# simonsobs/hmvec

Hardware: AMD Instinct MI355X
Metric: (z,m,k) grid-points/sec for P_1h+P_2h (higher is better)
Workload: dtype f64

## Files before the change

hmvec_amd/_native.py:

```python
import ctypes as C
import math
import os

import numpy as np

_HERE = os.path.dirname(os.path.abspath(__file__))
LIB_PATH = os.environ.get("HMG_LIB_PATH") or os.path.join(_HERE, "libhmgrid.so")
ABI_VERSION = 10
COMM_ID_BYTES = 128

c_double_p = C.c_void_p


class NativeError(RuntimeError):
    pass


class HaloStageArgs(C.Structure):
    _fields_ = [("d_zs", C.c_void_p), ("d_delta", C.c_void_p), ("d_rho", C.c_void_p),
                ("duffy_A", C.c_double), ("duffy_alpha", C.c_double), ("duffy_beta", C.c_double),
                ("h", C.c_double), ("d_cs", C.c_void_p), ("d_rvir", C.c_void_p), ("d_rs", C.c_void_p),
                ("d_nfw_series", C.c_void_p), ("d_drho1", C.c_void_p), ("delta2", C.c_double),
                ("d_rho2", C.c_void_p), ("d_m2", C.c_void_p), ("d_r2", C.c_void_p)]


class MassFnParams(C.Structure):
    _fields_ = [("mode", C.c_int), ("deltac", C.c_double), ("st_A", C.c_double),
                ("st_a", C.c_double), ("st_p", C.c_double), ("rho_m0", C.c_double),
                ("lnm_uniform", C.c_int), ("lnm_step", C.c_double)]


class HodParams(C.Structure):
    _fields_ = [("sig_log_mstellar", C.c_double), ("alphasat", C.c_double), ("Bsat", C.c_double),
                ("betasat", C.c_double), ("Bcut", C.c_double), ("betacut", C.c_double),
                ("corr", C.c_int)]


class Tracer(C.Structure):
    _fields_ = [("kind", C.c_int), ("d_prof", C.c_void_p), ("d_cprof", C.c_void_p),
                ("d_Nc", C.c_void_p), ("d_Ns", C.c_void_p), ("d_NcNs", C.c_void_p),
                ("d_NsNsm1", C.c_void_p), ("d_ngal", C.c_void_p),
                ("d_bias_override", C.c_void_p),
                ("d_prof_nconst", C.c_void_p), ("d_prof_cconst", C.c_void_p),
                ("d_cprof_nconst", C.c_void_p), ("d_cprof_cconst", C.c_void_p)]


class MassFnPart(C.Structure):
    _fields_ = [("h_par", C.POINTER(MassFnParams)), ("d_ms", C.c_void_p), ("d_lnms", C.c_void_p),
                ("d_tinker_z", C.c_void_p), ("d_sigma2", C.c_void_p), ("d_nzm", C.c_void_p), ("d_bh", C.c_void_p)]


class HodPart(C.Structure):
    _fields_ = [("stage", C.c_int), ("h_par", C.POINTER(HodParams)), ("d_zs", C.c_void_p), ("d_ms", C.c_void_p),
                ("d_log10mstar_thresh", C.c_void_p), ("d_nzm", C.c_void_p), ("d_bh", C.c_void_p),
                ("d_wm", C.c_void_p), ("d_Nc", C.c_void_p), ("d_Ns", C.c_void_p), ("d_NsNsm1", C.c_void_p),
                ("d_NcNs", C.c_void_p), ("d_ngal", C.c_void_p), ("d_bg", C.c_void_p)]


class RowsPart(C.Structure):
    _fields_ = [("kind", C.c_int), ("d_m200c", C.c_void_p), ("d_r200c", C.c_void_p), ("d_rvir", C.c_void_p),
                ("d_zs", C.c_void_p), ("d_rhocz", C.c_void_p), ("d_hz", C.c_void_p), ("fit", C.c_double * 9),
                ("gamma", C.c_double), ("alpha_const", C.c_double), ("amp_prefactor", C.c_double),
                ("post_prefactor", C.c_double), ("d_amp", C.c_void_p), ("d_xc", C.c_void_p),
                ("d_alpha", C.c_void_p), ("d_expo", C.c_void_p), ("d_cmax", C.c_void_p),
                ("d_rscale", C.c_void_p), ("d_post", C.c_void_p),
                ("d_ks", C.c_void_p), ("d_kts", C.c_void_p), ("nk", C.c_int), ("fft_m", C.c_int), ("d_rowsc", C.c_void_p)]


class NfwPart(C.Structure):
    _fields_ = [("d_cs", C.c_void_p), ("d_rs", C.c_void_p), ("d_zs", C.c_void_p), ("d_ks", C.c_void_p),
                ("d_nfw_series", C.c_void_p), ("d_uk", C.c_void_p)]


class ProfileFftPart(C.Structure):
    _fields_ = [("nxs", C.c_int), ("fft_step", C.c_double), ("d_xs", C.c_void_p), ("d_kts", C.c_void_p),
                ("d_amp", C.c_void_p), ("d_xc", C.c_void_p), ("d_alpha", C.c_void_p), ("d_expo", C.c_void_p),
                ("amp_const", C.c_double), ("xc_const", C.c_double), ("alpha_const", C.c_double),
                ("expo_const", C.c_double), ("gamma", C.c_double), ("d_cmax", C.c_void_p), ("d_rss", C.c_void_p),
                ("d_zs", C.c_void_p), ("d_ks", C.c_void_p), ("do_mass_norm", C.c_int), ("d_post", C.c_void_p),
                ("d_out", C.c_void_p), ("d_nconst", C.c_void_p), ("d_cconst", C.c_void_p), ("d_logxs", C.c_void_p),
                ("d_rowsc", C.c_void_p)]


class PowerBatchDesc(C.Structure):
    _fields_ = [("ntr", C.c_int), ("h_tr", C.POINTER(Tracer)), ("npairs", C.c_int),
                ("h_pair_a", C.POINTER(C.c_int)), ("h_pair_b", C.POINTER(C.c_int)),
                ("d_nzm", C.c_void_p), ("d_bh", C.c_void_p), ("d_ms", C.c_void_p), ("d_wm", C.c_void_p),
                ("d_ks", C.c_void_p), ("d_Pzk", C.c_void_p), ("rho_m0", C.c_double), ("kstar", C.c_double),
                ("h_P1h", C.POINTER(C.c_void_p)), ("h_P2h", C.POINTER(C.c_void_p))]


PB_PREPARED = 1
HOD_ALL, HOD_OCCUPATIONS, HOD_SUMS = 0, 1, 2
MF_SHETH_TORMEN, MF_TINKER10 = 0, 1
PROF_BATTAGLIA_GAS, PROF_BATTAGLIA_PRES = 1, 2
TRACER_MATTER, TRACER_HOD, TRACER_PRESSURE = 0, 1, 2
KERNEL_POWER, KERNEL_NFW, KERNEL_PROFILE_FFT = 0, 1, 2
EVENT_SLOTS = 4096
NFW_SERIES_STRIDE = 36
ROWSC_STRIDE = 8

_I, _D, _P, _Z = C.c_int, C.c_double, C.c_void_p, C.c_size_t
SIGNATURES = {
    "hmg_abi_version": [],
    "hmg_ctx_create": [_I, C.POINTER(_P)],
    "hmg_ctx_destroy": [_P],
    "hmg_malloc": [_P, _Z, C.POINTER(_P)],
    "hmg_free": [_P, _P],
    "hmg_memcpy_h2d": [_P, _P, _P, _Z],
    "hmg_memcpy_d2h": [_P, _P, _P, _Z],
    "hmg_memcpy_d2d": [_P, _P, _P, _Z],
    "hmg_sync": [_P],
    "hmg_host_alloc": [_P, _Z, C.POINTER(_P)],
    "hmg_host_free": [_P, _P],
    "hmg_memcpy_d2h_async": [_P, _P, _P, _Z],
    "hmg_memcpy_h2d_async": [_P, _P, _P, _Z],
    "hmg_event_synchronize": [_P, _I],
    "hmg_graph_begin": [_P],
    "hmg_graph_end": [_P, C.POINTER(_I)],
    "hmg_graph_abort": [_P],
    "hmg_graph_kernel_nodes": [_P, _I, C.POINTER(_I)],
    "hmg_graph_launch": [_P, _I],
    "hmg_graph_destroy": [_P, _I],
    "hmg_lane_set": [_P, _I],
    "hmg_profile_support_epoch": [_P, C.c_longlong],
    "hmg_event_wait": [_P, _I],
    "hmg_event_record": [_P, _I],
    "hmg_elapsed_ms": [_P, _I, _I, C.POINTER(_D)],
    "hmg_bracket_next": [_P, _I, _I, _I],
    "hmg_sigma2": [_P, _I, _I, _I, _P, _P, _P, _P, _D, _P],
    "hmg_sigma2_layout_size": [_I, _I, C.POINTER(_Z)],
    "hmg_sigma2_prepare": [_P, _I, _I, _P, _P],
    "hmg_sigma2_prepared": [_P, _I, _I, _I, _P, _P, _P, _P, _D, _P],
    "hmg_sigma2_massfn": [_P, _I, _I, _I, _P, _P, _P, _P, _D, C.POINTER(MassFnParams), _P, _P, _P, _P, _P, _P],
    "hmg_sigma2_massfn_halo": [_P, _I, _I, _I, _P, _P, _P, _P, _D, C.POINTER(MassFnParams), _P, _P, _P, _P, _P, _P,
                               C.POINTER(HaloStageArgs)],
    "hmg_halo_stage": [_P, _I, _I, _P, _P, _P, _P, _D, _D, _D, _D, _P, _P, _P, _P, _P, _D, _P, _P, _P],
    "hmg_massfn": [_P, _I, _I, C.POINTER(MassFnParams), _P, _P, _P, _P, _P, _P],
    "hmg_halo_structure": [_P, _I, _I, _P, _P, _P, _P, _D, _D, _D, _D, _P, _P, _P],
    "hmg_mdelta_convert": [_P, _I, _I, _P, _P, _P, _D, _P, _P, _P],
    "hmg_nfw_analytic": [_P, _I, _I, _I, _P, _P, _P, _P, _P, _P],
    "hmg_profile_rowparams": [_P, _I, _I, _I, _P, _P, _P, _P, _P, _P, C.POINTER(_D * 9), _D, _D, _D,
                              _D, _P, _P, _P, _P, _P, _P, _P],
    "hmg_profile_rows_from_mvir": [_P, _I, _I, _I, _P, _P, _P, _P, _P, _D, _P, _P, C.POINTER(_D * 9), _D, _D,
                                   _D, _D, _P, _P, _P, _P, _P, _P, _P, _P, _P],
    "hmg_profile_fft": [_P, _I, _I, _I, _I, _D, _P, _P, _P, _P, _P, _P, _D, _D, _D, _D, _D,
                        _P, _P, _P, _P, _I, _P, _P, _P, _P, _P],
    "hmg_profile_fft_logx": [_P, _I, _P, _P],
    "hmg_prefix_deferral": [_P, _I],
    "hmg_prefix_fill": [_P, _P],
    "hmg_prefix_pending": [_P, _P, C.POINTER(_I)],
    "hmg_prefix_fill_rows": [_P, _P, _P, _P, _I, _I],
    "hmg_hod": [_P, _I, _I, C.POINTER(HodParams), _P, _P, _P, _P, _P, _P, _P, _P, _P, _P, _P, _P],
    "hmg_power": [_P, _I, _I, _I, C.POINTER(Tracer), C.POINTER(Tracer), _P, _P, _P, _P, _P, _P,
                  _D, _D, _P, _P],
    "hmg_power_batch": [_P, _I, _I, _I, _I, C.POINTER(Tracer), _I, C.POINTER(_I), C.POINTER(_I),
                        _P, _P, _P, _P, _P, _P, _D, _D, C.POINTER(_P), C.POINTER(_P)],
    "hmg_power_2halo_terms": [_P, _I, _I, _I, C.POINTER(Tracer), C.POINTER(Tracer), _P, _P, _P, _P, _P, _D,
                              _P, _P, _P],
    "hmg_sigma2_halo_front": [_P, _I, _I, _I, _P, _P, _P, _P, _D, _P, C.POINTER(HaloStageArgs), C.POINTER(HodPart),
                              C.POINTER(RowsPart)],
    "hmg_group_rows": [_P, _I, _I, _I, _I, C.POINTER(MassFnPart), C.POINTER(HodPart), C.POINTER(RowsPart),
                       C.POINTER(NfwPart)],
    "hmg_group_profile": [_P, _I, _I, _I, C.POINTER(ProfileFftPart), C.POINTER(HodPart), C.POINTER(PowerBatchDesc)],
    "hmg_group_tensors": [_P, _I, _I, _I, _I, C.POINTER(MassFnPart), C.POINTER(HodPart), C.POINTER(PowerBatchDesc),
                          C.POINTER(NfwPart), C.POINTER(ProfileFftPart)],
    "hmg_power_batch_run": [_P, _I, _I, _I, C.POINTER(PowerBatchDesc), _I],
    "hmg_add": [_P, _Z, _P, _P, _P],
    "hmg_limber": [_P, _I, _P, _I, _I, _P, _P, _P, _P, _I, _P, _P, _P, _P, _P],
    "hmg_fn2d": [_P, _I, _I, _I, _I, C.POINTER(_P), C.POINTER(_I), C.POINTER(_I), C.POINTER(_D), _I, _P],
    "hmg_mstellar_halo": [_P, _I, _I, _P, _P, _P],
    "hmg_trapz_rows": [_P, _I, _I, _P, _P, _P],
    "hmg_sine_transform": [_P, _I, _I, _P, _P, _P],
    "hmg_profile_fft_table": [_P, _I, _I, _I, _I, _D, _P, _P, _P, _I, _P, _P, _P, _P, _I, _P],
    "hmg_lensing_sigma_nfw": [_P, _I, _I, _I, _P, _P, _P, _P, _P],
    "hmg_lensing_sigma_nfw_off": [_P, _I, _I, _I, _P, _P, _P, _P, _P, _P],
    "hmg_lensing_kappa_2h": [_P, _I, _I, _I, _I, _I, _P, _P, _P, _P, _P, _D, _D, _P, _P, _P, _P],
    "hmg_lensing_delta_sigma_nfw": [_P, _I, _I, _I, _P, _P, _P, _P, _P],
    "hmg_lensing_delta_sigma_nfw_off": [_P, _I, _I, _I, _P, _P, _P, _P, _P, _P],
    "hmg_lensing_gamma_t_2h": [_P, _I, _I, _I, _I, _I, _P, _P, _P, _P, _P, _D, _D, _P, _P, _P, _P],
    "hmg_ksz_pqperp": [_P, _I, _I, _I, _P, _P, _P, _P, _P, _P],
    "hmg_ksz_nvv": [_P, _I, _I, _I, _I, _I, _I, _P, _P, _P, _P, _P, _P, _P, _P, _P, _P, _P, _P, _P, _P],
    "hmg_ksz_limber_cl": [_P, _I, _I, _I, _I, _P, _P, _P, _P, _P, _P, _I, _D, _D, _P],
    "hmg_xi_transform": [_P, _I, _I, _I, _P, _P, _P, _P],
    "hmg_hankel_transform": [_P, _I, _I, _I, _P, _P, _P, _P, _P],
    "hmg_trispectrum_1h": [_P, _I, _I, _I, _I, C.POINTER(Tracer), C.POINTER(Tracer), C.POINTER(Tracer), C.POINTER(Tracer),
                           _P, _P, _P, _D, _P, _P, _P, _P, _P, _P],
    "hmg_comm_unique_id": [C.c_char * COMM_ID_BYTES],
    "hmg_comm_init": [_P, C.c_char * COMM_ID_BYTES, _I, _I],
    "hmg_comm_allgather": [_P, _P, _P, _Z],
    "hmg_comm_allgather_multi": [_P, _I, C.POINTER(_P), C.POINTER(_P), _Z],
    "hmg_comm_gather_async": [_P, _I, C.POINTER(_P), C.POINTER(_P), _Z, _I, _I, _I],
    "hmg_comm_allgatherv_multi": [_P, _I, C.POINTER(_P), C.POINTER(_P), C.POINTER(_Z)],
    "hmg_comm_gatherv_async": [_P, _I, C.POINTER(_P), C.POINTER(_P), C.POINTER(_Z), _I, _I, _I],
    "hmg_comm_info": [_P, C.POINTER(_I), C.POINTER(_I)],
    "hmg_comm_barrier": [_P],
    "hmg_comm_destroy": [_P],
}

_lib = None


def kernel_source_sha16():
    import hashlib
    h = hashlib.sha256()
    csrc = os.path.join(_HERE, "csrc")
    names = ["hmgrid.hip", "longgrid.hip", "longgrid.hpp", "rowdev.hpp", "sici.hpp", "ldsfft.hpp", "fastmath.hpp", "Makefile",
             "lensing.hip", "j0.hpp", "j1.hpp", "ksz.hip", "realspace.hip", "j01.hpp", "trispectrum.hip"]
    names += sorted(os.path.join("kernels", n) for n in os.listdir(os.path.join(csrc, "kernels")) if n.endswith(".hpp"))
    for name in names:
        with open(os.path.join(csrc, name), "rb") as f:
            h.update(f.read())
    return h.hexdigest()[:16]


def load():
    global _lib
    if _lib is not None:
        return _lib
    if not os.path.exists(LIB_PATH):
        raise ImportError(
            f"{LIB_PATH} not found: the HIP extension is not built and there is no CPU "
            "fallback. Run `make -C hmvec_amd/csrc` (needs hipcc, --offload-arch=gfx950).")
    lib = C.CDLL(LIB_PATH)
    for name, argtypes in SIGNATURES.items():
        fn = getattr(lib, name)
        fn.argtypes = argtypes
        fn.restype = C.c_int
    lib.hmg_last_error.argtypes = []
    lib.hmg_last_error.restype = C.c_char_p
    if lib.hmg_abi_version() != ABI_VERSION:
        raise ImportError(f"libhmgrid ABI {lib.hmg_abi_version()} != binding {ABI_VERSION}")
    _lib = lib
    return lib


def check(rc):
    if rc != 0:
        raise NativeError(load().hmg_last_error().decode("utf-8", "replace"))


class DeviceArray:

    __slots__ = ("ctx", "ptr", "shape", "_owner", "__weakref__")

    def __init__(self, ctx, ptr, shape, owner=True):
        self.ctx, self.ptr, self.shape, self._owner = ctx, ptr, tuple(int(s) for s in shape), owner

    @property
    def size(self):
        n = 1
        for s in self.shape:
            n *= s
        return n

    @property
    def nbytes(self):
        return self.size * 8

    def numpy(self):
        self.ctx.flush()
        out = np.empty(self.shape, dtype=np.float64)
        check(self.ctx.lib.hmg_memcpy_d2h(self.ctx.handle, out.ctypes.data, self.ptr, self.nbytes))
        return out

    def view(self, offset_elems, shape):
        v = DeviceArray(self.ctx, self.ptr + 8 * int(offset_elems), shape, owner=False)
        v._owner = self
        return v

    def free(self):
        if self._owner is True and self.ptr and self.ctx is not None and self.ctx.handle:
            self.ctx.lib.hmg_free(self.ctx.handle, self.ptr)
        self.ptr = 0

    def __del__(self):
        try:
            self.free()
        except Exception:
            pass


class PinnedArray:

    def __init__(self, ctx, shape):
        self.ctx = ctx
        shape = (shape,) if np.isscalar(shape) else tuple(int(s) for s in shape)
        n = int(np.prod(shape)) if shape else 1
        p = C.c_void_p()
        check(ctx.lib.hmg_host_alloc(ctx.handle, n * 8, C.byref(p)))
        self.ptr = p.value
        buf = (C.c_double * n).from_address(self.ptr)
        buf._hmg_owner = self
        self.array = np.frombuffer(buf, dtype=np.float64).reshape(shape)

    def __del__(self):
        try:
            if self.ptr and self.ctx.handle:
                self.ctx.lib.hmg_host_free(self.ctx.handle, self.ptr)
            self.ptr = 0
        except Exception:
            pass


class Context:

    def __init__(self, device=0):
        self.lib = load()
        h = C.c_void_p()
        check(self.lib.hmg_ctx_create(int(device), C.byref(h)))
        self.handle = h.value
        self.device = int(device)
        self.capture_serial = 0
        self._deferred = []
        self._trace = None
        self.shared = {}

    def defer(self, owner):
        if owner not in self._deferred:
            self._deferred.append(owner)

    def flush(self):
        while self._deferred:
            self._deferred.pop(0)._flush()

    def call_now(self, name, *args):
        if self._trace is not None:
            self._trace.append((name, args))
        check(getattr(self.lib, name)(self.handle, *args))

    def trace(self, fn):
        self.flush()
        self._trace = []
        try:
            fn()
            self.flush()
            return self._trace
        finally:
            self._trace = None

    def run_trace(self, calls):
        self.flush()
        lib, h = self.lib, self.handle
        for name, args in calls:
            check(getattr(lib, name)(h, *args))

    def close(self):
        self.shared = {}
        if getattr(self, "handle", None):
            self.lib.hmg_ctx_destroy(self.handle)
            self.handle = None

    def __del__(self):
        try:
            self.close()
        except Exception:
            pass

    def empty(self, shape):
        shape = (int(shape),) if isinstance(shape, (int, np.integer)) else tuple(int(v) for v in shape)
        n = math.prod(shape)
        p = C.c_void_p()
        check(self.lib.hmg_malloc(self.handle, n * 8, C.byref(p)))
        return DeviceArray(self, p.value, shape)

    def upload(self, arr):
        a = np.ascontiguousarray(arr, dtype=np.float64)
        d = self.empty(a.shape)
        check(self.lib.hmg_memcpy_h2d(self.handle, d.ptr, a.ctypes.data, a.nbytes))
        return d

    def upload_int32(self, arr):
        a = np.ascontiguousarray(arr, dtype=np.int32)
        d = self.empty(((a.size + 1) // 2,))
        check(self.lib.hmg_memcpy_h2d(self.handle, d.ptr, a.ctypes.data, a.nbytes))
        return d

    def write(self, dst, arr):
        self.flush()
        a = np.ascontiguousarray(arr, dtype=np.float64)
        if self._trace is not None:
            raise NativeError("Context.write inside Context.trace: a recorded call list cannot own host data")
        check(self.lib.hmg_memcpy_h2d(self.handle, dst.ptr, a.ctypes.data, a.nbytes))

    def copy(self, src):
        self.flush()
        d = self.empty(src.shape)
        self.call_now("hmg_memcpy_d2d", d.ptr, src.ptr, src.nbytes)
        return d

    def sync(self):
        self.flush()
        check(self.lib.hmg_sync(self.handle))

    def record(self, slot):
        self.call("hmg_event_record", slot)

    def lane(self, i):
        self.call("hmg_lane_set", i)

    def wait(self, slot):
        self.call("hmg_event_wait", slot)

    def elapsed_ms(self, s0, s1):
        ms = C.c_double()
        check(self.lib.hmg_elapsed_ms(self.handle, s0, s1, C.byref(ms)))
        return ms.value

    _NO_FLUSH = frozenset(["hmg_bracket_next", "hmg_profile_support_epoch", "hmg_prefix_deferral"])

    def call(self, name, *args):
        if name not in self._NO_FLUSH:
            self.flush()
        if self._trace is not None:
            self._trace.append((name, args))
        check(getattr(self.lib, name)(self.handle, *args))

    def capture(self, fn):
        self.flush()
        check(self.lib.hmg_graph_begin(self.handle))
        self.capture_serial += 1
        try:
            fn()
            self.flush()
        except BaseException:
            for o in self._deferred:
                o._drop_queue()
            self._deferred.clear()
            self.lib.hmg_graph_abort(self.handle)
            self.capture_serial += 1
            raise
        gid = C.c_int()
        try:
            check(self.lib.hmg_graph_end(self.handle, C.byref(gid)))
        finally:
            self.capture_serial += 1
        return gid.value

    def graph_kernel_nodes(self, gid):
        n = C.c_int()
        check(self.lib.hmg_graph_kernel_nodes(self.handle, gid, C.byref(n)))
        return n.value

    def replay(self, gid):
        self.call("hmg_graph_launch", gid)

    def copy_to_pinned(self, pinned, src):
        self.call("hmg_memcpy_d2h_async", pinned.ptr, src.ptr, src.nbytes)

    def copy_from_pinned(self, dst, pinned):
        self.call("hmg_memcpy_h2d_async", dst.ptr, pinned.ptr, dst.nbytes)

    def event_synchronize(self, slot):
        check(self.lib.hmg_event_synchronize(self.handle, slot))


_default_ctx = {}


def default_context(device=0):
    c = _default_ctx.get(device)
    if c is None or not c.handle:
        c = _default_ctx[device] = Context(device)
    return c


def context_or_default(ctx):
    return default_context(0) if ctx is None else ctx


def as_device(ctx, a):
    return a if isinstance(a, DeviceArray) else ctx.upload(np.ascontiguousarray(a, dtype=np.float64))


def ptr(x):
    return None if x is None else x.ptr
```

hmvec_amd/csrc/hmctx.hpp:

```cpp
#pragma once
#include <hip/hip_runtime.h>
#include <rccl/rccl.h>
#include <rocfft/rocfft.h>

#include <cstdio>
#include <map>
#include <string>
#include <tuple>
#include <vector>

#include "../../include/hmgrid.h"
#include "ldsfft.hpp"
#include "sici.hpp"

extern thread_local std::string g_last_error;
int fail(const char* what, const char* detail, const char* file, int line);
#define HIP_TRY(expr)                                                                   \
    do {                                                                                \
        hipError_t e_ = (expr);                                                         \
        if (e_ != hipSuccess) {                                                         \
            (void)hipGetLastError();                                                    \
            return fail(#expr, hipGetErrorString(e_), __FILE__, __LINE__);              \
        }                                                                               \
    } while (0)
#define FFT_TRY(expr)                                                                   \
    do {                                                                                \
        rocfft_status s_ = (expr);                                                      \
        if (s_ != rocfft_status_success) {                                              \
            char m_[32];                                                                \
            snprintf(m_, sizeof(m_), "rocfft status %d", (int)s_);                      \
            return fail(#expr, m_, __FILE__, __LINE__);                                 \
        }                                                                               \
    } while (0)
#define NCCL_TRY(expr)                                                                  \
    do {                                                                                \
        ncclResult_t r_ = (expr);                                                       \
        if (r_ != ncclSuccess) return fail(#expr, ncclGetErrorString(r_), __FILE__, __LINE__); \
    } while (0)
#define REQUIRE(cond, msg)                                                              \
    do {                                                                                \
        if (!(cond)) return fail("invalid argument", msg, __FILE__, __LINE__);          \
    } while (0)

struct FftPlan {
    rocfft_plan plan = nullptr;
    rocfft_execution_info info = nullptr;
    void* work = nullptr;
    size_t work_bytes = 0;
};

namespace hmg { struct UnpackTw; }
struct FusedPlan {
    hmg::FftPlanDev plan;
    hmg::cplx* twM = nullptr;
    hmg::UnpackTw* twN = nullptr;
    int maxb = 0, maxp = 0;
};

struct PrunedPlan {
    hmg::cplx* twB = nullptr;
    hmg::UnpackTw* twN = nullptr;
    hmg::cplx* twR = nullptr;
    hmg::UnpackTw* twNr = nullptr;
};
struct ChirpPlan {
    hmg::cplx *chP = nullptr, *chJ = nullptr, *Bw = nullptr;
    int Jw = 0;
};
struct SupportKey {
    const void *cmax, *xs, *rss, *ks;
    int rows, nxs, nk;
    long long epoch;
    bool operator<(const SupportKey& o) const {
        return std::tie(cmax, xs, rss, ks, rows, nxs, nk, epoch) < std::tie(o.cmax, o.xs, o.rss, o.ks, o.rows, o.nxs, o.nk, o.epoch);
    }
};

struct PrefixEntry {
    int* nconst = nullptr;
    double* cconst = nullptr;
    int rows = 0, nk = 0;
    bool pending = false;
};

struct hmg_ctx {
    int device = 0;
    hipStream_t stream = nullptr;
    hipStream_t lanes[HMG_LANES] = {};
    int lane = 0;
    hipEvent_t ev[HMG_EVENT_SLOTS] = {};
    int bracket[HMG_KERNEL_COUNT][2];
    void* scratch[7] = {nullptr, nullptr, nullptr, nullptr, nullptr, nullptr, nullptr};
    size_t scratch_bytes[7] = {0, 0, 0, 0, 0, 0, 0};
    std::map<std::pair<int, int>, FftPlan> plans;
    std::map<int, struct FusedPlan> fused;
    size_t fft_chunk_bytes = 0;
    int use_fused_fft = 1;
    int use_pruned_fft = 1;
    int fused_max_m = 6144;
    int fused_prefer_m = 2500;
    int pruned_lp_min = 0;
    int use_chirp = 1;
    int use_band_fft = 1;
    int use_tensor_group = 1;
    int fused_generic = 0;
    int force_gatherv = 0;
    std::map<std::tuple<int, int, int>, ChirpPlan> chirp;
    std::map<std::pair<int, int>, PrunedPlan> pruned;
    std::map<int, hmg::cplx*> pass_tw;
    std::map<SupportKey, std::pair<int, int>> support;
    int* h_fault = nullptr;
    int* d_fault = nullptr;
    long long support_epoch = 0;
    int sig_nz = 0, sig_nm = 0, sig_nq = 0;
    ncclComm_t comm = nullptr;
    int comm_rank = 0, comm_size = 1;
    double* d_barrier = nullptr;
    hmg::SiciTable* d_sici = nullptr;
    void* pinned[2] = {nullptr, nullptr};
    static constexpr int UP_SLOTS = 32;
    static constexpr size_t UP_SLOT_BYTES = (size_t)256 << 10;
    char* up_ring = nullptr;
    hipEvent_t up_ev[UP_SLOTS] = {};
    int up_next = 0;
    hipEvent_t pin_ev[2] = {nullptr, nullptr};
    int num_cu = 256;
    std::multimap<size_t, void*> free_blocks;
    std::map<void*, size_t> block_bytes;
    size_t cached_bytes = 0;
    bool lanes_dirty = false;
    bool capturing = false;
    std::vector<void*> freed_in_capture;
    std::map<int, std::vector<void*>> graph_blocks;
    std::map<int, hipGraphExec_t> graphs;
    std::map<int, int> graph_kernels;
    int next_graph_id = 1;
    int prefix_deferral = 0;
    std::map<void*, PrefixEntry> prefix;
    std::map<void*, PrefixEntry> prefix_capture;
    std::map<int, std::map<void*, PrefixEntry>> graph_prefix;
    hmg_ctx() { for (auto& b : bracket) b[0] = b[1] = -1; }
};
constexpr size_t FREE_CACHE_LIMIT = (size_t)4 << 30;

int event_at(hmg_ctx* c, int slot, hipEvent_t* out);
int check_fault(hmg_ctx* c);
int sync_all(hmg_ctx* c);
int ensure_scratch(hmg_ctx* c, int slot, size_t bytes);
int bracket_open(hmg_ctx* c, int kid, int* stop_slot);
int bracket_close(hmg_ctx* c, int stop_slot);
static inline void prefix_note(hmg_ctx* c, void* out, const PrefixEntry& e) {
    auto& m = c->capturing ? c->prefix_capture : c->prefix;
    if (e.nconst || c->capturing) m[out] = e;
    else m.erase(out);
}
static inline void prefix_replayed(hmg_ctx* c, const std::map<void*, PrefixEntry>& fx) {
    for (auto& kv : fx) {
        if (kv.second.nconst) c->prefix[kv.first] = kv.second;
        else c->prefix.erase(kv.first);
    }
}
static inline void prefix_drop_block(hmg_ctx* c, void* p, size_t bytes) {
    auto lo = c->prefix.lower_bound(p), hi = c->prefix.lower_bound((char*)p + bytes);
    c->prefix.erase(lo, hi);
}
static inline dim3 grid1d(size_t n, int block) { return dim3((unsigned)((n + block - 1) / block)); }
```

hmvec_amd/csrc/hmgrid.hip:

```cpp
#include <algorithm>
#include <cmath>
#include <cstdlib>
#include <cstring>

#include "hmctx.hpp"
#include "fastmath.hpp"
#include "rowdev.hpp"
#include "longgrid.hpp"

#include "kernels/common.hpp"
#include "kernels/sigma2.hpp"
#include "kernels/massfn.hpp"
#include "kernels/halo.hpp"
#include "kernels/nfw.hpp"
#include "kernels/rows.hpp"
#include "kernels/profile_chain.hpp"
#include "kernels/profile_fused.hpp"
#include "kernels/hod.hpp"
#include "kernels/power.hpp"
#include "kernels/power_batch.hpp"
#include "kernels/groups.hpp"
#include "kernels/limber.hpp"
#include "kernels/functions.hpp"

// ... 266 lines not shown
    FftPlan* P = nullptr;
    if (get_plan(c, n, nr, &P)) return 1;
    void* ib[1] = {in};
    void* ob[1] = {out};
    FFT_TRY(rocfft_execution_info_set_stream(P->info, c->stream));
    FFT_TRY(rocfft_execute(P->plan, ib, ob, P->info));
    return 0;
}


static int get_fused_plan(hmg_ctx* c, int nxs, FusedPlan** out) {
    *out = nullptr;
    auto it = c->fused.find(nxs);
    if (it != c->fused.end()) {
        if (it->second.twM) *out = &it->second;
        return 0;
    }
    FusedPlan P;
    const int M = nxs / 2;
    bool ok = (nxs % 2 == 0) && M >= 4 && fft_make_plan(M, &P.plan) && M <= c->fused_max_m;
    if (ok) {
        int maxb = 0;
        for (int i = 0; i < P.plan.npass; ++i) {
            const int nb = M / P.plan.radix[i];
            maxb = std::max(maxb, (nb + FUSED_NT - 1) / FUSED_NT);
        }
        P.maxb = maxb;
        P.maxp = (M / 2 + FUSED_NT - 1) / FUSED_NT;
        ok = maxb <= 4 && P.maxp <= 8;
    }
    if (!ok) {
        c->fused[nxs] = FusedPlan();
        return 0;
    }
    if (upload_table(pass_tw_table(P.plan), &P.twM) || upload_table(unpack_tw_table(nxs), &P.twN)) return 1;
    auto res = c->fused.emplace(nxs, P);
    *out = &res.first->second;
    return 0;
}

template <class... P, class... Args>
static int launch_lds(void (*kernel)(P...), dim3 grid, dim3 block, size_t lds, hipStream_t stream, const Args&... args) {
    if (lds > 48 * 1024)
        HIP_TRY(hipFuncSetAttribute((const void*)kernel, hipFuncAttributeMaxDynamicSharedMemorySize, (int)lds));
    hipLaunchKernelGGL(kernel, grid, block, lds, stream, args...);
    HIP_TRY(hipGetLastError());
    return 0;
}

template <int B, int P, int S, bool T = false>
struct RowShape {
    static constexpr int MAXB = B, MAXP = P, SPECM = S;
    static constexpr bool TABLE = T;
};
enum Shape { SHAPE_2500, SHAPE_500, SHAPE_1000, SHAPE_1500, SHAPE_2000, SHAPE_3000, SHAPE_RT12, SHAPE_RT23, SHAPE_RT24, SHAPE_RT48 };
template <class F>
static int with_shape(Shape s, F&& f) {
    switch (s) {
        case SHAPE_2500: return f(RowShape<2, 3, 2500, true>{});
        case SHAPE_500: return f(RowShape<1, 1, 500>{});
        case SHAPE_1000: return f(RowShape<1, 1, 1000>{});
        case SHAPE_1500: return f(RowShape<1, 2, 1500>{});
        case SHAPE_2000: return f(RowShape<2, 2, 2000>{});
        case SHAPE_3000: return f(RowShape<3, 3, 3000>{});
        case SHAPE_RT12: return f(RowShape<1, 2, 0>{});
        case SHAPE_RT23: return f(RowShape<2, 3, 0>{});
        case SHAPE_RT24: return f(RowShape<2, 4, 0, true>{});
        case SHAPE_RT48: return f(RowShape<4, 8, 0, true>{});
    }
    return fail("invalid argument", "internal: unknown row shape", __FILE__, __LINE__);
}

static Shape row_shape(const hmg_ctx* c, const FusedPlan& FP, bool table) {
    const FftPlanDev& pl = FP.plan;
    const bool ct = FUSED_NT == 512 && !c->fused_generic;
    if (ct && pl.M == 2500 && pl.npass == 5 && pl.radix[0] == 4 && pl.radix[1] == 5 && pl.radix[2] == 5 &&
        pl.radix[3] == 5 && pl.radix[4] == 5)
        return SHAPE_2500;
    if (table) return FP.maxb <= 2 && FP.maxp <= 4 ? SHAPE_RT24 : SHAPE_RT48;
    if (ct) switch (pl.M) {
            case 500: return SHAPE_500;
            case 1000: return SHAPE_1000;
            case 1500: return SHAPE_1500;
            case 2000: return SHAPE_2000;
            case 3000: return SHAPE_3000;
        }
    if (FP.maxb <= 1 && FP.maxp <= 2) return SHAPE_RT12;
    if (FP.maxb <= 2 && FP.maxp <= 3) return SHAPE_RT23;
    if (FP.maxb <= 2 && FP.maxp <= 4) return SHAPE_RT24;
    return SHAPE_RT48;
}

struct FftRiders {
    const ChainArgs* C = nullptr;
    int nchain = 0;
    size_t chain_lds = 0;
    const NfwArgs* N = nullptr;
    size_t nfw_blocks = 0;
    const double* rho_tab = nullptr;
    int rho_shared = 0;
    bool chain_done = false;
    bool nfw_done = false;
};

struct FftRoute {
    bool xs_aligned = false;
    bool try_long = false;
    FusedPlan* FP = nullptr;
    Shape shape = SHAPE_RT48;
    bool grouped = false;
    bool tensor = false;
};
static int fft_route(hmg_ctx* c, const hmg_profile_fft_part& p, bool chain, bool table, FftRoute* r) {
    *r = FftRoute{};
    r->xs_aligned = p.d_xs && ((uintptr_t)p.d_xs % 16) == 0;
    if (!c->use_fused_fft || !r->xs_aligned) return 0;
    if (get_fused_plan(c, p.nxs, &r->FP)) return 1;
    r->try_long = c->use_pruned_fft && (!r->FP || r->FP->plan.M > c->fused_prefer_m);
    if (!r->FP) return 0;
    r->shape = row_shape(c, *r->FP, table);
    r->grouped = chain && !table && FUSED_NT == 512 && p.d_rowsc && p.d_nconst;
    const bool ct = with_shape(r->shape, [](auto s) { return (int)(decltype(s)::SPECM != 0); });
    r->tensor = r->grouped && c->use_tensor_group && ct && !r->try_long;
    return 0;
}

template <class S>
static int launch_table(hmg_ctx* c, const FusedArgs& A, int rows) {
    const size_t lds = (size_t)A.plan.M * 16 + 32 * sizeof(double);
    if constexpr (S::TABLE)
        return launch_lds(profile_table_kernel<FUSED_NT, S::MAXB, S::MAXP, S::SPECM>, dim3(rows), dim3(FUSED_NT), lds, c->stream, A);
    else
        return fail("invalid argument", "internal: no table kernel of this row shape", __FILE__, __LINE__);
}

template <class S>
static int launch_fused(hmg_ctx* c, const FusedArgs& A, int rows) {
    const size_t lds = (size_t)A.plan.M * 16 + 32 * sizeof(double);
    return launch_lds(profile_fused_kernel<FUSED_NT, S::MAXB, S::MAXP, S::SPECM>, dim3(rows), dim3(FUSED_NT), lds, c->stream, A);
}

template <class S>
static int launch_group(hmg_ctx* c, const FusedArgs& A, int rows, const FftRiders& R) {
    constexpr int B = S::MAXB, P = S::MAXP, M = S::SPECM;
    const ChainArgs& C = *R.C;
    size_t lds = (size_t)A.plan.M * 16 + 32 * sizeof(double);
    if (R.chain_lds > lds) lds = R.chain_lds;
    if (R.N || C.has_mf) {
        if constexpr (M != 0) {
            const NfwArgs none{};
            const NfwArgs& N = R.N ? *R.N : none;
            const size_t nfw_blocks = R.N ? R.nfw_blocks : 0;
            REQUIRE((size_t)rows + R.nchain + nfw_blocks <= 2147483647u, "bad grid");
            return launch_lds(tensor_group_kernel<B, P, M>, dim3((unsigned)(rows + R.nchain + nfw_blocks)), dim3(FUSED_NT),
                              lds, c->stream, C, A, R.nchain, rows, N.T, N.acoef, N.ktile, N.nm, N.nk, N.cs, N.rss, N.zs,
                              N.ks, N.uk);
        } else {
            REQUIRE(false, "internal: the tensor group is compiled for compile-time plans only");
        }
    }
    return launch_lds(profile_group_kernel<B, P, M>, dim3(rows + R.nchain), dim3(FUSED_NT), lds, c->stream, C, A, R.nchain);
}

static const int PRUNED_LP[] = {1000, 1024, 1250, 1500, 2000, 2048, 2500};

static int get_pruned_plan(hmg_ctx* c, int nxs, int LP, PrunedPlan** out) {
    const auto key = std::make_pair(nxs, LP);
    auto it = c->pruned.find(key);
    if (it != c->pruned.end()) { *out = &it->second; return 0; }
    REQUIRE(!c->capturing, "long-grid tables cannot be built inside a captured step: run the step once eagerly first");
    const int M = nxs / 2;
    PrunedPlan P;
    if (LP == 0) {
        std::vector<cplx> twB(M);
        const long double twopi = 6.283185307179586476925286766559L;
        for (int t = 0; t < M; ++t) twB[t] = cplx{(double)cosl(twopi * t / M), (double)-sinl(twopi * t / M)};
        if (upload_table(twB, &P.twB) || upload_table(unpack_tw_table(nxs), &P.twN)) return 1;
    } else {
        if (upload_table(residue_tw_table(M, LP), &P.twR) || upload_table(residue_unpack_table(M, LP), &P.twNr)) return 1;
    }
    auto res = c->pruned.emplace(key, P);
    *out = &res.first->second;
    return 0;
}

static int get_pass_table(hmg_ctx* c, int L, const cplx** out) {
    auto it = c->pass_tw.find(L);
    if (it != c->pass_tw.end()) { *out = it->second; return 0; }
    REQUIRE(!c->capturing, "long-grid tables cannot be built inside a captured step: run the step once eagerly first");
    FftPlanDev plan;
    REQUIRE(fft_make_plan(L, &plan), "no radix-2/3/4/5 plan for a compiled sub-transform length");
    cplx* d = nullptr;
    if (upload_table(pass_tw_table(plan), &d)) return 1;
    c->pass_tw[L] = d;
    *out = d;
    return 0;
}

static int get_chirp_plan(hmg_ctx* c, int nxs, int LP, int p0, ChirpPlan** out) {
    const auto key = std::make_tuple(nxs, LP, p0);
    auto it = c->chirp.find(key);
    if (it != c->chirp.end()) { *out = &it->second; return 0; }
    REQUIRE(!c->capturing, "chirp tables cannot be built inside a captured step: run the step once eagerly first");
    const ChirpTables T = chirp_make_tables(nxs / 2, 2 * LP, p0);
    ChirpPlan P;
    P.Jw = T.Jw;
    if (upload_table(T.chP, &P.chP) || upload_table(T.chJ, &P.chJ) || upload_table(T.Bw, &P.Bw)) return 1;
    auto res = c->chirp.emplace(key, P);
    *out = &res.first->second;
    return 0;
}

static int profile_support(hmg_ctx* c, int rows, const FusedArgs& A, int* p0max, int* jnmax, int* known) {
    const SupportKey key{A.cmax, A.xs, A.nconst ? A.rss : nullptr, A.nconst ? A.ks : nullptr, rows, A.nxs, A.nk, c->support_epoch};
    *known = 1;
    if (c->capturing || c->support_epoch != 0) {
        auto it = c->support.find(key);
        if (it != c->support.end()) {
            *p0max = it->second.first;
            *jnmax = it->second.second;
            return 0;
        }
        if (c->capturing) { *known = 0; return 0; }
    }
    if (ensure_scratch(c, 2, 64)) return 1;
    int* d_p0 = (int*)c->scratch[2];
    HIP_TRY(hipMemsetAsync(d_p0, 0, 2 * sizeof(int), c->stream));
    HIP_TRY((hipError_t)launch_profile_support(c->stream, rows, A.nxs, A.xs, A.cmax, A.nconst ? A.rss : nullptr, A.zs, A.nm,
                                               A.kts, A.ks, A.nk, d_p0));
    int h[2] = {0, 0};
    HIP_TRY(hipMemcpyAsync(h, d_p0, 2 * sizeof(int), hipMemcpyDeviceToHost, c->stream));
    HIP_TRY(hipStreamSynchronize(c->stream));
    if (!A.nconst) h[1] = A.nxs / 2;
    if (c->support.size() >= 256) c->support.clear();
    c->support[key] = std::make_pair(h[0], h[1]);
    *p0max = h[0];
    *jnmax = h[1];
    return 0;
}

static int profile_fft_pruned(hmg_ctx* c, const FusedArgs& A0, int rows, bool can_fall_back, int* taken) {
    *taken = 0;
    const int nxs = A0.nxs, M = nxs / 2;
    if ((nxs & 1) || M < 2 * PRUNED_LP[0]) return 0;
    bool any = false;
    for (int lp : PRUNED_LP) any = any || (M % lp == 0 && M / lp >= 2);
    if (!any) return 0;
    int p0max = 0, jnmax = 0, known = 1;
    if (profile_support(c, rows, A0, &p0max, &jnmax, &known)) return 1;
    if (!known) {
        REQUIRE(can_fall_back, "profile support bound unknown inside a captured step: run the step once eagerly first");
        return 0;
    }
    int LP = 0;
    const int lp_min = c->pruned_lp_min > p0max ? c->pruned_lp_min : p0max;
    for (int lp : PRUNED_LP)
        if (M % lp == 0 && M / lp >= 2 && lp >= lp_min) { LP = lp; break; }
    if (!LP)
        for (int lp : PRUNED_LP)
            if (M % lp == 0 && M / lp >= 2 && lp >= p0max) { LP = lp; break; }
    if (!LP) {
        if (!c->use_band_fft || !A0.nconst) return 0;
        int LB = 0;
        for (int lb : {1000, 1024, 1250})
            if (M % lb == 0 && band_lb_compiled(lb) && 2 * jnmax + 2 <= lb) { LB = lb; break; }
        if (!LB) return 0;
        PrunedPlan *PP = nullptr, *PR = nullptr;
        const cplx* twL = nullptr;
        if (get_pruned_plan(c, nxs, 0, &PP)) return 1;
        if (get_pruned_plan(c, nxs, LB, &PR)) return 1;
        if (get_pass_table(c, LB, &twL)) return 1;
        PrunedArgs G{};
        G.F = A0;
        G.F.twN = PP->twN;
        if (ensure_scratch(c, 0, (size_t)3 * nxs * 8)) return 1;
        G.M = M; G.R = M / LB; G.twB = PP->twB; G.twL = twL; G.u = (double*)c->scratch[0]; G.fault = c->d_fault; G.row0 = 0;
        G.twR = PR->twR;
        int stop = -1;
        if (bracket_open(c, HMG_KERNEL_PROFILE_FFT, &stop)) return 1;
        HIP_TRY((hipError_t)launch_band(c->stream, LB, G, rows, jnmax));
        *taken = 1;
        return bracket_close(c, stop);
    }
    PrunedPlan *PP = nullptr, *PR = nullptr;
    const cplx* twL = nullptr;
    if (get_pruned_plan(c, nxs, 0, &PP)) return 1;
    if (get_pruned_plan(c, nxs, LP, &PR)) return 1;
    if (get_pass_table(c, LP, &twL)) return 1;
    size_t rpl = ((size_t)8 << 30) / ((size_t)M * 8);
    if (rpl < 1) rpl = 1;
    if (rpl > (size_t)rows) rpl = rows;
    if (ensure_scratch(c, 0, rpl * (size_t)M * 8)) return 1;
    PrunedArgs G;
    G.F = A0;
    G.F.twN = PP->twN;
    G.M = M; G.R = M / LP; G.twB = PP->twB; G.twL = twL; G.u = (double*)c->scratch[0]; G.fault = c->d_fault; G.row0 = 0;
    G.twR = PR->twR; G.twNr = PR->twNr; G.rmagic = (unsigned)(4294967296ull / (unsigned)G.R) + 1u;
    G.chP = G.chJ = G.Bw = G.twC = nullptr;
    G.Jw = 0; G.p0 = 0;
    if (c->use_chirp && (LP == 1000 || LP == 1250) && p0max >= 1) {
        int p0 = (p0max + 15) / 16 * 16;
        if (p0 > LP) p0 = LP;
        ChirpPlan* CP = nullptr;
        const cplx* twC = nullptr;
        if (get_chirp_plan(c, nxs, LP, p0, &CP)) return 1;
        if (get_pass_table(c, 2 * LP, &twC)) return 1;
        G.chP = CP->chP; G.chJ = CP->chJ; G.Bw = CP->Bw; G.twC = twC; G.Jw = CP->Jw; G.p0 = p0;
    }
    int stop = -1;
    if (bracket_open(c, HMG_KERNEL_PROFILE_FFT, &stop)) return 1;
    HIP_TRY((hipError_t)launch_pruned(c->stream, LP, G, rows, rpl));
    *taken = 1;
    return bracket_close(c, stop);
}

static FusedArgs fused_args(int nm, int nk, const hmg_profile_fft_part& p, const FusedPlan* FP, const FftRiders& R) {
    FusedArgs A{};
    if (FP) { A.plan = FP->plan; A.twM = FP->twM; A.twN = FP->twN; }
    A.nxs = p.nxs; A.nm = nm; A.nk = nk; A.do_norm = p.do_mass_norm;
    A.xs = p.d_xs; A.kts = p.d_kts;
    A.amp = p.d_amp; A.xc = p.d_xc; A.alpha = p.d_alpha; A.expo = p.d_expo;
    A.amp_c = p.amp_const; A.xc_c = p.xc_const; A.alpha_c = p.alpha_const; A.expo_c = p.expo_const; A.gamma = p.gamma;
    A.step = p.fft_step; A.cmax = p.d_cmax; A.rss = p.d_rss; A.zs = p.d_zs; A.ks = p.d_ks; A.post = p.d_post; A.out = p.d_out;
    A.nconst = p.d_nconst; A.cconst = p.d_cconst;
    A.logx = p.d_logxs;
    A.rho_tab = R.rho_tab; A.rho_shared = R.rho_shared;
    A.rowsc = (p.d_rowsc && p.d_nconst) ? p.d_rowsc : nullptr;
    return A;
}

static int profile_fft_impl(hmg_ctx* c, int nz, int nm, int nk, const hmg_profile_fft_part& p, FftRiders& R) {
    const int nxs = p.nxs;
    const double step = p.fft_step;
    const double *xs = p.d_xs, *kts = p.d_kts, *cmax = p.d_cmax, *rss = p.d_rss, *zs = p.d_zs, *ks = p.d_ks;
    R.chain_done = R.nfw_done = false;
    REQUIRE(c && xs && kts && cmax && rss && zs && ks && p.d_out, "NULL argument");
    REQUIRE((p.d_nconst == nullptr) == (p.d_cconst == nullptr), "pass both hint arrays or neither");
    REQUIRE(nz > 0 && nm > 0 && nk > 0, "empty grid");
    prefix_note(c, p.d_out, PrefixEntry{p.d_nconst, p.d_cconst, nz * nm, nk, false});
    REQUIRE(nxs >= 4, "nxs too small");
    const int nh = nxs / 2;
    const int rows = nz * nm;
    REQUIRE(step > 0.0, "step must be positive");
    const bool table = R.rho_tab != nullptr;
    FftRoute r;
    if (fft_route(c, p, R.C && R.nchain > 0, table, &r)) return 1;
    if (r.try_long) {
        int took = 0;
        if (profile_fft_pruned(c, fused_args(nm, nk, p, nullptr, R), rows, r.FP != nullptr, &took)) return 1;
        if (took) return 0;
    }
    if (r.FP) {
        FusedArgs A = fused_args(nm, nk, p, r.FP, R);
        A.defer = c->prefix_deferral && A.nconst;
        int stop = -1;
        if (bracket_open(c, HMG_KERNEL_PROFILE_FFT, &stop)) return 1;
        if (!table && !A.logx && rows >= 8192) {
            if (ensure_scratch(c, 2, (size_t)nxs * 8)) return 1;
            hipLaunchKernelGGL(logx_kernel, grid1d((size_t)nxs, 256), dim3(256), 0, c->stream, nxs, xs,
                               (double*)c->scratch[2]);
            HIP_TRY(hipGetLastError());
            A.logx = (const double*)c->scratch[2];
        }
        int rc;
        if (table) rc = with_shape(r.shape, [&](auto s) { return launch_table<decltype(s)>(c, A, rows); });
        else if (r.grouped) rc = with_shape(r.shape, [&](auto s) { return launch_group<decltype(s)>(c, A, rows, R); });
        else rc = with_shape(r.shape, [&](auto s) { return launch_fused<decltype(s)>(c, A, rows); });
        if (rc) return 1;
        if (A.defer) prefix_note(c, p.d_out, PrefixEntry{A.nconst, A.cconst, rows, nk, true});
        R.chain_done = r.grouped;
        R.nfw_done = r.grouped && R.N;
        return bracket_close(c, stop);
    }
    const int chunk = fft_chunk(c->fft_chunk_bytes ? c->fft_chunk_bytes : ((size_t)160 << 20),
                                (size_t)nxs * 8 + (size_t)(nh + 1) * 16, rows);
    if (ensure_scratch(c, 0, (size_t)chunk * nxs * 8)) return 1;
    if (ensure_scratch(c, 1, (size_t)chunk * (nh + 1) * 16)) return 1;
    if (ensure_scratch(c, 2, (size_t)chunk * 8)) return 1;
    double* fin = (double*)c->scratch[0];
    double2* fout = (double2*)c->scratch[1];
    double* mnorm = (double*)c->scratch[2];
    const bool stage = (size_t)nh * sizeof(double) <= 64 * 1024;
    const size_t lds = stage ? (size_t)nh * sizeof(double) : 0;
    int stop = -1;
    if (!table && bracket_open(c, HMG_KERNEL_PROFILE_FFT, &stop)) return 1;
    for (int r0 = 0; r0 < rows; r0 += chunk) {
        const int nr = rows - r0 < chunk ? rows - r0 : chunk;
        if (table)
            hipLaunchKernelGGL(table_integrand_kernel, dim3(nr), dim3(256), 0, c->stream, nxs, r0, xs, R.rho_tab,
                               R.rho_shared, cmax, p.do_mass_norm, fin, mnorm);
        else
            hipLaunchKernelGGL(integrand_kernel, dim3(nr), dim3(256), 0, c->stream, nxs, r0, xs, p.d_amp, p.d_xc,
                               p.d_alpha, p.d_expo, p.amp_const, p.xc_const, p.alpha_const, p.expo_const, p.gamma, cmax,
                               p.do_mass_norm, (int)r.xs_aligned, fin, mnorm);
        HIP_TRY(hipGetLastError());
        if (fft_r2c(c, nxs, nr, fin, fout)) return 1;
        if (stage)
            hipLaunchKernelGGL(interp_kernel<true>, dim3(nr), dim3(256), lds, c->stream, nm, nk, nh, r0, step,
                               (const double2*)fout, kts, mnorm, rss, zs, ks, p.d_post, p.d_out, p.d_nconst, p.d_cconst);
        else
            hipLaunchKernelGGL(interp_kernel<false>, dim3(nr), dim3(256), 0, c->stream, nm, nk, nh, r0, step,
                               (const double2*)fout, kts, mnorm, rss, zs, ks, p.d_post, p.d_out, p.d_nconst, p.d_cconst);
        HIP_TRY(hipGetLastError());
    }
    return bracket_close(c, stop);
}

int hmg_profile_fft(hmg_ctx* c, int nz, int nm, int nk, int nxs, double step, const double* xs, const double* kts,
                    const double* amp, const double* xcs, const double* alpha, const double* expo,
                    double amp_c, double xc_c, double alpha_c, double expo_c, double gamma,
                    const double* cmax, const double* rss, const double* zs, const double* ks,
                    int do_mass_norm, const double* post, double* out, int* nconst, double* cconst,
                    const double* logxs) {
    const hmg_profile_fft_part p{nxs, step, xs, kts, amp, xcs, alpha, expo, amp_c, xc_c, alpha_c, expo_c, gamma,
                                 cmax, rss, zs, ks, do_mass_norm, post, out, nconst, cconst, logxs};
    FftRiders R;
    return profile_fft_impl(c, nz, nm, nk, p, R);
}

int hmg_prefix_deferral(hmg_ctx* c, int on) {
    REQUIRE(c, "NULL ctx");
    c->prefix_deferral = on != 0;
    return 0;
}

int hmg_prefix_fill_rows(hmg_ctx* c, double* out, const int* nconst, const double* cconst, int rows, int nk) {
    REQUIRE(c && out && nconst && cconst, "NULL argument");
    REQUIRE(rows > 0 && nk > 0, "empty grid");
    hipLaunchKernelGGL(prefix_fill_kernel, dim3(rows), dim3(256), 0, c->stream, nk, nconst, cconst, out);
    HIP_TRY(hipGetLastError());
    return 0;
}

int hmg_prefix_pending(hmg_ctx* c, const double* out, int* pending) {
    REQUIRE(c && out && pending, "NULL argument");
    REQUIRE(!c->capturing, "the pending state is what replays make it: ask outside the captured step");
    auto it = c->prefix.find((void*)out);
    *pending = it != c->prefix.end() && it->second.pending;
    return 0;
}

int hmg_prefix_fill(hmg_ctx* c, double* out) {
    REQUIRE(c && out, "NULL argument");
    PrefixEntry e;
    if (c->capturing) {
        auto ic = c->prefix_capture.find(out);
        if (ic != c->prefix_capture.end()) {
            if (!ic->second.nconst || !ic->second.pending) return 0;
            e = ic->second;
        } else {
            auto ig = c->prefix.find(out);
            if (ig == c->prefix.end()) return 0;
            e = ig->second;
        }
    } else {
        auto it = c->prefix.find(out);
        if (it == c->prefix.end() || !it->second.pending) return 0;
        e = it->second;
    }
    if (hmg_prefix_fill_rows(c, out, e.nconst, e.cconst, e.rows, e.nk)) return 1;
    e.pending = false;
    prefix_note(c, out, e);
    return 0;
}

int hmg_profile_support_epoch(hmg_ctx* c, long long epoch) {
    REQUIRE(c, "NULL ctx");
    c->support_epoch = epoch;
    return 0;
}

int hmg_profile_fft_logx(hmg_ctx* c, int nxs, const double* xs, double* logxs) {
    REQUIRE(c && xs && logxs && nxs > 0, "bad argument");
    hipLaunchKernelGGL(logx_kernel, grid1d((size_t)nxs, 256), dim3(256), 0, c->stream, nxs, xs, logxs);
    HIP_TRY(hipGetLastError());
    return 0;
}

static int hod_dev(int nm, const hmg_hod_params* p, HodDev* P) {
    REQUIRE(p->corr == 0 || p->corr == 1, "corr must be 0 (max) or 1 (min)");
    REQUIRE((nm + 63) / 64 <= HOD_MAX_TILES, "nm too large for the HOD reduction (65536)");
    *P = HodDev{p->sig_log_mstellar, p->alphasat, p->Bsat, p->betasat, p->Bcut, p->betacut, p->corr};
    return 0;
}

int hmg_hod(hmg_ctx* c, int nz, int nm, const hmg_hod_params* p, const double* zs, const double* ms,
            const double* lthr, const double* nzm, const double* bh, const double* wm, double* Nc,
            double* Ns, double* NsNsm1, double* NcNs, double* ngal, double* bg) {
    REQUIRE(c && p && zs && ms && lthr && nzm && bh && wm && Nc && Ns && NsNsm1 && NcNs && ngal && bg,
            "NULL argument");
    REQUIRE(nz > 0 && nm > 0, "empty grid");
    HodDev P;
    if (hod_dev(nm, p, &P)) return 1;
    int hod_threads = std::min(1024, std::max(64, (nm + 63) / 64 * 64));
    if (const char* e = getenv("HMG_HOD_THREADS")) hod_threads = atoi(e);
    REQUIRE(hod_threads >= 64 && hod_threads <= 1024 && hod_threads % 64 == 0, "HMG_HOD_THREADS must be a multiple of 64 up to 1024");
    const HodRowArgs A{nm, P, zs, ms, lthr, nzm, bh, wm, Nc, Ns, NsNsm1, NcNs, ngal, bg};
    hipLaunchKernelGGL(hod_kernel, dim3(nz), dim3(hod_threads), 0, c->stream, A);
    HIP_TRY(hipGetLastError());
    return 0;
}

static int tensor_slot(std::vector<const double*>& list, const double* p) {
    if (!p) return -1;
    for (size_t i = 0; i < list.size(); ++i)
        if (list[i] == p) return (int)i;
    list.push_back(p);
    return (int)list.size() - 1;
}

static int fill_tracer(const hmg_tracer* t, std::vector<const double*>& tens, TracerDev* out) {
    REQUIRE(t->kind == HMG_TRACER_MATTER || t->kind == HMG_TRACER_HOD || t->kind == HMG_TRACER_PRESSURE,
            "unknown tracer kind");
    REQUIRE(t->d_prof, "tracer has no profile tensor");
    out->kind = t->kind;
    out->t_prof = tensor_slot(tens, t->d_prof);
    out->t_cprof = (t->kind == HMG_TRACER_HOD) ? tensor_slot(tens, t->d_cprof) : -1;
    out->Nc = t->d_Nc; out->Ns = t->d_Ns; out->NcNs = t->d_NcNs; out->NsNsm1 = t->d_NsNsm1;
    out->ngal = t->d_ngal; out->bias_override = t->d_bias_override;
    if (t->kind == HMG_TRACER_HOD)
        REQUIRE(t->d_Nc && t->d_Ns && t->d_NcNs && t->d_NsNsm1 && t->d_ngal, "HOD tracer needs Nc,Ns,NcNs,NsNsm1,ngal");
    return 0;
}

template <int NT, int V>
static int launch_power(hmg_ctx* c, const PowerArgs& A, int nz, int ms_split) {
    const int per_block = 64 * V;
    dim3 grid((A.nk + per_block - 1) / per_block, nz);
    const size_t lds = (size_t)ms_split * 3 * V * 64 * sizeof(double);
    int stop = -1;
    if (bracket_open(c, HMG_KERNEL_POWER, &stop)) return 1;
    if (launch_lds(power_kernel<NT, V>, grid, dim3(64 * ms_split), lds, c->stream, A)) return 1;
    return bracket_close(c, stop);
}

static int power_impl(hmg_ctx* c, int nz, int nm, int nk, const hmg_tracer* ta, const hmg_tracer* tb,
                      const double* nzm, const double* bh, const double* ms, const double* wm, const double* ks,
                      const double* Pzk, double rho_m0, double kstar, double* P1h, double* P2h,
                      double* I1, double* I2, double* Cout) {
    REQUIRE(c && ta && tb && nzm && bh && ms && wm && ks, "NULL argument");
    REQUIRE(P1h || P2h || (I1 && I2 && Cout), "no output requested");
    REQUIRE(!P2h || Pzk, "P2h needs Pzk");
    REQUIRE(nz > 0 && nm > 0 && nk > 0, "empty grid");
    REQUIRE(nz <= 65535, "nz too large");
    std::vector<const double*> tens;
    PowerPrep Q;
    if (fill_tracer(ta, tens, &Q.a)) return 1;
    if (fill_tracer(tb, tens, &Q.b)) return 1;
    Q.nt = (int)tens.size();
    Q.rho_m0 = rho_m0;
    REQUIRE(Q.nt >= 1 && Q.nt <= PW_MAXT, "bad tensor count");
    const int nc1 = 1 + Q.nt;
    if (ensure_scratch(c, 3, (size_t)nz * nm * PW_NF * nc1 * 8 + (size_t)nz * 4 * 8 + 64)) return 1;
    double* coef = (double*)c->scratch[3];
    double* side = coef + (size_t)nz * nm * PW_NF * nc1;
    hipLaunchKernelGGL(power_prep_kernel, dim3(nz), dim3(256), 0, c->stream, nm, Q, nzm, bh, ms, wm, coef, side);
    HIP_TRY(hipGetLastError());
    PowerArgs A;
    for (int i = 0; i < PW_MAXT; ++i) A.tens[i] = i < Q.nt ? tens[i] : nullptr;
    A.coef = coef; A.side = side; A.ks = ks; A.Pzk = Pzk; A.P1h = P1h; A.P2h = P2h;
    A.I1 = I1; A.I2 = I2; A.Cout = Cout;
    A.kstar = kstar; A.nm = nm; A.nk = nk;
    bool vec2 = (nk % 2 == 0);
    for (int i = 0; i < Q.nt; ++i) vec2 = vec2 && (((uintptr_t)tens[i]) % 16 == 0);
    int ms_split = 8;
    while (ms_split > 1 && ms_split > nm) ms_split >>= 1;
#define PW_CASE(NT_)                                                      \
    case NT_:                                                             \
        return vec2 ? launch_power<NT_, 2>(c, A, nz, ms_split) : launch_power<NT_, 1>(c, A, nz, ms_split);
    switch (Q.nt) {
        PW_CASE(1)
        PW_CASE(2)
        PW_CASE(3)
        PW_CASE(4)
    }
#undef PW_CASE
    return fail("hmg_power", "unreachable", __FILE__, __LINE__);
}

int hmg_power(hmg_ctx* c, int nz, int nm, int nk, const hmg_tracer* ta, const hmg_tracer* tb,
              const double* nzm, const double* bh, const double* ms, const double* wm, const double* ks,
              const double* Pzk, double rho_m0, double kstar, double* P1h, double* P2h) {
    return power_impl(c, nz, nm, nk, ta, tb, nzm, bh, ms, wm, ks, Pzk, rho_m0, kstar, P1h, P2h, nullptr, nullptr, nullptr);
}

int hmg_power_2halo_terms(hmg_ctx* c, int nz, int nm, int nk, const hmg_tracer* ta, const hmg_tracer* tb,
                          const double* nzm, const double* bh, const double* ms, const double* wm,
                          const double* ks, double rho_m0, double* I1, double* I2, double* C12) {
    REQUIRE(I1 && I2 && C12, "NULL output");
    return power_impl(c, nz, nm, nk, ta, tb, nzm, bh, ms, wm, ks, nullptr, rho_m0, 1.0, nullptr, nullptr, I1, I2, C12);
}

template <int NT, int NTR, int V, bool W16, unsigned CODE = 0>
static int launch_power_batch(hmg_ctx* c, const BatchArgs& A, int nz) {
    const int per_block = 64 * V;
    dim3 grid((A.nk + per_block - 1) / per_block, nz);
    constexpr int NACC = NTR + NTR * (NTR + 1) / 2;
    const size_t lds = (size_t)8 * NACC * V * 64 * sizeof(double);
    int stop = -1;
    if (bracket_open(c, HMG_KERNEL_POWER, &stop)) return 1;
    if (launch_lds(power_batch_kernel<NT, NTR, V, W16, CODE>, grid, dim3(W16 ? 1024 : 512), lds, c->stream, A)) return 1;
    return bracket_close(c, stop);
}

struct PbPlan {
    BatchPrep Q;
    PrepArgs PA;
    BatchArgs A;
    int ntr = 0, nt = 0, thin = 0;
    unsigned code = 0;
    bool vec2 = false;
};
static int pb_plan(hmg_ctx* c, int nz, int nm, int nk, const hmg_power_batch_desc* d, PbPlan* P) {
    REQUIRE(c && d && P, "NULL argument");
    const int ntr = d->ntr, npairs = d->npairs;
    const hmg_tracer* tr_in = d->h_tr;
    const int *pair_a = d->h_pair_a, *pair_b = d->h_pair_b;
    double* const* P1h = d->h_P1h;
    double* const* P2h = d->h_P2h;
    REQUIRE(tr_in && pair_a && pair_b && d->d_nzm && d->d_bh && d->d_ms && d->d_wm && d->d_ks, "NULL argument");
    REQUIRE(nz > 0 && nm > 0 && nk > 0, "empty grid");
    REQUIRE(nz <= 65535, "nz too large");
    REQUIRE(ntr >= 1 && ntr <= PB_MAXTR, "1..4 tracers per batch");
    REQUIRE(npairs >= 1, "no pairs");
    hmg_tracer tr[PB_MAXTR];
    int where[PB_MAXTR];
    {
        auto group = [&](int t) {
            if (tr_in[t].kind == HMG_TRACER_HOD) return 2;
            for (int u = 0; u < ntr; ++u)
                if (tr_in[u].kind == HMG_TRACER_HOD && tr_in[u].d_prof == tr_in[t].d_prof) return 0;
            return 1;
        };
        int n = 0;
        for (int pass = 0; pass < 3; ++pass)
            for (int t = 0; t < ntr; ++t)
                if (group(t) == pass) { tr[n] = tr_in[t]; where[t] = n++; }
    }
    std::vector<const double*> tens;
    BatchPrep& Q = P->Q;
    for (int t = 0; t < ntr; ++t) {
        REQUIRE(!tr[t].d_bias_override, "bias overrides are not supported in the batched kernel");
        if (fill_tracer(&tr[t], tens, &Q.tr[t])) return 1;
    }
    Q.ntr = ntr;
    Q.nt = (int)tens.size();
    Q.rho_m0 = d->rho_m0;
    REQUIRE(Q.nt >= 1 && Q.nt <= PW_MAXT, "more than 4 distinct profile tensors in one batch");
    unsigned code = 0;
    for (int t = 0; t < ntr; ++t) {
        const bool hod = Q.tr[t].kind == HMG_TRACER_HOD;
        if (hod && Q.tr[t].t_cprof >= 0) { code = 0; break; }
        code |= (hod ? PB_HOD(Q.tr[t].t_prof) : PB_LIN(Q.tr[t].t_prof)) << (4 * t);
    }
    if (getenv("HMG_PB_GENERIC")) code = 0;
    BatchArgs& A = P->A;
    for (int p = 0; p < PB_MAXPAIR; ++p) A.P1h[p] = A.P2h[p] = nullptr;
    bool any2 = false;
    for (int i = 0; i < npairs; ++i) {
        REQUIRE(pair_a[i] >= 0 && pair_a[i] < ntr && pair_b[i] >= 0 && pair_b[i] < ntr, "pair index out of range");
        int a = where[pair_a[i]], b = where[pair_b[i]];
        if (a > b) { int t = a; a = b; b = t; }
        const int p = a * ntr - a * (a - 1) / 2 + (b - a);
        REQUIRE((P1h && P1h[i]) || (P2h && P2h[i]), "pair without output");
        REQUIRE(!A.P1h[p] && !A.P2h[p], "the same unordered pair was requested twice");
        if (P1h && P1h[i]) A.P1h[p] = P1h[i];
        if (P2h && P2h[i]) { A.P2h[p] = P2h[i]; any2 = true; }
    }
    REQUIRE(!any2 || d->d_Pzk, "P2h needs Pzk");
    static const struct { int nt, ntr; unsigned code; } spec_list[] = {
#define PB_SPEC(NT_, NTR_, ...) {NT_, NTR_, pb_code(__VA_ARGS__)},
        PB_SPEC_LIST
#undef PB_SPEC
    };
    bool compiled = false;
    for (const auto& e : spec_list) compiled = compiled || (e.nt == Q.nt && e.ntr == ntr && e.code == code);
    if (!compiled) code = 0;
    Q.code = code;
    const int nc1 = 1 + Q.nt;
    const int stride = pb_stride(code, ntr, nc1);
    const int nblk = (nm + 63) / 64;
    REQUIRE(nblk <= 65535, "nm too large");
    if (ensure_scratch(c, 3, (size_t)nz * nm * stride * 8 + (size_t)nz * nblk * ntr * 2 * 8 + 64)) return 1;
    double* coef = (double*)c->scratch[3];
    double* sidep = coef + (size_t)nz * nm * stride;
    P->PA = PrepArgs{nm, nblk, Q, d->d_nzm, d->d_bh, d->d_ms, d->d_wm, coef, sidep};
    for (int i = 0; i < PW_MAXT; ++i) {
        A.tens[i] = i < Q.nt ? tens[i] : nullptr;
        A.nconst[i] = nullptr;
        A.cconst[i] = nullptr;
    }
    for (int t = 0; t < ntr; ++t) {
        const int sp = Q.tr[t].t_prof, sc = Q.tr[t].t_cprof;
        REQUIRE((tr[t].d_prof_nconst == nullptr) == (tr[t].d_prof_cconst == nullptr) &&
                (tr[t].d_cprof_nconst == nullptr) == (tr[t].d_cprof_cconst == nullptr), "hint arrays come in pairs");
        if (sp >= 0 && tr[t].d_prof_nconst && !A.nconst[sp]) { A.nconst[sp] = tr[t].d_prof_nconst; A.cconst[sp] = tr[t].d_prof_cconst; }
        if (sc >= 0 && tr[t].d_cprof_nconst && !A.nconst[sc]) { A.nconst[sc] = tr[t].d_cprof_nconst; A.cconst[sc] = tr[t].d_cprof_cconst; }
    }
    for (int t = 0; t < PB_MAXTR; ++t) {
        A.ngal[t] = (t < ntr && tr[t].kind == HMG_TRACER_HOD) ? tr[t].d_ngal : nullptr;
        A.bias_const[t] = (t < ntr && tr[t].kind == HMG_TRACER_MATTER) ? 1.0 : 0.0;
    }
    A.nblk = nblk;
    A.coef = coef; A.sidep = sidep; A.ks = d->d_ks; A.Pzk = d->d_Pzk; A.kstar = d->kstar; A.nm = nm; A.nk = nk;
    bool vec2 = (nk % 2 == 0);
    for (int i = 0; i < Q.nt; ++i) vec2 = vec2 && (((uintptr_t)tens[i]) % 16 == 0);
    const long tiles128 = (long)((nk + 127) / 128) * nz;
    int thin = tiles128 < c->num_cu ? 1 : (tiles128 < 2L * c->num_cu && vec2 ? 3 : 0);
    if (const char* e = getenv("HMG_PB_THIN")) thin = atoi(e);
    if (thin == 3 && !vec2) thin = 1;
    if (thin == 1 || thin == 2) vec2 = false;
    P->ntr = ntr; P->nt = Q.nt; P->thin = thin; P->code = code; P->vec2 = vec2;
    return 0;
}

static int pb_launch_main(hmg_ctx* c, const PbPlan& P, int nz) {
    const BatchArgs& A = P.A;
    const int thin = P.thin, ntr = P.ntr;
    const bool vec2 = P.vec2;
    const unsigned code = P.code;
#define PB_SHAPES(NT_, NTR_, CODE_)                                                        \
    if (thin == 3) return launch_power_batch<NT_, NTR_, 2, true, CODE_>(c, A, nz);         \
    return thin == 1 ? launch_power_batch<NT_, NTR_, 1, true, CODE_>(c, A, nz)             \
                     : (vec2 ? launch_power_batch<NT_, NTR_, 2, false, CODE_>(c, A, nz)    \
                             : launch_power_batch<NT_, NTR_, 1, false, CODE_>(c, A, nz));
    if (code) {
#define PB_SPEC(NT_, NTR_, ...)                                                            \
        if (P.nt == NT_ && ntr == NTR_ && code == pb_code(__VA_ARGS__)) { PB_SHAPES(NT_, NTR_, pb_code(__VA_ARGS__)) }
        PB_SPEC_LIST
#undef PB_SPEC
    }
#define PB_V(NT_, NTR_) PB_SHAPES(NT_, NTR_, 0u)
#define PB_NTR(NT_)                         \
    switch (ntr) {                          \
        case 1: PB_V(NT_, 1)                \
        case 2: PB_V(NT_, 2)                \
        case 3: PB_V(NT_, 3)                \
        case 4: PB_V(NT_, 4)                \
    }                                       \
    break;
    switch (P.nt) {
        case 1: PB_NTR(1)
        case 2: PB_NTR(2)
        case 3: PB_NTR(3)
        case 4: PB_NTR(4)
    }
#undef PB_NTR
#undef PB_V
#undef PB_SHAPES
    return fail("hmg_power_batch", "unreachable", __FILE__, __LINE__);
}

int hmg_power_batch_run(hmg_ctx* c, int nz, int nm, int nk, const hmg_power_batch_desc* d, int flags) {
    PbPlan P;
    if (pb_plan(c, nz, nm, nk, d, &P)) return 1;
    if (!(flags & HMG_PB_PREPARED)) {
        hipLaunchKernelGGL(power_batch_prep_kernel, dim3(nz, P.PA.nblk), dim3(64), 0, c->stream, P.PA);
        HIP_TRY(hipGetLastError());
    }
    return pb_launch_main(c, P, nz);
}

int hmg_power_batch(hmg_ctx* c, int nz, int nm, int nk, int ntr, const hmg_tracer* tr_in, int npairs,
                    const int* pair_a, const int* pair_b, const double* nzm, const double* bh,
                    const double* ms, const double* wm, const double* ks, const double* Pzk,
                    double rho_m0, double kstar, double* const* P1h, double* const* P2h) {
    const hmg_power_batch_desc d{ntr, tr_in, npairs, pair_a, pair_b, nzm, bh, ms, wm, ks, Pzk, rho_m0, kstar, P1h, P2h};
    return hmg_power_batch_run(c, nz, nm, nk, &d, 0);
}

static int rows_setup(int nz, int nm, const hmg_rows_part* rows, RowsArgs* out) {
    RowsArgs Rw{};
    REQUIRE(rows->d_m200c && rows->d_r200c && rows->d_rvir && rows->d_zs && rows->d_rhocz && rows->d_amp && rows->d_xc &&
                rows->d_alpha && rows->d_expo && rows->d_cmax && rows->d_rscale, "NULL argument in the rows part");
    if (row_fit(rows->kind, rows->d_hz, rows->d_post, rows->fit, &Rw.F)) return 1;
    Rw.n = nz * nm; Rw.kind = rows->kind; Rw.nm = nm;
    Rw.m200 = rows->d_m200c; Rw.r200 = rows->d_r200c; Rw.rvir = rows->d_rvir; Rw.zs = rows->d_zs;
    Rw.rhoc = rows->d_rhocz; Rw.hz = rows->d_hz;
    Rw.gamma = rows->gamma; Rw.alpha_const = rows->alpha_const; Rw.pref = rows->amp_prefactor;
    Rw.post_pref = rows->post_prefactor;
    Rw.O = RowOut{rows->d_amp, rows->d_xc, rows->d_alpha, rows->d_expo, rows->d_cmax, rows->d_rscale, rows->d_post};
    if (rows->d_rowsc) {
        REQUIRE(rows->d_ks && rows->d_kts && rows->nk > 0 && rows->fft_m >= 2, "row scalars need d_ks, d_kts, nk and fft_m");
        Rw.O.rowsc = rows->d_rowsc; Rw.O.ks = rows->d_ks; Rw.O.kts = rows->d_kts; Rw.O.nk = rows->nk; Rw.O.M = rows->fft_m;
    }
    *out = Rw;
    return 0;
}

static int hod_args(int nm, const hmg_hod_part* hod, HodRowArgs* A) {
    const hmg_hod_params* p = hod->h_par;
    REQUIRE(p && hod->d_zs && hod->d_ms && hod->d_log10mstar_thresh && hod->d_Nc && hod->d_Ns && hod->d_NsNsm1 &&
                hod->d_NcNs, "NULL argument in the HOD part");
    REQUIRE(hod->stage == HMG_HOD_OCCUPATIONS || (hod->d_nzm && hod->d_bh && hod->d_wm && hod->d_ngal && hod->d_bg),
            "NULL argument in the HOD part");
    HodDev P;
    if (hod_dev(nm, p, &P)) return 1;
    *A = HodRowArgs{nm, P, hod->d_zs, hod->d_ms, hod->d_log10mstar_thresh, hod->d_nzm, hod->d_bh, hod->d_wm,
                    hod->d_Nc, hod->d_Ns, hod->d_NsNsm1, hod->d_NcNs, hod->d_ngal, hod->d_bg};
    return 0;
}

int hmg_sigma2_halo_front(hmg_ctx* c, int nz, int nm, int nq, const double* PT, const double* kq, const double* wq,
                          const double* R, double tswitch, const double* ms, const hmg_halo_stage_args* h,
                          const hmg_hod_part* hod, const hmg_rows_part* rows) {
    REQUIRE(c && PT && kq && wq && R, "NULL argument");
    REQUIRE(nz > 0 && nm > 0 && nq > 0, "empty grid");
    HaloStageArgs H;
    if (halo_stage_check(c, nz, nm, ms, h, &H)) return 1;
    HodRowArgs O{};
    int nocc = 0;
    if (hod) {
        REQUIRE(hod->stage == HMG_HOD_OCCUPATIONS, "only the occupations of an HOD need inputs only");
        if (hod_args(nm, hod, &O)) return 1;
        nocc = (nz * nm + 63) / 64;
    }
    RowsArgs Rw{};
    if (rows) {
        if (rows_setup(nz, nm, rows, &Rw)) return 1;
        REQUIRE(h->d_m2 && rows->d_m200c == h->d_m2 && rows->d_r200c == h->d_r2 && rows->d_rvir == h->d_rvir,
                "row parameters in the front launch take M_200c, R_200c, r_vir from the halo stage of the same call");
    }
    const int nhalo = (nz * nm + 63) / 64;
    SigmaFrontArgs G;
    dim3 sig;
    if (sigma2_setup(c, nz, nm, nq, PT, kq, wq, R, tswitch, (size_t)nhalo + nocc, &G, &sig)) return 1;
    const dim3 grid((unsigned)((size_t)sig.x * sig.y * sig.z + nhalo + nocc));
    if (sigma2_ztile(nz) == 32)
        hipLaunchKernelGGL(front_group_kernel<2>, grid, dim3(64), 0, c->stream, G, H, nhalo, O, nocc, Rw);
    else
        hipLaunchKernelGGL(front_group_kernel<1>, grid, dim3(64), 0, c->stream, G, H, nhalo, O, nocc, Rw);
    HIP_TRY(hipGetLastError());
    return 0;
}

static int chain_setup(int nm, const hmg_hod_part* hod, const PbPlan* prep, ChainArgs* C, int* n) {
    C->has_hod = C->has_prep = C->has_mf = C->mf_pad = 0;
    if (hod) {
        REQUIRE(hod->stage == HMG_HOD_SUMS, "a chain takes the n_gal, b_g sums of an HOD (its occupations ride with the front)");
        if (hod_args(nm, hod, &C->H)) return 1;
        C->has_hod = 1;
    }
    if (prep && prep->code) {
        C->PA = prep->PA;
        C->has_prep = 1;
    }
    *n = (C->has_hod || C->has_prep) ? 1 : 0;
    return 0;
}
static int massfn_setup(hmg_ctx* c, int nz, int nm, int nq, const hmg_massfn_part* mf, SigmaMassFnArgs* S) {
    const hmg_massfn_params* p = mf->h_par;
    REQUIRE(p && mf->d_ms && mf->d_lnms && mf->d_sigma2 && mf->d_nzm && mf->d_bh, "NULL argument in the massfn part");
    MassFnDev P;
    if (massfn_dev(p, mf->d_tinker_z, &P)) return 1;
    REQUIRE(c->sig_nz == nz && c->sig_nm == nm && c->sig_nq == nq && c->scratch[4],
            "no sigma^2 partial sums of this shape in the context: call hmg_sigma2_halo_front first");
    const int nseg = (nq + SIG_SEG_LEN - 1) / SIG_SEG_LEN;
    *S = SigmaMassFnArgs{nz, nm, nseg, P, (const double*)c->scratch[4], mf->d_ms, mf->d_lnms, mf->d_tinker_z,
                         mf->d_sigma2, mf->d_nzm, mf->d_bh};
    return 0;
}

static int nfw_setup(hmg_ctx* c, int nz, int nm, int nk, const hmg_nfw_part* nfw, NfwArgs* N, size_t* blocks) {
    REQUIRE(nfw->d_cs && nfw->d_rs && nfw->d_zs && nfw->d_ks && nfw->d_nfw_series && nfw->d_uk, "NULL argument in the NFW part");
    const int ktile = 4096;
    *blocks = (size_t)nz * nm * ((nk + ktile - 1) / ktile);
    *N = NfwArgs{c->d_sici, nfw->d_nfw_series, ktile, nm, nk, nfw->d_cs, nfw->d_rs, nfw->d_zs, nfw->d_ks, nfw->d_uk};
    return 0;
}

static int launch_rows_group(hmg_ctx* c, int nz, int nm, const ChainArgs& C, int nchain, const SigmaMassFnArgs* S,
                             const RowsArgs& Rw, const NfwArgs* N, size_t nfw_blocks) {
    const int nrowblk = Rw.n ? (Rw.n + 255) / 256 : 0;
    const int mf_ntile = (nm + MF_TILE - 1) / MF_TILE;
    const int nmfblk = S ? nz * mf_ntile : 0;
    const size_t blocks = (size_t)nchain + nmfblk + nrowblk + nfw_blocks;
    REQUIRE(blocks > 0 && blocks <= 2147483647u, "bad grid");
    const size_t lds = nchain ? chain_lds_doubles(nm) * 8 : 0;
    RowsGroupArgs G{};
    G.C = C; G.Rw = Rw; G.nchain = nchain; G.nrowblk = nrowblk; G.nmfblk = nmfblk; G.mf_ntile = mf_ntile;
    if (S) G.S = *S;
    const NfwArgs n = N ? *N : NfwArgs{};
    hipLaunchKernelGGL(rows_group_kernel, dim3((unsigned)blocks), dim3(256), lds, c->stream, G, n.T, n.acoef, n.ktile,
                       n.nm, n.nk, n.cs, n.rss, n.zs, n.ks, n.uk);
    HIP_TRY(hipGetLastError());
    return 0;
}

int hmg_group_rows(hmg_ctx* c, int nz, int nm, int nk, int nq, const hmg_massfn_part* mf, const hmg_hod_part* hod,
                   const hmg_rows_part* rows, const hmg_nfw_part* nfw) {
    REQUIRE(c, "NULL ctx");
    REQUIRE(nz > 0 && nm > 0, "empty grid");
    REQUIRE(mf || hod || rows || nfw, "empty group");
    REQUIRE(!(mf && hod), "an HOD needs the n, b of the massfn part: it cannot share its launch");
    REQUIRE((nm + 63) / 64 <= HOD_MAX_TILES, "nm too large");
    ChainArgs C;
    int one = 0;
    if (chain_setup(nm, hod, nullptr, &C, &one)) return 1;
    REQUIRE(one || mf || rows || nfw, "empty group");
    SigmaMassFnArgs S;
    if (mf && massfn_setup(c, nz, nm, nq, mf, &S)) return 1;
    RowsArgs Rw{};
    if (rows && rows_setup(nz, nm, rows, &Rw)) return 1;
    NfwArgs N{};
    size_t nfw_blocks = 0;
    int stop = -1;
    if (nfw) {
        REQUIRE(nk > 0, "empty grid");
        if (nfw_setup(c, nz, nm, nk, nfw, &N, &nfw_blocks)) return 1;
        if (bracket_open(c, HMG_KERNEL_NFW, &stop)) return 1;
    }
    if (launch_rows_group(c, nz, nm, C, one ? nz : 0, mf ? &S : nullptr, Rw, nfw ? &N : nullptr, nfw_blocks)) return 1;
    return bracket_close(c, stop);
}

static int profile_group_launches(hmg_ctx* c, int nz, int nm, int nk, const hmg_profile_fft_part* fft, const ChainArgs& C, int one,
                                  const hmg_power_batch_desc* prep, const PbPlan& P, const NfwArgs* N = nullptr,
                                  size_t nfw_blocks = 0, bool* nfw_done = nullptr) {
    FftRiders R;
    R.C = &C; R.nchain = one ? nz : 0; R.chain_lds = chain_lds_doubles(nm, C.has_mf != 0, 512) * 8;
    R.N = N; R.nfw_blocks = nfw_blocks;
    if (fft && profile_fft_impl(c, nz, nm, nk, *fft, R)) return 1;
    if (nfw_done) *nfw_done = R.nfw_done;
    if (one && !R.chain_done) {
        REQUIRE(!C.has_mf, "internal: the transform did not take the route the tensor group was set up for");
        const RowsArgs none{};
        if (launch_rows_group(c, nz, nm, C, nz, nullptr, none, nullptr, 0)) return 1;
    }
    if (prep && !P.code) {
        hipLaunchKernelGGL(power_batch_prep_kernel, dim3(nz, P.PA.nblk), dim3(64), 0, c->stream, P.PA);
        HIP_TRY(hipGetLastError());
    }
    return 0;
}

int hmg_group_profile(hmg_ctx* c, int nz, int nm, int nk, const hmg_profile_fft_part* fft, const hmg_hod_part* hod,
                      const hmg_power_batch_desc* prep) {
    REQUIRE(c, "NULL ctx");
    REQUIRE(nz > 0 && nm > 0 && nk > 0, "empty grid");
    REQUIRE(fft || hod || prep, "empty group");
    REQUIRE((nm + 63) / 64 <= HOD_MAX_TILES, "nm too large");
    PbPlan P;
    if (prep && pb_plan(c, nz, nm, nk, prep, &P)) return 1;
    ChainArgs C;
    int one = 0;
    if (chain_setup(nm, hod, prep ? &P : nullptr, &C, &one)) return 1;
    return profile_group_launches(c, nz, nm, nk, fft, C, one, prep, P);
}

int hmg_group_tensors(hmg_ctx* c, int nz, int nm, int nk, int nq, const hmg_massfn_part* mf, const hmg_hod_part* hod,
                      const hmg_power_batch_desc* prep, const hmg_nfw_part* nfw, const hmg_profile_fft_part* fft) {
    REQUIRE(c, "NULL ctx");
    REQUIRE(nz > 0 && nm > 0 && nk > 0, "empty grid");
    REQUIRE(fft, "the tensor group is built around the rows of a profile transform: use hmg_group_rows without one");
    REQUIRE((nm + 63) / 64 <= HOD_MAX_TILES, "nm too large");
    PbPlan P;
    if (prep && pb_plan(c, nz, nm, nk, prep, &P)) return 1;
    ChainArgs C;
    int one = 0;
    if (chain_setup(nm, hod, prep ? &P : nullptr, &C, &one)) return 1;
    FftRoute r;
    if (fft_route(c, *fft, one || mf, false, &r)) return 1;
    if (!r.tensor) {
        if ((mf || nfw) && hmg_group_rows(c, nz, nm, nk, nq, mf, nullptr, nullptr, nfw)) return 1;
        return profile_group_launches(c, nz, nm, nk, fft, C, one, prep, P);
    }
    if (mf) {
        if (massfn_setup(c, nz, nm, nq, mf, &C.S)) return 1;
        C.has_mf = 1;
        one = 1;
    }
    NfwArgs N{};
    size_t nfw_blocks = 0;
    if (nfw && nfw_setup(c, nz, nm, nk, nfw, &N, &nfw_blocks)) return 1;
    bool nfw_done = false;
    if (profile_group_launches(c, nz, nm, nk, fft, C, one, prep, P, nfw ? &N : nullptr, nfw_blocks, &nfw_done)) return 1;
    REQUIRE(!nfw || nfw_done, "internal: the transform did not take the route the tensor group was set up for");
    return 0;
}

int hmg_limber(hmg_ctx* c, int nells, const double* ells, int nz, int nk, const double* zs,
               const double* ks, const double* P, const double* P2, int ngz, const double* gzs,
               const double* pref, const double* chis, const double* wz, double* out) {
    REQUIRE(c && ells && zs && ks && P && gzs && pref && chis && wz && out, "NULL argument");
    REQUIRE(nells > 0 && nz >= 1 && nk >= 2 && ngz >= 1, "bad sizes");
    hipLaunchKernelGGL(limber_kernel, grid1d((size_t)nells, LIMBER_E), dim3(LIMBER_G * LIMBER_E), 0, c->stream, nells, ells, nz,
                       nk, zs, ks, P, P2, ngz, gzs, pref, chis, wz, out);
    HIP_TRY(hipGetLastError());
    return 0;
}

int hmg_fn2d(hmg_ctx* c, int op, int rows, int cols, int nin, const double* const* in, const int* sr,
             const int* sc, const double* par, int npar, double* out) {
    static const int need_in[HMG_FN_COUNT] = {1, 4, 2, 2, 4, 1, 2, 2, 1, 3, 3, 2, 2, 4, 4, 5, 4, 3, 1, 4, 4, 1, 4, 2, 3, 2, 3};
    static const int need_par[HMG_FN_COUNT] = {1, 3, 0, 1, 1, 2, 1, 1, 0, 0, 0, 4, 3, 12, 12, 14, 14, 0, 0, 0, 0, 4, 4, 1, 3, 10, 0};
    REQUIRE(c && in && sr && sc && out, "NULL argument");
    REQUIRE(op >= 0 && op < HMG_FN_COUNT, "unknown function id");
    REQUIRE(rows > 0 && cols > 0, "empty grid");
    REQUIRE(nin == need_in[op] && nin <= HMG_FN_MAXIN, "wrong number of inputs for this function");
    REQUIRE(npar == need_par[op] && npar <= HMG_FN_MAXPAR && (npar == 0 || par), "wrong number of parameters for this function");
    FnArgs A;
    A.op = op; A.rows = rows; A.cols = cols; A.out = out;
    for (int i = 0; i < HMG_FN_MAXIN; ++i) { A.in[i] = nullptr; A.sr[i] = 0; A.sc[i] = 0; }
    for (int i = 0; i < nin; ++i) {
        REQUIRE(in[i], "NULL input");
        REQUIRE(sr[i] >= 0 && sc[i] >= 0, "negative stride");
        A.in[i] = in[i]; A.sr[i] = sr[i]; A.sc[i] = sc[i];
    }
    for (int i = 0; i < HMG_FN_MAXPAR; ++i) A.par[i] = i < npar ? par[i] : 0.0;
    if (op == HMG_FN_TINKER_FNU || op == HMG_FN_TINKER_FSIGMA) REQUIRE(par[0] == 0.0 || par[2] >= 2.0, "alpha table needs >= 2 rows");
    if (op == HMG_FN_HOD_NSNSM1 || op == HMG_FN_HOD_NCNS) REQUIRE(par[0] == 0.0 || par[0] == 1.0, "corr must be 0 (max) or 1 (min)");
    hipLaunchKernelGGL(fn2d_kernel, grid1d((size_t)rows * cols, 256), dim3(256), 0, c->stream, A);
    HIP_TRY(hipGetLastError());
    return 0;
}

int hmg_mstellar_halo(hmg_ctx* c, int nz, int nm, const double* zs, const double* lmh, double* out) {
    REQUIRE(c && zs && lmh && out, "NULL argument");
    REQUIRE(nz > 0 && nm > 0, "empty grid");
    hipLaunchKernelGGL(mstellar_halo_kernel, dim3(nz), dim3(1024), 0, c->stream, nm, zs, lmh, out);
    HIP_TRY(hipGetLastError());
    return 0;
}

int hmg_add(hmg_ctx* c, size_t n, const double* a, const double* b, double* out) {
    REQUIRE(c && a && b && out, "NULL argument");
    if (!n) return 0;
    hipLaunchKernelGGL(add2_kernel, grid1d(n, 256), dim3(256), 0, c->stream, n, a, b, out);
    HIP_TRY(hipGetLastError());
    return 0;
}

int hmg_trapz_rows(hmg_ctx* c, int rows, int cols, const double* y, const double* x, double* out) {
    REQUIRE(c && y && x && out, "NULL argument");
    REQUIRE(rows > 0 && cols > 0, "empty grid");
    hipLaunchKernelGGL(trapz_rows_kernel, dim3(rows), dim3(256), 0, c->stream, cols, y, x, out);
    HIP_TRY(hipGetLastError());
    return 0;
}

int hmg_sine_transform(hmg_ctx* c, int rows, int n, const double* x, const double* y, double* uk) {
    REQUIRE(c && x && y && uk, "NULL argument");
    REQUIRE(rows > 0 && n >= 2, "bad sizes");
    const int nh1 = n / 2 + 1;
    const int chunk = fft_chunk((size_t)160 << 20, (size_t)n * 8 + (size_t)nh1 * 16, rows);
    if (ensure_scratch(c, 0, (size_t)chunk * n * 8)) return 1;
    if (ensure_scratch(c, 1, (size_t)chunk * nh1 * 16)) return 1;
    double* fin = (double*)c->scratch[0];
    double2* fout = (double2*)c->scratch[1];
    double ends[2];
    HIP_TRY(hipMemcpyAsync(&ends[0], x, 8, hipMemcpyDeviceToHost, c->stream));
    HIP_TRY(hipMemcpyAsync(&ends[1], x + (n - 1), 8, hipMemcpyDeviceToHost, c->stream));
    HIP_TRY(hipStreamSynchronize(c->stream));
    const double step = (ends[1] - ends[0]) / (double)n;
    for (int r0 = 0; r0 < rows; r0 += chunk) {
        const int nr = rows - r0 < chunk ? rows - r0 : chunk;
        hipLaunchKernelGGL(xy_kernel, grid1d((size_t)nr * n, 256), dim3(256), 0, c->stream, nr, n, x,
                           y + (size_t)r0 * n, fin);
        HIP_TRY(hipGetLastError());
        if (fft_r2c(c, n, nr, fin, fout)) return 1;
        hipLaunchKernelGGL(neg_imag_kernel, grid1d((size_t)nr * nh1, 256), dim3(256), 0, c->stream,
                           (size_t)nr * nh1, step, (const double2*)fout, uk + (size_t)r0 * nh1);
        HIP_TRY(hipGetLastError());
    }
    return 0;
}

int hmg_profile_fft_table(hmg_ctx* c, int nz, int nm, int nk, int nxs, double step, const double* xs,
                          const double* kts, const double* rho, int rho_rows, const double* cmax,
                          const double* rss, const double* zs, const double* ks, int do_mass_norm,
                          double* out) {
    REQUIRE(c && xs && kts && rho && cmax && rss && zs && ks && out, "NULL argument");
    REQUIRE(nz > 0 && nm > 0 && nk > 0, "empty grid");
    REQUIRE(nxs >= 4, "nxs too small");
    REQUIRE(step > 0.0, "step must be positive");
    const int rows = nz * nm;
    REQUIRE(rho_rows == 1 || rho_rows == rows, "rho must have 1 or nz*nm rows");
    hmg_profile_fft_part p{};
    p.nxs = nxs; p.fft_step = step; p.d_xs = xs; p.d_kts = kts; p.d_cmax = cmax; p.d_rss = rss; p.d_zs = zs; p.d_ks = ks;
    p.do_mass_norm = do_mass_norm; p.d_out = out;
    p.amp_const = p.xc_const = p.alpha_const = p.expo_const = 1.0;
    FftRiders R;
    R.rho_tab = rho; R.rho_shared = rho_rows == 1;
    return profile_fft_impl(c, nz, nm, nk, p, R);
}
```

hmvec_amd/csrc/kernels/groups.hpp:

```cpp
#pragma once

namespace hmg {

struct RowsArgs {
    int n;
    int kind, nm;
    const double *m200, *r200, *rvir, *zs, *rhoc, *hz;
    RowFit F;
    double gamma, alpha_const, pref, post_pref;
    RowOut O;
};
struct SigmaFrontArgs {
    int nz, nzp, nm, nq, gx, nseg;
    const double *PT, *kq, *wq, *R;
    double tswitch;
    double* partial;
};
template <int ZB>
__global__ __launch_bounds__(64, HMG_SIG_OCC) void front_group_kernel(SigmaFrontArgs G, HaloStageArgs H, int nhalo,
                                                                     HodRowArgs O, int nocc, RowsArgs Rw) {
    int b = blockIdx.x;
    if (b < nocc) {
        const int idx = b * 64 + threadIdx.x;
        if (idx < G.nz * O.nm) hod_occ_point(O, idx / O.nm, idx - (idx / O.nm) * O.nm);
        return;
    }
    b -= nocc;
    if (b < nhalo) {
        const int idx = b * 64 + threadIdx.x;
        if (idx < H.nz * H.nm) {
            double rv, m2, r2;
            halo_stage_point(H, idx, &rv, &m2, &r2);
            if (Rw.n) {
                const int z = idx / Rw.nm;
                rowparams_body(Rw.kind, idx, m2, r2, rv, 1.0 + Rw.zs[z], Rw.rhoc[z], Rw.hz ? Rw.hz[z] : 1.0, Rw.F,
                               Rw.gamma, Rw.alpha_const, Rw.pref, Rw.post_pref, Rw.O);
            }
        }
        return;
    }
    b -= nhalo;
    const int r = b / G.gx, bx = b - r * G.gx;
    const int bz = r / G.nseg, seg = r - bz * G.nseg;
    sigma2_mfma_block<ZB>(bx, seg, bz, G.nz, G.nzp, G.nm, G.nq, G.PT, G.kq, G.wq, G.R, G.tswitch, G.partial);
}

struct ChainArgs {
    int has_hod, has_prep;
    HodRowArgs H;
    PrepArgs PA;
    int has_mf, mf_pad;
    SigmaMassFnArgs S;
};
static inline size_t chain_lds_doubles(int nm, bool has_mf = false, int nt = 512) {
    const size_t hod = 2 * (size_t)((nm + 63) / 64), mf = has_mf ? (size_t)nt : 0;
    return hod > mf ? hod : mf;
}
#define HMG_KERNARG __attribute__((address_space(4)))
template <class T>
__device__ __forceinline__ const T HMG_KERNARG* uniform_kernarg(const T HMG_KERNARG* p) {
    const unsigned long long v = (unsigned long long)p;
    const unsigned lo = __builtin_amdgcn_readfirstlane((unsigned)v), hi = __builtin_amdgcn_readfirstlane((unsigned)(v >> 32));
    return (const T HMG_KERNARG*)(((unsigned long long)hi << 32) | lo);
}
template <class T>
__device__ __forceinline__ T kernarg_load(const T HMG_KERNARG* p) {
    static_assert(sizeof(T) % 8 == 0, "pad the argument block to 8 bytes");
    union { T v; unsigned long long w[sizeof(T) / 8]; } u;
    const unsigned long long HMG_KERNARG* q = (const unsigned long long HMG_KERNARG*)p;
#pragma unroll
    for (unsigned i = 0; i < sizeof(T) / 8; ++i) u.w[i] = q[i];
    return u.v;
}
template <int NT, bool MF = false>
__device__ __forceinline__ void chain_row(const ChainArgs& C, int z, double* lds) {
    if (MF && C.has_mf) {
        massfn_row<NT>(C.S, z, lds);
        __threadfence_block();
        __syncthreads();
    }
    if (C.has_hod) {
        hod_sums_row(C.H, z, NT, lds);
        __syncthreads();
    }
    if (C.has_prep)
        for (int blk = threadIdx.x >> 6; blk < C.PA.nblk; blk += NT / 64) batch_prep_tile_compact(C.PA, z, blk);
}

__device__ __forceinline__ void rows_block(const RowsArgs& Rw, int b) {
    const int idx = b * 256 + threadIdx.x;
    if (idx < Rw.n) {
        const int z = idx / Rw.nm;
        rowparams_body(Rw.kind, idx, Rw.m200[idx], Rw.r200[idx], Rw.rvir[idx], 1.0 + Rw.zs[z], Rw.rhoc[z],
                       Rw.hz ? Rw.hz[z] : 1.0, Rw.F, Rw.gamma, Rw.alpha_const, Rw.pref, Rw.post_pref, Rw.O);
    }
}
__device__ __forceinline__ void massfn_block(const SigmaMassFnArgs& S, int b, int nt) {
    __shared__ double red[4 * 64];
    __shared__ double sig[64];
    sigma2_massfn_tile(S, b / nt, b - (b / nt) * nt, red, sig);
}
struct RowsGroupArgs {
    ChainArgs C;
    RowsArgs Rw;
    SigmaMassFnArgs S;
    int nchain, nrowblk, nmfblk, mf_ntile;
};
#ifndef HMG_ROWS_OCC
#define HMG_ROWS_OCC 7
#endif
__global__ __launch_bounds__(256, HMG_ROWS_OCC) void rows_group_kernel(RowsGroupArgs G, const SiciTable* __restrict__ T,
                                                                      const double* __restrict__ acoef, int ktile, int nm,
                                                                      int nk, const double* __restrict__ cs,
                                                                      const double* __restrict__ rss,
                                                                      const double* __restrict__ zs,
                                                                      const double* __restrict__ ks,
                                                                      double* __restrict__ uk) {
    extern __shared__ double lds[];
    int b = blockIdx.x;
    if (b < G.nchain) {
        chain_row<256>(G.C, b, lds);
        return;
    }
    b -= G.nchain;
    if (b < G.nmfblk) {
        massfn_block(G.S, b, G.mf_ntile);
        return;
    }
    b -= G.nmfblk;
    if (b < G.nrowblk) {
        rows_block(G.Rw, b);
        return;
    }
    nfw_rows(T, acoef, ktile, nm, nk, cs, rss, zs, ks, uk, b - G.nrowblk, 256, threadIdx.x);
}

template <int MAXB, int MAXP, int SPECM>
__global__ __launch_bounds__(512, (fused_occ<MAXB, SPECM>())) void profile_group_kernel(ChainArgs C, FusedArgs A,
                                                                                              int nchain) {
    extern __shared__ __attribute__((aligned(16))) double smem[];
    const int b = blockIdx.x;
    if (b < nchain) {
        chain_row<512>(C, b, smem);
        return;
    }
    profile_fused_row<512, MAXB, MAXP, SPECM, false, true>(A, row_order(b - nchain, A.nm), smem);
}

template <int MAXB, int MAXP, int SPECM>
__global__ __launch_bounds__(512, (fused_occ<MAXB, SPECM>())) void tensor_group_kernel(
    ChainArgs C, FusedArgs A, int nchain, int nprof, const SiciTable* __restrict__ T, const double* __restrict__ acoef,
    int ktile, int nm, int nk, const double* __restrict__ cs, const double* __restrict__ rss,
    const double* __restrict__ zs, const double* __restrict__ ks, double* __restrict__ uk) {
    extern __shared__ __attribute__((aligned(16))) double smem[];
    int b = blockIdx.x;
    if (b < nchain) {
        chain_row<512, true>(C, b, smem);
        return;
    }
    b -= nchain;
    if (b < nprof) profile_fused_row<512, MAXB, MAXP, SPECM, false, true>(A, row_order(b, A.nm), smem);
    else nfw_rows(T, acoef, ktile, nm, nk, cs, rss, zs, ks, uk, b - nprof, 512, threadIdx.x);
}

}
```

hmvec_amd/csrc/kernels/massfn.hpp:

```cpp
#pragma once

namespace hmg {

struct MassFnDev {
    int mode;
    double deltac, A, a, p, rho_m0;
    int uniform;
    double step;
};

__device__ __forceinline__ double tinker10_bias(double nu) {
    const double dc = 1.686;
    const double y = log10(200.0);
    const double ey = exp(-pow(4.0 / y, 4.0));
    const double A = 1.0 + 0.24 * y * ey;
    const double a = 0.44 * y - 0.88;
    const double C = 0.019 + 0.107 * y + 0.19 * ey;
    const double nua = pow(nu, a);
    return 1.0 - A * nua / (nua + pow(dc, a)) + 0.183 * pow(nu, 1.5) + C * pow(nu, 2.4);
}

template <class SigmaAt>
__device__ __forceinline__ void massfn_point(const MassFnDev& P, int z, int m, int nm, SigmaAt S,
                                             const double* __restrict__ ms, const double* __restrict__ lnm,
                                             const double* __restrict__ tz, double& n_out, double& b_out) {
    const double sig2 = S(m);
    const double dc = P.deltac;
    double f, b;
    if (P.mode == HMG_MF_SHETH_TORMEN) {
        const double sig = sqrt(sig2);
        f = P.A * sqrt(2.0 * P.a / M_PI) * (1.0 + pow(sig2 / P.a / (dc * dc), P.p)) * (dc / sig) *
            exp(-P.a * (dc * dc) / 2.0 / sig2);
        const double t = P.a * (dc * dc) / sig2;
        b = 1.0 + (1.0 / dc) * (t - 1.0) + (2.0 * P.p / dc) / (1.0 + pow(t, P.p));
    } else {
        const double nu = dc / sqrt(sig2);
        const double al = tz[z * 5 + 0], be = tz[z * 5 + 1], ph = tz[z * 5 + 2], et = tz[z * 5 + 3],
                     ga = tz[z * 5 + 4];
        const double fnu = al * ((1.0 + pow(be * nu, -2.0 * ph)) * pow(nu, 2.0 * et) *
                                 exp(-ga * (nu * nu) / 2.0));
        f = nu * fnu;
        b = tinker10_bias(nu);
    }
    auto L = [&](int i) { return -0.5 * log(S(i)); };
    double g;
    if (nm == 1) {
        g = 0.0;
    } else if (m == 0) {
        g = (L(1) - L(0)) / (P.uniform ? P.step : (lnm[1] - lnm[0]));
    } else if (m == nm - 1) {
        g = (L(nm - 1) - L(nm - 2)) / (P.uniform ? P.step : (lnm[nm - 1] - lnm[nm - 2]));
    } else if (P.uniform) {
        g = (L(m + 1) - L(m - 1)) / (2.0 * P.step);
    } else {
        const double d1 = lnm[m] - lnm[m - 1], d2 = lnm[m + 1] - lnm[m];
        const double ca = -d2 / (d1 * (d1 + d2)), cb = (d2 - d1) / (d1 * d2), cc = d1 / (d2 * (d1 + d2));
        g = ca * L(m - 1) + cb * L(m) + cc * L(m + 1);
    }
    const double mm = ms[m];
    n_out = P.rho_m0 * f * g / (mm * mm);
    b_out = b;
}

__global__ void massfn_kernel(int nz, int nm, MassFnDev P, const double* __restrict__ s2,
                              const double* __restrict__ ms, const double* __restrict__ lnm,
                              const double* __restrict__ tz, double* __restrict__ nzm,
                              double* __restrict__ bh) {
    const int idx = blockIdx.x * blockDim.x + threadIdx.x;
    if (idx >= nz * nm) return;
    const int z = idx / nm, m = idx - z * nm;
    const double* row = s2 + (size_t)z * nm;
    double n, b;
    massfn_point(P, z, m, nm, [&](int i) { return row[i]; }, ms, lnm, tz, n, b);
    nzm[idx] = n;
    bh[idx] = b;
}

struct SigmaMassFnArgs {
    int nz, nm, parts;
    MassFnDev P;
    const double *partial , *ms, *lnm, *tz;
    double *s2, *nzm, *bh;
};
__device__ __forceinline__ void sigma2_massfn_block(const SigmaMassFnArgs& A, int z, int m0, double (*red)[66],
                                                    double* sig) {
    const int lane = threadIdx.x & 63, w = threadIdx.x >> 6;
    const int nm = A.nm, n = A.nz * nm;
    const int j = w < 4 ? lane + 1 : (lane == 0 ? 0 : 65);
    if (w < 4 || lane < 2) {
        const int m = min(max(m0 - 1 + j, 0), nm - 1);
        red[w & 3][j] = sigma2_segment_sum(n, A.parts, A.partial, (size_t)z * nm + m, w & 3);
    }
    __syncthreads();
    if (threadIdx.x < 66) {
        const int jj = threadIdx.x;
        const double v = ((red[0][jj] + red[1][jj]) + red[2][jj]) + red[3][jj];
        sig[jj] = v;
        const int m = m0 - 1 + jj;
        if (jj >= 1 && jj <= 64 && m < nm) A.s2[(size_t)z * nm + m] = v;
    }
    __syncthreads();
    const int m = m0 + threadIdx.x;
    if (threadIdx.x < 64 && m < nm) {
        double nn, bb;
        massfn_point(A.P, z, m, nm, [&](int i) { return sig[i - m0 + 1]; }, A.ms, A.lnm, A.tz, nn, bb);
        A.nzm[(size_t)z * nm + m] = nn;
        A.bh[(size_t)z * nm + m] = bb;
    }
}
__global__ __launch_bounds__(512) void sigma2_massfn_kernel(SigmaMassFnArgs A) {
    __shared__ double red[4][66];
    __shared__ double sig[66];
    sigma2_massfn_block(A, blockIdx.y, blockIdx.x * 64, red, sig);
}
constexpr int MF_TILE = 62;
__device__ __forceinline__ void sigma2_massfn_tile(const SigmaMassFnArgs& A, int z, int tile, double* red, double* sig) {
    const int lane = threadIdx.x & 63, w = threadIdx.x >> 6;
    const int nm = A.nm, n = A.nz * nm, m0 = tile * MF_TILE;
    if (w < 4) {
        const int m = min(max(m0 - 1 + lane, 0), nm - 1);
        red[w * 64 + lane] = sigma2_segment_sum(n, A.parts, A.partial, (size_t)z * nm + m, w);
    }
    __syncthreads();
    if (w == 0) {
        const double v = ((red[lane] + red[64 + lane]) + red[128 + lane]) + red[192 + lane];
        sig[lane] = v;
        const int m = m0 - 1 + lane;
        if (lane >= 1 && lane <= MF_TILE && m < nm) A.s2[(size_t)z * nm + m] = v;
    }
    __syncthreads();
    const int m = m0 + (int)threadIdx.x;
    if (threadIdx.x < MF_TILE && m < nm) {
        double nn, bb;
        massfn_point(A.P, z, m, nm, [&](int i) { return sig[i - m0 + 1]; }, A.ms, A.lnm, A.tz, nn, bb);
        A.nzm[(size_t)z * nm + m] = nn;
        A.bh[(size_t)z * nm + m] = bb;
    }
}

template <int NT>
__device__ __forceinline__ void massfn_row(const SigmaMassFnArgs& A, int z, double* sig) {
    const int nm = A.nm, n = A.nz * nm, t = (int)threadIdx.x;
    const bool one = nm <= NT;
    const int stride = one ? NT : NT - 2;
    for (int first = 0; first < nm; first += stride) {
        const int base = one ? 0 : first - 1;
        const int m = base + t;
        const size_t i = (size_t)z * nm + min(max(m, 0), nm - 1);
        const double g0 = sigma2_segment_sum(n, A.parts, A.partial, i, 0), g1 = sigma2_segment_sum(n, A.parts, A.partial, i, 1);
        const double g2 = sigma2_segment_sum(n, A.parts, A.partial, i, 2), g3 = sigma2_segment_sum(n, A.parts, A.partial, i, 3);
        const double v = ((g0 + g1) + g2) + g3;
        sig[t] = v;
        const bool mine = m < nm && (one || (t >= 1 && t <= NT - 2));
        if (mine) A.s2[i] = v;
        __syncthreads();
        if (mine) {
            double nn, bb;
            massfn_point(A.P, z, m, nm, [&](int k) { return sig[k - base]; }, A.ms, A.lnm, A.tz, nn, bb);
            A.nzm[i] = nn;
            A.bh[i] = bb;
        }
        __syncthreads();
    }
}

}
```

hmvec_amd/csrc/kernels/power_batch.hpp:

```cpp
#pragma once

namespace hmg {

constexpr int PB_MAXTR = 4;
constexpr int PB_MAXPAIR = PB_MAXTR * (PB_MAXTR + 1) / 2;

constexpr unsigned PB_LIN(int s) { return 1u | ((unsigned)s << 2); }
constexpr unsigned PB_HOD(int s) { return 2u | ((unsigned)s << 2); }
constexpr unsigned pb_code(unsigned t0, unsigned t1 = 0, unsigned t2 = 0, unsigned t3 = 0) {
    return t0 | (t1 << 4) | (t2 << 8) | (t3 << 12);
}
constexpr int pb_kind(unsigned code, int r) { return (int)((code >> (4 * r)) & 3u); }
constexpr int pb_slot(unsigned code, int r) { return (int)((code >> (4 * r + 2)) & 3u); }
constexpr int pb_ncoef(unsigned code, int ntr) {
    int n = 2;
    for (int r = 0; r < ntr; ++r) n += pb_kind(code, r) == 2 ? 4 : 1;
    return n;
}
constexpr int pb_stride(unsigned code, int ntr, int nc1) {
    return code ? ((pb_ncoef(code, ntr) + 7) & ~7) : 2 + ntr * 3 * nc1;
}

#define PB_SPEC_LIST                                                  \
    PB_SPEC(1, 1, PB_LIN(0))                                          \
    PB_SPEC(1, 2, PB_LIN(0), PB_HOD(0))                               \
    PB_SPEC(2, 2, PB_LIN(0), PB_LIN(1))                               \
    PB_SPEC(2, 3, PB_LIN(0), PB_LIN(1), PB_HOD(0))                    \
    PB_SPEC(3, 3, PB_LIN(0), PB_LIN(1), PB_LIN(2))                    \
    PB_SPEC(3, 4, PB_LIN(0), PB_LIN(1), PB_LIN(2), PB_HOD(0))

struct BatchPrep {
    TracerDev tr[PB_MAXTR];
    int ntr, nt;
    double rho_m0;
    unsigned code;
};

struct PrepArgs {
    int nm, nblk;
    BatchPrep Q;
    const double *nzm, *bh, *ms, *wm;
    double *coef, *sidep;
};
__device__ __forceinline__ void batch_prep_tile(const PrepArgs& PA, int z, int blk) {
    const int nm = PA.nm, nblk = PA.nblk;
    const BatchPrep& Q = PA.Q;
    const double* __restrict__ nzm = PA.nzm;
    const double* __restrict__ bh = PA.bh;
    const double* __restrict__ ms = PA.ms;
    const double* __restrict__ wm = PA.wm;
    double* __restrict__ coef = PA.coef;
    double* __restrict__ sidep = PA.sidep;
    const int m = blk * 64 + (threadIdx.x & 63);
    const int nc1 = 1 + Q.nt;
    const int stride = pb_stride(Q.code, Q.ntr, nc1);
    double accC[PB_MAXTR], accB[PB_MAXTR];
    for (int t = 0; t < PB_MAXTR; ++t) accC[t] = accB[t] = 0.0;
    if (m < nm) {
        const size_t idx = (size_t)z * nm + m;
        const double mass = ms[m];
        const double wn = wm[m] * nzm[idx];
        const double wnb = wn * bh[idx];
        double* c = coef + idx * (size_t)stride;
        c[0] = wn;
        c[1] = wnb;
        int pos = 2;
        for (int t = 0; t < Q.ntr; ++t) {
            const TracerDev& T = Q.tr[t];
            double w[1 + PW_MAXT], a1[1 + PW_MAXT], a2[1 + PW_MAXT], low;
            tracer_form(T, idx, z, mass, Q.rho_m0, w, low);
            for (int i = 0; i <= PW_MAXT; ++i) { a1[i] = w[i]; a2[i] = w[i]; }
            if (T.kind == HMG_TRACER_HOD) {
                for (int i = 0; i <= PW_MAXT; ++i) a1[i] = a2[i] = 0.0;
                const double ng = T.ngal[z], ng2 = ng * ng;
                a1[1 + T.t_prof] = 1.0;
                const double cc = 2.0 * T.NcNs[idx] / ng2;
                if (T.t_cprof >= 0) a2[1 + T.t_cprof] += cc; else a2[0] += cc;
                a2[1 + T.t_prof] += T.NsNsm1[idx] / ng2;
                accB[t] = wnb * (T.Nc[idx] + T.Ns[idx]);
            }
            if (Q.code == 0) {
                double* ct = c + 2 + t * 3 * nc1;
                for (int i = 0; i < nc1; ++i) {
                    ct[i] = w[i];
                    ct[nc1 + i] = a1[i];
                    ct[2 * nc1 + i] = a2[i];
                }
            } else {
                const int sl = 1 + pb_slot(Q.code, t);
                if (pb_kind(Q.code, t) == 1) {
                    c[pos++] = w[sl];
                } else {
                    c[pos++] = w[0]; c[pos++] = w[sl]; c[pos++] = a2[0]; c[pos++] = a2[sl];
                }
            }
            accC[t] = wnb * low;
        }
        if (Q.code) for (; pos < stride; ++pos) c[pos] = 0.0;
    }
    for (int t = 0; t < Q.ntr; ++t) {
        const double C = wave_sum(accC[t]);
        const double B = wave_sum(accB[t]);
        if ((threadIdx.x & 63) == 0) {
            double* sp = sidep + ((size_t)(z * nblk + blk) * Q.ntr + t) * 2;
            sp[0] = B;
            sp[1] = C;
        }
    }
}
__device__ __forceinline__ void batch_prep_tile_compact(const PrepArgs& PA, int z, int blk) {
    const BatchPrep& Q = PA.Q;
    const int nm = PA.nm, lane = threadIdx.x & 63, m = blk * 64 + lane;
    int ncoef = 2;
#pragma unroll
    for (int t = 0; t < PB_MAXTR; ++t)
        if (t < Q.ntr) ncoef += Q.tr[t].kind == HMG_TRACER_HOD ? 4 : 1;
    const int stride = (ncoef + 7) & ~7;
    double accC[PB_MAXTR], accB[PB_MAXTR];
#pragma unroll
    for (int t = 0; t < PB_MAXTR; ++t) accC[t] = accB[t] = 0.0;
    if (m < nm) {
        const size_t idx = (size_t)z * nm + m;
        const double mass = PA.ms[m];
        const double wn = PA.wm[m] * PA.nzm[idx];
        const double wnb = wn * PA.bh[idx];
        double* __restrict__ c = PA.coef + idx * (size_t)stride;
        c[0] = wn;
        c[1] = wnb;
        int pos = 2;
#pragma unroll
        for (int t = 0; t < PB_MAXTR; ++t) {
            if (t >= Q.ntr) continue;
            const TracerDev& T = Q.tr[t];
            double low = 0.0;
            if (T.kind == HMG_TRACER_HOD) {
                const double ng = T.ngal[z], ng2 = ng * ng, nc = T.Nc[idx], ns = T.Ns[idx];
                c[pos] = nc / ng;
                c[pos + 1] = ns / ng;
                c[pos + 2] = 2.0 * T.NcNs[idx] / ng2;
                c[pos + 3] = T.NsNsm1[idx] / ng2;
                pos += 4;
                accB[t] = wnb * (nc + ns);
                low = (nc + ns) / ng;
            } else {
                low = T.kind == HMG_TRACER_MATTER ? mass / Q.rho_m0 : 0.0;
                c[pos++] = T.kind == HMG_TRACER_MATTER ? low : 1.0;
            }
            accC[t] = wnb * low;
        }
        for (; pos < stride; ++pos) c[pos] = 0.0;
    }
#pragma unroll
    for (int t = 0; t < PB_MAXTR; ++t) {
        if (t >= Q.ntr) continue;
        const double C = wave_sum(accC[t]);
        const double B = wave_sum(accB[t]);
        if (lane == 0) {
            double* sp = PA.sidep + ((size_t)(z * PA.nblk + blk) * Q.ntr + t) * 2;
            sp[0] = B;
            sp[1] = C;
        }
    }
}
__global__ __launch_bounds__(64) void power_batch_prep_kernel(PrepArgs PA) {
    if (PA.Q.code) batch_prep_tile_compact(PA, blockIdx.x, blockIdx.y);
    else batch_prep_tile(PA, blockIdx.x, blockIdx.y);
}

struct BatchArgs {
    const double* tens[PW_MAXT];
    const int* nconst[PW_MAXT];
    const double* cconst[PW_MAXT];
    const double* coef;
    const double* sidep;
    const double* ngal[PB_MAXTR];
    double bias_const[PB_MAXTR];
    int nblk;
    const double* ks;
    const double* Pzk;
    double* P1h[PB_MAXPAIR];
    double* P2h[PB_MAXPAIR];
    double kstar;
    int nm, nk;
};

constexpr int PB_NV = 16;

__device__ __forceinline__ double lane_value(double v, int l) {
    const int lo = __builtin_amdgcn_readlane(__double2loint(v), l), hi = __builtin_amdgcn_readlane(__double2hiint(v), l);
    return __hiloint2double(hi, lo);
}

template <int NT, int NTR, int V, bool W16, unsigned CODE = 0>
__global__ __launch_bounds__(W16 ? 1024 : 512) void power_batch_kernel(BatchArgs A) {
    extern __shared__ double red[];
    using vec_t = typename VecT<V>::type;
    static_assert(V == 1 || V == 2, "k-tile widths the deferred left fill was checked for");
    static_assert(HMG_PREFIX_TILE % (64 * V) == 0, "HMG_PREFIX_TILE must be a multiple of every k-tile width");
    constexpr int NC1 = 1 + NT;
    constexpr int STRIDE = pb_stride(CODE, NTR, NC1);
    constexpr int NPAIR = NTR * (NTR + 1) / 2;
    constexpr int NACC = NTR + NPAIR;
    const int lane = threadIdx.x & 63;
    const int wv = __builtin_amdgcn_readfirstlane(threadIdx.x >> 6);
    const int z = blockIdx.y;
    const int k0 = (blockIdx.x * 64 + lane) * V;
    const bool live = k0 < A.nk;
    double acc[NACC][V];
#pragma unroll
    for (int a = 0; a < NACC; ++a)
#pragma unroll
        for (int v = 0; v < V; ++v) acc[a][v] = 0.0;
    const size_t zrow = (size_t)z * A.nm;
    const int kend = min(A.nk, (int)(blockIdx.x + 1) * 64 * V);
    const size_t kofs = live ? (size_t)k0 : 0;
    const int L = (A.nm + PB_NV - 1) / PB_NV;
    const int NB = W16 ? L : 2 * L;
    auto bin = [&](int i) {
        if (W16) return wv + PB_NV * i;
        return i < L ? wv + PB_NV * i : wv + 8 + PB_NV * (i - L);
    };
    struct Hint { int n[NT]; double val[NT]; };
    auto load_hint = [&](Hint& h, int m) {
        const size_t r = zrow + min(m, A.nm - 1);
#pragma unroll
        for (int i = 0; i < NT; ++i) {
            h.n[i] = A.nconst[i] ? A.nconst[i][r] : -1;
            h.val[i] = A.nconst[i] ? A.cconst[i][r] : 0.0;
        }
    };
    auto fetch = [&](vec_t (&dst)[NT], int m, const Hint& h) {
        const size_t off = (zrow + min(m, A.nm - 1)) * (size_t)A.nk + kofs;
#pragma unroll
        for (int i = 0; i < NT; ++i) {
            if (h.n[i] >= kend) dst[i] = vsplat<V>(h.val[i]);
            else dst[i] = vload_nt<V>(A.tens[i] + off);
        }
    };
    auto park = [&]() {
#pragma unroll
        for (int a = 0; a < NACC; ++a)
#pragma unroll
            for (int v = 0; v < V; ++v) {
                red[((wv * NACC + a) * V + v) * 64 + lane] = acc[a][v];
                acc[a][v] = 0.0;
            }
    };
    auto accumulate = [&](const vec_t (&t)[NT], int i) {
        if (!W16 && i == L) park();
        const int m = bin(i);
        if (m >= A.nm) return;
        const double* __restrict__ c = A.coef + (zrow + m) * (size_t)STRIDE;
        const double wn = c[0], wnb = c[1];
#pragma unroll
        for (int v = 0; v < V; ++v) {
            double W[NTR], A1[NTR], A2[NTR];
            if constexpr (CODE != 0) {
                int pos = 2;
#pragma unroll
                for (int r = 0; r < NTR; ++r) {
                    const double ts = vget<V>(t[pb_slot(CODE, r)], v);
                    if (pb_kind(CODE, r) == 1) {
                        W[r] = c[pos] * ts;
                        A1[r] = W[r]; A2[r] = W[r];
                        pos += 1;
                    } else {
                        W[r] = fma(c[pos + 1], ts, c[pos]);
                        A1[r] = ts;
                        A2[r] = fma(c[pos + 3], ts, c[pos + 2]);
                        pos += 4;
                    }
                    acc[r][v] += wnb * W[r];
                }
            } else
#pragma unroll
            for (int r = 0; r < NTR; ++r) {
                const double* cr = c + 2 + r * 3 * NC1;
                double w = cr[0], a1 = cr[NC1], a2 = cr[2 * NC1];
#pragma unroll
                for (int i2 = 0; i2 < NT; ++i2) {
                    const double tv = vget<V>(t[i2], v);
                    w += cr[1 + i2] * tv;
                    a1 += cr[NC1 + 1 + i2] * tv;
                    a2 += cr[2 * NC1 + 1 + i2] * tv;
                }
                W[r] = w; A1[r] = a1; A2[r] = a2;
                acc[r][v] += wnb * w;
            }
            int p = NTR;
#pragma unroll
            for (int a = 0; a < NTR; ++a) {
                acc[p][v] += wn * (A1[a] * A2[a]);
                ++p;
#pragma unroll
                for (int b = a + 1; b < NTR; ++b) {
                    acc[p][v] += wn * (W[a] * W[b]);
                    ++p;
                }
            }
        }
    };
    int i = 0;
    vec_t ta[NT], tb[NT];
    Hint ha, hb;
    load_hint(ha, bin(0));
    load_hint(hb, bin(1));
    fetch(ta, bin(0), ha);
#pragma unroll 1
    for (; i + 1 < NB; i += 2) {
        fetch(tb, bin(i + 1), hb);
        load_hint(ha, bin(i + 2));
        __builtin_amdgcn_sched_barrier(0);
        accumulate(ta, i);
        __builtin_amdgcn_sched_barrier(0);
        fetch(ta, bin(i + 2), ha);
        load_hint(hb, bin(i + 3));
        __builtin_amdgcn_sched_barrier(0);
        accumulate(tb, i + 1);
        __builtin_amdgcn_sched_barrier(0);
    }
    if (i < NB) accumulate(ta, i);
    if (W16) {
        if (wv >= 8) {
#pragma unroll
            for (int a = 0; a < NACC; ++a)
#pragma unroll
                for (int v = 0; v < V; ++v) red[(((wv - 8) * NACC + a) * V + v) * 64 + lane] = acc[a][v];
        }
        __syncthreads();
    }
    if (wv < 8) {
#pragma unroll
        for (int a = 0; a < NACC; ++a)
#pragma unroll
            for (int v = 0; v < V; ++v) {
                const double other = red[((wv * NACC + a) * V + v) * 64 + lane];
                acc[a][v] = W16 ? acc[a][v] + other : other + acc[a][v];
            }
    }
    auto reduce = [&](double (&x)[V]) {
        __syncthreads();
        if (wv < 8) {
#pragma unroll
            for (int v = 0; v < V; ++v) red[(wv * V + v) * 64 + lane] = x[v];
        }
        __syncthreads();
        if (wv == 0) {
#pragma unroll
            for (int v = 0; v < V; ++v) {
                double sum = 0.0;
                for (int w = 0; w < 8; ++w) sum += red[(w * V + v) * 64 + lane];
                x[v] = sum;
            }
        }
    };
#pragma unroll
    for (int a = 0; a < NACC; ++a) reduce(acc[a]);
    if (wv == 0) {
        double kv[V], pl[V];
#pragma unroll
        for (int v = 0; v < V; ++v) {
            kv[v] = live ? A.ks[k0 + v] : 1.0;
            pl[v] = (live && A.Pzk) ? A.Pzk[(size_t)z * A.nk + k0 + v] : 0.0;
        }
        double* o1[NPAIR];
        double* o2[NPAIR];
#pragma unroll
        for (int p = 0; p < NPAIR; ++p) { o1[p] = A.P1h[p]; o2[p] = A.P2h[p]; }
        double bmc[NTR];
        {
            double Bs[NTR], Cs[NTR];
#pragma unroll
            for (int t = 0; t < NTR; ++t) Bs[t] = Cs[t] = 0.0;
            constexpr int CH = 64 / (2 * NTR);
            const double* __restrict__ spz = A.sidep + (size_t)z * A.nblk * (NTR * 2);
            for (int blk0 = 0; blk0 < A.nblk; blk0 += CH) {
                const int nb = min(CH, A.nblk - blk0);
                const double val = lane < nb * NTR * 2 ? spz[(size_t)blk0 * (NTR * 2) + lane] : 0.0;
                for (int b = 0; b < nb; ++b) {
#pragma unroll
                    for (int t = 0; t < NTR; ++t) {
                        Bs[t] += lane_value(val, (b * NTR + t) * 2);
                        Cs[t] += lane_value(val, (b * NTR + t) * 2 + 1);
                    }
                }
            }
#pragma unroll
            for (int t = 0; t < NTR; ++t) {
                const double bias = A.ngal[t] ? Bs[t] / A.ngal[t][z] : A.bias_const[t];
                bmc[t] = bias - Cs[t];
            }
        }
        if (live) {
#pragma unroll
            for (int v = 0; v < V; ++v) {
                const int k = k0 + v;
                const size_t o = (size_t)z * A.nk + k;
                const double q = kv[v] / A.kstar;
                const double damp = 1.0 - exp(-(q * q));
                const double plin = pl[v];
                int p = 0;
#pragma unroll
                for (int a = 0; a < NTR; ++a) {
#pragma unroll
                    for (int b = a; b < NTR; ++b) {
                        if (o1[p]) o1[p][o] = acc[NTR + p][v] * damp;
                        if (o2[p]) o2[p][o] = plin * ((acc[a][v] + bmc[a]) * (acc[b][v] + bmc[b]));
                        ++p;
                    }
                }
            }
        }
    }
}

}
```

hmvec_amd/csrc/runtime.hip:

```cpp
#include <algorithm>
#include <cmath>
#include <cstdlib>
#include <cstring>

#include "hmctx.hpp"

using namespace hmg;

thread_local std::string g_last_error;

int fail(const char* what, const char* detail, const char* file, int line) {
    char buf[512];
    snprintf(buf, sizeof(buf), "%s: %s (%s:%d)", what, detail, file, line);
    g_last_error = buf;
    return 1;
}

static int rocfft_refcount = 0;

int event_at(hmg_ctx* c, int slot, hipEvent_t* out) {
    if (!c->ev[slot]) HIP_TRY(hipEventCreate(&c->ev[slot]));
    *out = c->ev[slot];
    return 0;
}
// ... 181 lines not shown
    c->block_bytes.erase(it);
    return 0;
}
int hmg_host_alloc(hmg_ctx* c, size_t bytes, void** h_out) {
    REQUIRE(c && h_out, "NULL argument");
    HIP_TRY(hipSetDevice(c->device));
    HIP_TRY(hipHostMalloc(h_out, bytes ? bytes : 8, hipHostMallocDefault));
    return 0;
}
int hmg_host_free(hmg_ctx* c, void* h) {
    REQUIRE(c, "NULL ctx");
    if (h) HIP_TRY(hipHostFree(h));
    return 0;
}
int hmg_memcpy_d2h_async(hmg_ctx* c, void* h_pinned, const void* d, size_t bytes) {
    REQUIRE(c && h_pinned && d, "NULL argument");
    HIP_TRY(hipMemcpyAsync(h_pinned, d, bytes, hipMemcpyDeviceToHost, c->stream));
    return 0;
}
int hmg_memcpy_h2d_async(hmg_ctx* c, void* d, const void* h_pinned, size_t bytes) {
    REQUIRE(c && h_pinned && d, "NULL argument");
    HIP_TRY(hipMemcpyAsync(d, h_pinned, bytes, hipMemcpyHostToDevice, c->stream));
    return 0;
}
int hmg_event_synchronize(hmg_ctx* c, int slot) {
    REQUIRE(c && slot >= 0 && slot < HMG_EVENT_SLOTS, "bad event slot");
    REQUIRE(!c->capturing, "hmg_event_synchronize inside a captured step");
    REQUIRE(c->ev[slot] != nullptr, "event slot was never recorded");
    HIP_TRY(hipEventSynchronize(c->ev[slot]));
    return check_fault(c);
}
constexpr size_t PIN_CHUNK = (size_t)8 << 20;

static int ensure_pinned(hmg_ctx* c) {
    for (int i = 0; i < 2; ++i) {
        if (!c->pinned[i]) HIP_TRY(hipHostMalloc(&c->pinned[i], PIN_CHUNK, hipHostMallocDefault));
        if (!c->pin_ev[i]) HIP_TRY(hipEventCreateWithFlags(&c->pin_ev[i], hipEventDisableTiming));
    }
    return 0;
}

int hmg_memcpy_h2d(hmg_ctx* c, void* d, const void* h, size_t bytes) {
    REQUIRE(c && d && h, "NULL argument");
    if (bytes <= hmg_ctx::UP_SLOT_BYTES && !c->capturing && !c->lanes_dirty && c->stream == c->lanes[0]) {
        if (!c->up_ring) {
            HIP_TRY(hipHostMalloc((void**)&c->up_ring, hmg_ctx::UP_SLOTS * hmg_ctx::UP_SLOT_BYTES, hipHostMallocDefault));
            for (int i = 0; i < hmg_ctx::UP_SLOTS; ++i)
                HIP_TRY(hipEventCreateWithFlags(&c->up_ev[i], hipEventDisableTiming));
        }
        const int slot = c->up_next;
        c->up_next = (c->up_next + 1) % hmg_ctx::UP_SLOTS;
        HIP_TRY(hipEventSynchronize(c->up_ev[slot]));
        char* stage = c->up_ring + (size_t)slot * hmg_ctx::UP_SLOT_BYTES;
        memcpy(stage, h, bytes);
        HIP_TRY(hipMemcpyAsync(d, stage, bytes, hipMemcpyHostToDevice, c->stream));
        HIP_TRY(hipEventRecord(c->up_ev[slot], c->stream));
        return 0;
    }
    if (bytes < (256u << 10)) {
        HIP_TRY(hipMemcpyAsync(d, h, bytes, hipMemcpyHostToDevice, c->stream));
        HIP_TRY(hipStreamSynchronize(c->stream));
        return 0;
    }
    if (ensure_pinned(c)) return 1;
    size_t done = 0;
    int b = 0;
    while (done < bytes) {
        const size_t n = bytes - done < PIN_CHUNK ? bytes - done : PIN_CHUNK;
        HIP_TRY(hipEventSynchronize(c->pin_ev[b]));
        memcpy(c->pinned[b], (const char*)h + done, n);
        HIP_TRY(hipMemcpyAsync((char*)d + done, c->pinned[b], n, hipMemcpyHostToDevice, c->stream));
        HIP_TRY(hipEventRecord(c->pin_ev[b], c->stream));
        done += n;
        b ^= 1;
    }
    HIP_TRY(hipStreamSynchronize(c->stream));
    return 0;
}
int hmg_memcpy_d2h(hmg_ctx* c, void* h, const void* d, size_t bytes) {
    REQUIRE(c && d && h, "NULL argument");
    REQUIRE(!c->capturing, "hmg_memcpy_d2h inside a captured step");
    if (c->lanes_dirty && sync_all(c)) return 1;
    if (bytes < (256u << 10)) {
        HIP_TRY(hipMemcpyAsync(h, d, bytes, hipMemcpyDeviceToHost, c->stream));
        HIP_TRY(hipStreamSynchronize(c->stream));
        return check_fault(c);
    }
    if (ensure_pinned(c)) return 1;
    size_t issued = 0, copied = 0;
    size_t len[2] = {0, 0};
    int bi = 0, bo = 0;
    while (copied < bytes) {
        while (issued < bytes && issued - copied < 2 * PIN_CHUNK && len[bi] == 0) {
            const size_t n = bytes - issued < PIN_CHUNK ? bytes - issued : PIN_CHUNK;
            HIP_TRY(hipMemcpyAsync(c->pinned[bi], (const char*)d + issued, n, hipMemcpyDeviceToHost, c->stream));
            HIP_TRY(hipEventRecord(c->pin_ev[bi], c->stream));
            len[bi] = n;
            issued += n;
            bi ^= 1;
        }
        HIP_TRY(hipEventSynchronize(c->pin_ev[bo]));
        memcpy((char*)h + copied, c->pinned[bo], len[bo]);
        copied += len[bo];
        len[bo] = 0;
        bo ^= 1;
    }
    return check_fault(c);
}
int hmg_memcpy_d2d(hmg_ctx* c, void* dst, const void* src, size_t bytes) {
    REQUIRE(c && dst && src, "NULL argument");
    HIP_TRY(hipMemcpyAsync(dst, src, bytes, hipMemcpyDeviceToDevice, c->stream));
    return 0;
}
int hmg_sync(hmg_ctx* c) {
    REQUIRE(c, "NULL ctx");
    return sync_all(c);
}
int hmg_lane_set(hmg_ctx* c, int lane) {
    REQUIRE(c && lane >= 0 && lane < HMG_LANES, "bad lane");
    if (lane != 0) c->lanes_dirty = true;
    c->lane = lane;
    c->stream = c->lanes[lane];
    return 0;
}
int hmg_event_wait(hmg_ctx* c, int slot) {
    REQUIRE(c && slot >= 0 && slot < HMG_EVENT_SLOTS, "bad event slot");
    if (!c->ev[slot]) return 0;
    HIP_TRY(hipStreamWaitEvent(c->stream, c->ev[slot], 0));
    return 0;
}
int hmg_event_record(hmg_ctx* c, int slot) {
    REQUIRE(c && slot >= 0 && slot < HMG_EVENT_SLOTS, "bad event slot");
    hipEvent_t e;
    if (event_at(c, slot, &e)) return 1;
    HIP_TRY(hipEventRecord(e, c->stream));
    return 0;
}
int hmg_elapsed_ms(hmg_ctx* c, int s0, int s1, double* ms) {
    REQUIRE(c && ms && s0 >= 0 && s0 < HMG_EVENT_SLOTS && s1 >= 0 && s1 < HMG_EVENT_SLOTS, "bad event slot");
    REQUIRE(c->ev[s0] && c->ev[s1], "event slot was never recorded");
    HIP_TRY(hipEventSynchronize(c->ev[s1]));
    float f = 0.f;
    HIP_TRY(hipEventElapsedTime(&f, c->ev[s0], c->ev[s1]));
    *ms = (double)f;
    return 0;
}

int hmg_graph_begin(hmg_ctx* c) {
    REQUIRE(c, "NULL ctx");
    REQUIRE(!c->capturing, "already capturing");
    REQUIRE(c->lane == 0, "start a capture on lane 0");
    HIP_TRY(hipStreamBeginCapture(c->lanes[0], hipStreamCaptureModeRelaxed));
    c->capturing = true;
    return 0;
}
static void release_deferred_frees(hmg_ctx* c) {
    std::vector<void*> v;
    v.swap(c->freed_in_capture);
    for (void* p : v) (void)hmg_free(c, p);
}
int hmg_graph_end(hmg_ctx* c, int* id) {
    REQUIRE(c && id, "NULL argument");
    REQUIRE(c->capturing, "no capture in progress");
    c->capturing = false;
    c->lane = 0;
    c->stream = c->lanes[0];
    hipGraph_t g = nullptr;
    HIP_TRY(hipStreamEndCapture(c->lanes[0], &g));
    int nkern = 0;
    {
        size_t nn = 0;
        if (hipGraphGetNodes(g, nullptr, &nn) == hipSuccess && nn) {
            std::vector<hipGraphNode_t> nodes(nn);
            if (hipGraphGetNodes(g, nodes.data(), &nn) == hipSuccess)
                for (size_t i = 0; i < nn; ++i) {
                    hipGraphNodeType t;
                    if (hipGraphNodeGetType(nodes[i], &t) == hipSuccess && t == hipGraphNodeTypeKernel) ++nkern;
                }
        }
    }
    hipGraphExec_t ge = nullptr;
    hipError_t e = hipGraphInstantiate(&ge, g, nullptr, nullptr, 0);
    (void)hipGraphDestroy(g);
    if (e != hipSuccess) { release_deferred_frees(c); c->prefix_capture.clear(); }
    HIP_TRY(e);
    *id = c->next_graph_id++;
    c->graphs[*id] = ge;
    c->graph_kernels[*id] = nkern;
    c->graph_blocks[*id].swap(c->freed_in_capture);
    c->graph_prefix[*id].swap(c->prefix_capture);
    c->prefix_capture.clear();
    return 0;
}
int hmg_graph_kernel_nodes(hmg_ctx* c, int id, int* n) {
    REQUIRE(c && n, "NULL argument");
    auto it = c->graph_kernels.find(id);
    REQUIRE(it != c->graph_kernels.end(), "unknown graph id");
    *n = it->second;
    return 0;
}
int hmg_graph_abort(hmg_ctx* c) {
    REQUIRE(c, "NULL ctx");
    if (!c->capturing) return 0;
    c->capturing = false;
    release_deferred_frees(c);
    c->prefix_capture.clear();
    c->lane = 0;
    c->stream = c->lanes[0];
    hipGraph_t g = nullptr;
    (void)hipStreamEndCapture(c->lanes[0], &g);
    if (g) (void)hipGraphDestroy(g);
    (void)hipGetLastError();
    return 0;
}
int hmg_graph_launch(hmg_ctx* c, int id) {
    REQUIRE(c, "NULL ctx");
    REQUIRE(!c->capturing, "cannot replay a graph inside a capture");
    auto it = c->graphs.find(id);
    REQUIRE(it != c->graphs.end(), "unknown graph id");
    HIP_TRY(hipGraphLaunch(it->second, c->stream));
    auto gp = c->graph_prefix.find(id);
    if (gp != c->graph_prefix.end()) prefix_replayed(c, gp->second);
    return 0;
}
int hmg_graph_destroy(hmg_ctx* c, int id) {
    REQUIRE(c, "NULL ctx");
    auto it = c->graphs.find(id);
    if (it == c->graphs.end()) return 0;
    if (sync_all(c)) return 1;
    HIP_TRY(hipGraphExecDestroy(it->second));
    c->graphs.erase(it);
    c->graph_prefix.erase(id);
    auto gb = c->graph_blocks.find(id);
    if (gb != c->graph_blocks.end()) {
        for (void* p : gb->second) (void)hmg_free(c, p);
        c->graph_blocks.erase(gb);
    }
    return 0;
}

int hmg_bracket_next(hmg_ctx* c, int kernel_id, int s0, int s1) {
    REQUIRE(c && kernel_id >= 0 && kernel_id < HMG_KERNEL_COUNT, "bad kernel id");
    REQUIRE(s0 >= -1 && s0 < HMG_EVENT_SLOTS && s1 >= -1 && s1 < HMG_EVENT_SLOTS, "bad event slot");
    c->bracket[kernel_id][0] = s0;
    c->bracket[kernel_id][1] = s1;
    return 0;
}

int bracket_open(hmg_ctx* c, int kid, int* stop_slot) {
    *stop_slot = -1;
    const int s0 = c->bracket[kid][0], s1 = c->bracket[kid][1];
    c->bracket[kid][0] = c->bracket[kid][1] = -1;
    if (s0 >= 0) {
        hipEvent_t e;
        if (event_at(c, s0, &e)) return 1;
        HIP_TRY(hipEventRecord(e, c->stream));
    }
    *stop_slot = s1;
    return 0;
}
int bracket_close(hmg_ctx* c, int stop_slot) {
    if (stop_slot >= 0) {
        hipEvent_t e;
        if (event_at(c, stop_slot, &e)) return 1;
        HIP_TRY(hipEventRecord(e, c->stream));
    }
    return 0;
}
```

hmvec_amd/halomodel.py:

```python
import ctypes as C
import itertools
import os
from collections import namedtuple
from collections.abc import MutableMapping

import numpy as np
import scipy.constants as constants

from . import _native as nat
from . import realspace, spectra, stages
from .cosmology import Cosmology, _is_shared_product, sigma2_kgrid, sigma2_weights
from .params import battaglia_defaults, default_params
from .quadrature import gradient_is_uniform, simpson_weights, trapz_weights
from .functions import FN_BG_INTEGRAND, FN_ST_FSIGMA, FN_TINKER_FSIGMA, fn2d, ngal_from_mthresh, trapz_lastaxis
from .functions import context as fn_context
from .utils import vectorized_bisection_search

_trapz = getattr(np, "trapezoid", None) or np.trapz
_EPOCHS = itertools.count(1)
_DATA = os.path.join(os.path.dirname(os.path.abspath(__file__)), "data")
_Spectra = namedtuple("_Spectra", "version p1h p2h host i1h i2h", defaults=(None, None, None))


def _tinker_alpha_table():
    with np.load(os.path.join(_DATA, "tinker10_alpha_of_z.npz")) as f:
        return f["z"], f["alpha"]


class DeviceDict(MutableMapping):

    def __init__(self, ctx_getter, on_change=None):
        self._ctx_getter = ctx_getter
        self._on_change = on_change or (lambda: None)
        self._dev = {}
        self._host = {}
        self._hint = {}

    def dev(self, name, fill=True):
        d = self._dev[name]
        if fill and name in self._hint:
            self._ctx_getter().call("hmg_prefix_fill", d.ptr)
        return d

    def on_device(self, name, shape):
        d = self._dev.get(name)
        return d is not None and d.shape == tuple(shape)

    def _pending(self, name):
        if name not in self._hint:
            return False
        ctx = self._ctx_getter()
        n = C.c_int()
        nat.check(ctx.lib.hmg_prefix_pending(ctx.handle, self._dev[name].ptr, C.byref(n)))
        return bool(n.value)

    def hint(self, name):
        return self._hint.get(name, (None, None))

    def set_dev(self, name, darr, hint=None):
        self._dev[name] = darr
        self._host.pop(name, None)
        if hint is None:
            self._hint.pop(name, None)
        else:
            self._hint[name] = hint
        self._on_change()

    def __getitem__(self, name):
        if name in self._host and self._pending(name):
            del self._host[name]
        if name not in self._host:
            self._host[name] = self.dev(name).numpy()
        return self._host[name]

    def __setitem__(self, name, value):
        if isinstance(value, nat.DeviceArray):
            self.set_dev(name, value)
        else:
            self.set_dev(name, self._ctx_getter().upload(np.asarray(value, dtype=np.float64)))

    def __delitem__(self, name):
        del self._dev[name]
        self._host.pop(name, None)
        self._hint.pop(name, None)
        self._on_change()

    def __contains__(self, name):
        return name in self._dev

    def __iter__(self):
        return iter(self._dev)

    def __len__(self):
        return len(self._dev)


class HodEntry(MutableMapping):

    _ARR = ("Nc", "Ns", "NsNsm1", "NcNs", "ngal", "bg")

    def __init__(self, dev, meta):
        self.dev = dev
        self._vals = dict(meta)

    def __getitem__(self, k):
        if k not in self._vals:
            self._vals[k] = self.dev[k].numpy()
        return self._vals[k]

    def __setitem__(self, k, v):
        self._vals[k] = v

    def __delitem__(self, k):
        self._vals.pop(k, None)
        self.dev.pop(k, None)

    def __contains__(self, k):
        return k in self._vals or k in self.dev

    def __iter__(self):
        seen = list(self.dev) + [k for k in self._vals if k not in self.dev]
        return iter(seen)

    def __len__(self):
        return len(set(self.dev) | set(self._vals))


def _R_from_M(M, rho, delta):
    return (3.0 * M / 4.0 / np.pi / delta / rho) ** (1.0 / 3.0)


class HaloModel(Cosmology):
    def __init__(self, zs, ks, ms=None, params={}, mass_function="sheth-torman",
                 halofit=None, mdef="vir", nfw_numeric=False, skip_nfw=False, accuracy="medium",
                 engine="camb", *, device=0, ctx=None, background=None):
        self.zs = np.asarray(zs, dtype=np.float64)
        self.ks = np.asarray(ks, dtype=np.float64)
        self._device = device
        self.ctx = ctx
        self.ms = self._ms_key = self._sync_serial = self._rho_m0_val = None
        self._version = self._epoch = self._nq = 0
        self._aux_pending = self._m200c_valid = False
        Cosmology.__init__(self, params, halofit, engine=engine, accuracy=accuracy, background=background)

        self.mdef = mdef
        self.mode = mass_function
        self.hods = {}
        self._dcache = {}
        self._pool = {}
        self._use_lanes = os.environ.get("HMG_LANES", "0") == "1"
        self._groups = os.environ.get("HMG_NO_GROUPS", "0") != "1" and not self._use_lanes
        self._stages = []
        self._stage_dims = None
        self.prefix_deferral = os.environ.get("HMG_NO_PREFIX_DEFERRAL", "0") != "1"

        self._pcache = {}
        self.uk_profiles = DeviceDict(self._ctx, self._bump)
        self.pk_profiles = DeviceDict(self._ctx, self._bump)

        if ms is not None:
            self.ms = np.asarray(ms, dtype=np.float64)
            self.init_mass_function(self.ms)

        if not skip_nfw:
            self.add_nfw_profile("nfw", numeric=nfw_numeric)

    def _init_cosmology(self, params, halofit):
        Cosmology._init_cosmology(self, params, halofit)
        if self.accuracy == "low":
            self.Pzk = self.P_lin_approx(self.ks, self.zs)
        else:
            self.Pzk = self._get_matter_power(self.zs, self.ks, nonlinear=False)
        if halofit is not None:
            self.nPzk = self._get_matter_power(self.zs, self.ks, nonlinear=True)

    def deltav(self, z):
        x = self.omz(z) - 1.0
        return 18.0 * np.pi ** 2.0 + 82.0 * x - 39.0 * x ** 2.0

    def _mdef_delta_rho(self):
        if self.mdef == "vir":
            return self.deltav(self.zs), self.rho_critical_z(self.zs)
        if self.mdef == "mean":
            return 200.0 + 0.0 * self.zs, self.rho_matter_z(self.zs)
        raise NotImplementedError(self.mdef)

    def rvir(self, m, z):
        if self.mdef == "vir":
            return _R_from_M(m, self.rho_critical_z(z), delta=self.deltav(z))
        elif self.mdef == "mean":
            return _R_from_M(m, self.rho_matter_z(z), delta=200.0)

    def R_of_m(self, ms):
        return _R_from_M(ms, self.rho_matter_z(0), delta=1.0)

    def _bump(self):
        self._version += 1

    def _release_inputs(self, keys):
        if self._stages:
            self._ctx().flush()
        for k in keys:
            self._dcache.pop(k, None)

    def _dev(self, key, builder):
        if key not in self._dcache:
            self._dcache[key] = self._ctx().upload(builder())
        return self._dcache[key]

    _AUX = 1
    _EV_SYNC, _EV_AUX = 0, 1

    def _sync_point(self):
        if self._use_lanes:
            ctx = self._ctx()
            ctx.lane(0)
            ctx.record(self._EV_SYNC)
            self._sync_serial = ctx.capture_serial

    def _aux(self):
        ctx = self._ctx()
        if self._use_lanes:
            if self._sync_serial != ctx.capture_serial:
                self._sync_point()
            ctx.lane(self._AUX)
            ctx.wait(self._EV_SYNC)
        return ctx

    def _aux_done(self):
        if self._use_lanes:
            ctx = self._ctx()
            ctx.record(self._EV_AUX)
            self._aux_pending = True
            ctx.lane(0)

    def _main(self, needs_aux=False):
        ctx = self._ctx()
        if self._use_lanes:
            ctx.lane(0)
            if needs_aux and self._aux_pending:
                ctx.wait(self._EV_AUX)
        return ctx

    def _buf(self, key, shape):
        shape = tuple(int(x) for x in shape)
        b = self._pool.get(key)
        if b is None or b.shape != shape:
            if b is not None:
                self._ctx().flush()
            b = self._ctx().empty(shape)
            self._pool[key] = b
        return b

    @property
    def _nz(self):
        return self.zs.size

    @property
    def _nm(self):
        return self.ms.size

    @property
    def _nk(self):
        return self.ks.size

    def _d_zs(self):
        return self._dev("zs", lambda: self.zs)

    def _d_ks(self):
        return self._dev("ks", lambda: self.ks)

    def _d_ms(self):
        return self._dev("ms", lambda: self.ms)

    def _d_wm(self):
        return self._dev("wm", lambda: trapz_weights(self.ms))

    def _d_Pzk(self):
        return self._dev("Pzk", lambda: self.Pzk)

    def _lazy_host(self, name):
        h = "_h_" + name
        if getattr(self, h, None) is None:
            setattr(self, h, getattr(self, "_d_" + name).numpy())
        return getattr(self, h)

    sigma2 = property(lambda self: self._lazy_host("sigma2"))
    nzm = property(lambda self: self._lazy_host("nzm"))
    bh = property(lambda self: self._lazy_host("bh"))

    def _stage(self, kind, part, keep=()):
        ctx = self._ctx()
        dims = (self._nz, self._nm if self.ms is not None else 0, self._nk, self._nq)
        if not self._groups:
            ctx.flush()
            return self._issue(ctx.call, [stages.alone(kind, part, dims)])
        if stages.must_issue_first([st[0] for st in self._stages], self._stage_dims, kind, dims):
            ctx.flush()
        self._stage_dims = dims
        self._stages.append((kind, part, keep))
        ctx.defer(self)

    def _drop_queue(self):
        self._stages = []

    def _issue(self, call, launches):
        for entry, args, tagged in launches:
            if not tagged:
                call(entry, *args)
                continue
            call("hmg_profile_support_epoch", self._epoch)
            call("hmg_prefix_deferral", int(self.prefix_deferral))
            try:
                call(entry, *args)
            finally:
                call("hmg_prefix_deferral", 0)
                call("hmg_profile_support_epoch", 0)

    def _ks_ascending(self):
        if "ks_ascending" not in self._dcache:
            self._dcache["ks_ascending"] = (bool(np.all(np.diff(self.ks) > 0))
                                            and os.environ.get("HMG_NO_HINTS", "0") != "1")
        return self._dcache["ks_ascending"]

    def _flush(self, prep=None):
        queued, self._stages = self._stages, []
        launches, prepared = stages.plan(queued, self._stage_dims, prep, os.environ.get("HMG_X", ""))
        self._issue(self._ctx().call_now, launches)
        return prepared

    def get_sigma2(self):
        return self.sigma2

    def _tinker_z_params(self):
        zs = self.zs
        zc = zs * np.heaviside(3 - zs, 0) + 3 * np.heaviside(zs - 3, 0)
        tz, ta = _tinker_alpha_table()
        if np.any(zc < tz[0]) or np.any(zc > tz[-1]):
            raise ValueError("A value in x_new is outside the interpolation range.")
        alpha = np.interp(zc, tz, ta)
        beta = 0.589 * (1 + zc) ** 0.20
        phi = -0.729 * (1 + zc) ** (-0.08)
        eta = -0.243 * (1 + zc) ** 0.27
        gamma = 0.864 * (1 + zc) ** (-0.01)
        return np.stack([alpha, beta, phi, eta, gamma], axis=1)

    def init_mass_function(self, ms):
        ms = np.asarray(ms, dtype=np.float64)
        if self._ms_key is None or not np.array_equal(ms, self._ms_key):
            self._release_inputs([k for k in self._dcache if k != "zs" and k != "ks" and k != "Pzk"
                                  and not (isinstance(k, tuple) and k[0] == "fftgrid")])
            self._ms_key = ms.copy()
            self._epoch = next(_EPOCHS)
        self.ms = ms
        self._bump()
        if self.mode not in ("sheth-torman", "tinker"):
            raise NotImplementedError
        if self.mdef not in ("vir", "mean"):
            raise NotImplementedError
        ctx = self._ctx()
        nz, nm = self._nz, self._nm
        self._h_sigma2 = self._h_nzm = self._h_bh = None
        if "sig_in" not in self._dcache:
            kmin, kmax, numks = self.p["sigma2_kmin"], self.p["sigma2_kmax"], self.p["sigma2_numks"]
            kq = sigma2_kgrid(kmin, kmax, numks)
            if self.accuracy == "high":
                self.sPzk = self.P_lin_slow(kq, self.zs, kmax=kmax)
            elif self.accuracy == "medium":
                self.sPzk = self.P_lin(kq, self.zs)
            else:
                self.sPzk = self._P_lin_approx_shared(kq, self.zs)
            wq = sigma2_weights(kq)
            owned = _is_shared_product(self.sPzk)
            shared = ctx.shared.get(id(self.sPzk)) if owned else None
            if shared is None or shared[0] is not self.sPzk:
                d_sP = ctx.upload(self.sPzk)
                n = C.c_size_t()
                nat.check(ctx.lib.hmg_sigma2_layout_size(nz, kq.size, C.byref(n)))
                d_PT = ctx.empty((n.value,))
                ctx.call("hmg_sigma2_prepare", nz, kq.size, d_sP.ptr, d_PT.ptr)
                shared = (self.sPzk, d_PT, ctx.upload(kq), ctx.upload(wq))
                if owned:
                    if len(ctx.shared) >= 4:
                        ctx.flush()
                        ctx.shared.clear()
                    ctx.shared[id(self.sPzk)] = shared
            self._dcache["sig_in"] = shared[1:] + (ctx.upload(self.R_of_m(ms)),)
        d_PT, d_kq, d_wq, d_R = self._dcache["sig_in"]
        self._sync_point()
        ctx = self._aux()
        self._d_sigma2 = self._buf("sigma2", (nz, nm))
        if "mf_in" not in self._dcache:
            lnm = np.log(ms)
            uniform, step = gradient_is_uniform(lnm)
            par = nat.MassFnParams(
                mode=nat.MF_SHETH_TORMEN if self.mode == "sheth-torman" else nat.MF_TINKER10,
                deltac=self.p["st_deltac"], st_A=self.p["st_A"], st_a=self.p["st_a"], st_p=self.p["st_p"],
                rho_m0=float(self.rho_matter_z(0)[0]), lnm_uniform=int(uniform), lnm_step=step)
            d_tz = ctx.upload(self._tinker_z_params()) if self.mode == "tinker" else None
            delta, rho = self._mdef_delta_rho()
            self._dcache["mf_in"] = (par, ctx.upload(lnm), d_tz, ctx.upload(delta), ctx.upload(rho))
            ctx = self._aux()
        par, d_lnm, d_tz, d_delta, d_rho = self._dcache["mf_in"]
        self._d_nzm, self._d_bh = self._buf("nzm", (nz, nm)), self._buf("bh", (nz, nm))
        d_ms = self._d_ms()
        self._d_cs, self._d_rvir, self._d_rs = (self._buf(k, (nz, nm)) for k in ("cs", "rvir", "rs"))
        self._d_nfw_series = self._buf("nfw_series", (nz, nm, nat.NFW_SERIES_STRIDE))
        m2, r2, d_drho1, d_rhoc = self._m200c_io()
        duffy = tuple(float(self.p[f"duffy_{k}_{self.mdef}"]) for k in ("A", "alpha", "beta"))
        halo = nat.HaloStageArgs(self._d_zs().ptr, d_delta.ptr, d_rho.ptr, *duffy, float(self.h),
                                 self._d_cs.ptr, self._d_rvir.ptr, self._d_rs.ptr, self._d_nfw_series.ptr,
                                 d_drho1.ptr, 200.0, d_rhoc.ptr, m2.ptr, r2.ptr)
        massfn = nat.MassFnPart(C.pointer(par), d_ms.ptr, d_lnm.ptr, nat.ptr(d_tz), self._d_sigma2.ptr, self._d_nzm.ptr, self._d_bh.ptr)
        front = stages.FrontArgs((nz, nm, d_kq.size, d_PT.ptr, d_kq.ptr, d_wq.ptr, d_R.ptr,
                                  float(self.p["Wkr_taylor_switch"])), d_ms.ptr, halo)
        if self._groups:
            self._nq = int(d_kq.size)
            self._stage("front", front)
            self._stage("massfn", massfn, keep=(par,))
        elif not self._use_lanes:
            ctx.call("hmg_sigma2_massfn_halo", *front.sigma2, *stages.fields(massfn), C.byref(halo))
        else:
            ctx.call("hmg_sigma2_massfn", *front.sigma2, *stages.fields(massfn))
            self._aux_done()
            ctx = self._main()
            ctx.call("hmg_halo_stage", nz, nm, d_ms.ptr, *stages.fields(halo))
        self._m200c_valid = True

    def get_fsigmaz(self):
        dc = self.p["st_deltac"]
        with fn_context(self._ctx()):
            if self.mode == "sheth-torman":
                return fn2d(FN_ST_FSIGMA, [self.sigma2], [self.p["st_A"], self.p["st_a"], self.p["st_p"], dc])
            if self.mode == "tinker":
                tz, ta = _tinker_alpha_table()
                return fn2d(FN_TINKER_FSIGMA, [self.sigma2, self.zs[:, None]], [1.0, 0.368, float(tz.size), dc],
                            tables=(tz, ta))
        raise NotImplementedError

    def get_bh(self):
        return self.bh

    def get_nzm(self):
        return self.nzm

    def concentration(self, mode="duffy"):
        if mode != "duffy":
            raise NotImplementedError
        return self._d_cs.numpy()

    def _m200c_io(self):
        return (self._buf("m200c", (self._nz, self._nm)), self._buf("r200c", (self._nz, self._nm)), self._d_drho1(),
                self._dev("rhocz", lambda: self.rho_critical_z(self.zs)))

    def _m200c(self):
        m2, r2, d1, d_rhoc = self._m200c_io()
        if not self._m200c_valid:
            self._ctx().call("hmg_mdelta_convert", self._nz, self._nm, self._d_ms().ptr, self._d_cs.ptr, d1.ptr, 200.0,
                             d_rhoc.ptr, m2.ptr, r2.ptr)
            self._m200c_valid = True
        return m2, r2

    def _d_drho1(self):
        def drho1():
            delta, rho = self._mdef_delta_rho()
            return rho * delta if self.mdef == "vir" else rho * 200.0
        return self._dev("drho1", drho1)

    def _fft_grids(self, xmax, nxs):
        key = ("fftgrid", float(xmax), int(nxs))
        if key not in self._dcache:
            xs = np.linspace(0.0, xmax, nxs + 1)[1:]
            step = (xs[-1] - xs[0]) / xs.size
            kts = np.fft.rfftfreq(xs.size, step) * 2 * np.pi
            ctx = self._ctx()
            d_xs = ctx.upload(xs)
            d_lx = ctx.empty((xs.size,))
            ctx.call("hmg_profile_fft_logx", xs.size, d_xs.ptr, d_lx.ptr)
            self._dcache[key] = (d_xs, ctx.upload(kts), float(step), d_lx)
        return self._dcache[key]

    def _profile_fft(self, key, nxs, xmax, rowp, consts, gamma, d_cmax, d_rss, do_mass_norm, d_post=None, d_rowsc=None):
        nz, nm, nk = self._nz, self._nm, self._nk
        d_xs, d_kts, step, d_lx = self._fft_grids(xmax, nxs)
        out = self._buf(key, (nz, nm, nk))
        hint = ((self._buf((key, "nconst"), ((nz * nm + 1) // 2,)), self._buf((key, "cconst"), (nz, nm)))
                if self._ks_ascending() else None)
        self._stage("fft", nat.ProfileFftPart(
            int(nxs), step, d_xs.ptr, d_kts.ptr, *(nat.ptr(r) for r in rowp), *(float(c) for c in consts), float(gamma),
            d_cmax.ptr, d_rss.ptr, self._d_zs().ptr, self._d_ks().ptr, int(do_mass_norm), nat.ptr(d_post), out.ptr,
            nat.ptr(hint[0] if hint else None), nat.ptr(hint[1] if hint else None), d_lx.ptr,
            nat.ptr(d_rowsc if hint else None)))
        return out, hint

    def _battaglia_rowparams(self, key, kind, fit9, gamma, alpha_const, pref, post_pref, nxs=None, xmax=None):
        nz, nm = self._nz, self._nm
        outs = [self._buf((key, "rowp", i), (nz, nm)) for i in range(7)]
        fit = (C.c_double * 9)(*fit9)
        d_hz = self._dev("hz", lambda: self.h_of_z(self.zs))
        m200c, r200c, d_drho1, d_rhoc = self._m200c_io()
        if not self._m200c_valid:
            self._ctx().call("hmg_profile_rows_from_mvir", kind, nz, nm, self._d_ms().ptr, self._d_cs.ptr,
                             self._d_rvir.ptr, self._d_zs().ptr, d_drho1.ptr, 200.0, d_rhoc.ptr, d_hz.ptr,
                             C.byref(fit), float(gamma), float(alpha_const), float(pref), float(post_pref),
                             m200c.ptr, r200c.ptr, *[o.ptr for o in outs])
            self._m200c_valid = True
            return outs, None
        d_rowsc, extra = None, (None, None, 0, 0, None)
        if (self._groups and nxs is not None and nxs % 2 == 0 and os.environ.get("HMG_NO_ROWSC", "0") != "1"
                and self._ks_ascending()):
            d_kts = self._fft_grids(xmax, nxs)[1]
            d_rowsc = self._buf((key, "rowsc"), (nz, nm, nat.ROWSC_STRIDE))
            extra = (self._d_ks().ptr, d_kts.ptr, self._nk, int(nxs) // 2, d_rowsc.ptr)
        self._stage("rows", nat.RowsPart(kind, m200c.ptr, r200c.ptr, self._d_rvir.ptr, self._d_zs().ptr, d_rhoc.ptr,
                                         d_hz.ptr, fit, float(gamma), float(alpha_const), float(pref),
                                         float(post_pref), *[o.ptr for o in outs], *extra))
        return outs, d_rowsc

    def add_battaglia_profile(self, name, family=None, param_override=None, nxs=None, xmax=None,
                              ignore_existing=False):
        if not (ignore_existing):
            assert name not in self.uk_profiles.keys(), "Profile name already exists."
        assert name != "nfw", "Name nfw is reserved."
        if nxs is None:
            nxs = self.p["electron_density_profile_integral_numxs"]
        if xmax is None:
            xmax = self.p["electron_density_profile_integral_xmax"]
        if family is None:
            family = self.p["battaglia_gas_family"]
        pparams = {"battaglia_gas_gamma": self.p["battaglia_gas_gamma"]}
        pparams.update(battaglia_defaults[family])
        if param_override is not None:
            print(param_override)
            for key in param_override.keys():
                if key == "battaglia_gas_gamma" or key in battaglia_defaults[family]:
                    pparams[key] = param_override[key]
        omb = self.p["ombh2"] / self.h ** 2.0
        gamma = pparams["battaglia_gas_gamma"]
        fit9 = [pparams[a + b] for a in ("rho0_", "alpha_", "beta_") for b in ("A0", "alpham", "alphaz")]
        key = ("uk", name)
        self._main()
        (amp, xc, alpha, expo, cmax, rscale, _post), rowsc = self._battaglia_rowparams(
            key, nat.PROF_BATTAGLIA_GAS, fit9, gamma, 0.0, omb / self.omm0, 0.0, nxs=nxs, xmax=xmax)
        out, hint = self._profile_fft(key, nxs, xmax, (amp, None, alpha, expo), (0.0, 1.0, 0.0, 0.0), gamma,
                                      cmax, rscale, True, d_rowsc=rowsc)
        self.uk_profiles.set_dev(name, out, hint)

    def add_battaglia_pres_profile(self, name, family=None, param_override=None, nxs=None, xmax=None,
                                   ignore_existing=False):
        if not (ignore_existing):
            assert name not in self.pk_profiles.keys(), "Profile name already exists."
        assert name != "nfw", "Name nfw is reserved."
        if nxs is None:
            nxs = self.p["electron_pressure_profile_integral_numxs"]
        if xmax is None:
            xmax = self.p["electron_pressure_profile_integral_xmax"]
        if family is None:
# ... 685 lines not shown
```

include/hmgrid.h:

```cpp
#ifndef HMGRID_H
#define HMGRID_H

#include <stddef.h>

#ifdef __cplusplus
extern "C" {
#endif

#define HMG_ABI_VERSION 10

typedef struct hmg_ctx hmg_ctx;

int         hmg_abi_version(void);
const char* hmg_last_error(void);
int hmg_ctx_create(int device, hmg_ctx** out);
int hmg_ctx_destroy(hmg_ctx* ctx);
int hmg_malloc(hmg_ctx* ctx, size_t bytes, void** d_out);
int hmg_free(hmg_ctx* ctx, void* d_ptr);
int hmg_memcpy_h2d(hmg_ctx* ctx, void* d_dst, const void* h_src, size_t bytes);
int hmg_memcpy_d2h(hmg_ctx* ctx, void* h_dst, const void* d_src, size_t bytes);
int hmg_memcpy_d2d(hmg_ctx* ctx, void* d_dst, const void* d_src, size_t bytes);
int hmg_sync(hmg_ctx* ctx);
int hmg_host_alloc(hmg_ctx* ctx, size_t bytes, void** h_out);
int hmg_host_free(hmg_ctx* ctx, void* h_ptr);
int hmg_memcpy_d2h_async(hmg_ctx* ctx, void* h_pinned_dst, const void* d_src, size_t bytes);
int hmg_memcpy_h2d_async(hmg_ctx* ctx, void* d_dst, const void* h_pinned_src, size_t bytes);
int hmg_event_synchronize(hmg_ctx* ctx, int slot);
#define HMG_LANES 4
int hmg_lane_set(hmg_ctx* ctx, int lane);
int hmg_event_wait(hmg_ctx* ctx, int slot);
#define HMG_EVENT_SLOTS 4096
int hmg_event_record(hmg_ctx* ctx, int slot);
int hmg_elapsed_ms(hmg_ctx* ctx, int slot_start, int slot_stop, double* h_ms);
#define HMG_KERNEL_POWER       0
#define HMG_KERNEL_NFW         1
#define HMG_KERNEL_PROFILE_FFT 2
#define HMG_KERNEL_COUNT       3
int hmg_bracket_next(hmg_ctx* ctx, int kernel_id, int slot_start, int slot_stop);
int hmg_graph_begin(hmg_ctx* ctx);
int hmg_graph_end(hmg_ctx* ctx, int* h_graph_id);
int hmg_graph_abort(hmg_ctx* ctx);
int hmg_graph_kernel_nodes(hmg_ctx* ctx, int graph_id, int* h_n);
int hmg_graph_launch(hmg_ctx* ctx, int graph_id);
int hmg_graph_destroy(hmg_ctx* ctx, int graph_id);

int hmg_sigma2(hmg_ctx* ctx, int nz, int nm, int nq,
               const double* d_sPzk , const double* d_kq ,
               const double* d_wq , const double* d_R ,
               double taylor_switch, double* d_sigma2 );
int hmg_sigma2_layout_size(int nz, int nq, size_t* h_doubles);
int hmg_sigma2_prepare(hmg_ctx* ctx, int nz, int nq, const double* d_sPzk, double* d_PT);
int hmg_sigma2_prepared(hmg_ctx* ctx, int nz, int nm, int nq, const double* d_PT,
                        const double* d_kq, const double* d_wq, const double* d_R,
                        double taylor_switch, double* d_sigma2);

#define HMG_MF_SHETH_TORMEN 0
#define HMG_MF_TINKER10     1
typedef struct {
    int    mode;
    double deltac, st_A, st_a, st_p;
    double rho_m0;
    int    lnm_uniform;
    double lnm_step;
} hmg_massfn_params;
int hmg_massfn(hmg_ctx* ctx, int nz, int nm, const hmg_massfn_params* h_par,
               const double* d_sigma2 , const double* d_ms ,
               const double* d_lnms ,
               const double* d_tinker_z ,
               double* d_nzm , double* d_bh );

int hmg_sigma2_massfn(hmg_ctx* ctx, int nz, int nm, int nq, const double* d_PT,
                      const double* d_kq, const double* d_wq, const double* d_R, double taylor_switch,
                      const hmg_massfn_params* h_par, const double* d_ms, const double* d_lnms,
                      const double* d_tinker_z, double* d_sigma2, double* d_nzm, double* d_bh);

int hmg_halo_structure(hmg_ctx* ctx, int nz, int nm, const double* d_ms, const double* d_zs,
                       const double* d_delta , const double* d_rho ,
                       double duffy_A, double duffy_alpha, double duffy_beta, double h,
                       double* d_cs , double* d_rvir ,
                       double* d_rs );

#define HMG_NFW_SERIES_STRIDE 36
int hmg_halo_stage(hmg_ctx* ctx, int nz, int nm, const double* d_ms, const double* d_zs,
                   const double* d_delta , const double* d_rho ,
                   double duffy_A, double duffy_alpha, double duffy_beta, double h,
                   double* d_cs, double* d_rvir, double* d_rs, double* d_nfw_series,
                   const double* d_drho1 , double delta2, const double* d_rho2 ,
                   double* d_m2, double* d_r2);

typedef struct {
    const double *d_zs, *d_delta , *d_rho ;
    double duffy_A, duffy_alpha, duffy_beta, h;
    double *d_cs, *d_rvir, *d_rs, *d_nfw_series ;
    const double* d_drho1 ;
    double delta2;
    const double* d_rho2 ;
    double *d_m2, *d_r2 ;
} hmg_halo_stage_args;
int hmg_sigma2_massfn_halo(hmg_ctx* ctx, int nz, int nm, int nq, const double* d_PT,
                           const double* d_kq, const double* d_wq, const double* d_R, double taylor_switch,
                           const hmg_massfn_params* h_par, const double* d_ms, const double* d_lnms,
                           const double* d_tinker_z, double* d_sigma2, double* d_nzm, double* d_bh,
                           const hmg_halo_stage_args* h_halo);

int hmg_mdelta_convert(hmg_ctx* ctx, int nz, int nm, const double* d_ms, const double* d_cs,
                       const double* d_drho1 , double delta2, const double* d_rho2 ,
                       double* d_m2 , double* d_r2 );

int hmg_nfw_analytic(hmg_ctx* ctx, int nz, int nm, int nk, const double* d_cs,
                     const double* d_rs, const double* d_zs, const double* d_ks,
                     const double* d_nfw_series ,
                     double* d_uk );

#define HMG_PROF_BATTAGLIA_GAS  1
#define HMG_PROF_BATTAGLIA_PRES 2
int hmg_profile_rowparams(hmg_ctx* ctx, int kind, int nz, int nm, const double* d_m200c,
                          const double* d_r200c, const double* d_rvir, const double* d_zs,
                          const double* d_rhocz , const double* d_hz ,
                          const double h_fit[9], double gamma, double alpha_const,
                          double amp_prefactor, double post_prefactor,
                          double* d_amp, double* d_xc, double* d_alpha, double* d_expo,
                          double* d_cmax , double* d_rscale ,
                          double* d_post );

int hmg_profile_rows_from_mvir(hmg_ctx* ctx, int kind, int nz, int nm, const double* d_ms,
                               const double* d_cs, const double* d_rvir, const double* d_zs,
                               const double* d_drho1 , double delta2,
                               const double* d_rhocz , const double* d_hz ,
                               const double h_fit[9], double gamma, double alpha_const,
                               double amp_prefactor, double post_prefactor,
                               double* d_m200c, double* d_r200c,
                               double* d_amp, double* d_xc, double* d_alpha, double* d_expo,
                               double* d_cmax, double* d_rscale, double* d_post);

int hmg_profile_fft(hmg_ctx* ctx, int nz, int nm, int nk, int nxs, double fft_step,
                    const double* d_xs, const double* d_kts,
                    const double* d_amp, const double* d_xc, const double* d_alpha,
                    const double* d_expo, double amp_const, double xc_const,
                    double alpha_const, double expo_const, double gamma,
                    const double* d_cmax , const double* d_rss ,
                    const double* d_zs, const double* d_ks, int do_mass_norm,
                    const double* d_post ,
                    double* d_out ,
                    int* d_nconst , double* d_cconst ,
                    const double* d_logxs );
int hmg_profile_support_epoch(hmg_ctx* ctx, long long epoch);
int hmg_profile_fft_logx(hmg_ctx* ctx, int nxs, const double* d_xs, double* d_logxs);

#define HMG_PREFIX_TILE 128
int hmg_prefix_deferral(hmg_ctx* ctx, int on);
int hmg_prefix_fill(hmg_ctx* ctx, double* d_out);
int hmg_prefix_pending(hmg_ctx* ctx, const double* d_out, int* pending);
int hmg_prefix_fill_rows(hmg_ctx* ctx, double* d_out, const int* d_nconst, const double* d_cconst, int rows, int nk);

typedef struct {
    double sig_log_mstellar, alphasat, Bsat, betasat, Bcut, betacut;
    int    corr;
} hmg_hod_params;
int hmg_hod(hmg_ctx* ctx, int nz, int nm, const hmg_hod_params* h_par, const double* d_zs,
            const double* d_ms, const double* d_log10mstar_thresh ,
            const double* d_nzm, const double* d_bh, const double* d_wm ,
            double* d_Nc, double* d_Ns, double* d_NsNsm1, double* d_NcNs ,
            double* d_ngal , double* d_bg );

#define HMG_TRACER_MATTER   0
#define HMG_TRACER_HOD      1
#define HMG_TRACER_PRESSURE 2
typedef struct {
    int kind;
    const double* d_prof;
    const double* d_cprof;
    const double *d_Nc, *d_Ns, *d_NcNs, *d_NsNsm1, *d_ngal;
    const double* d_bias_override;
    const int*    d_prof_nconst;   const double* d_prof_cconst;
    const int*    d_cprof_nconst;  const double* d_cprof_cconst;
} hmg_tracer;
int hmg_power(hmg_ctx* ctx, int nz, int nm, int nk, const hmg_tracer* h_a, const hmg_tracer* h_b,
              const double* d_nzm, const double* d_bh, const double* d_ms, const double* d_wm,
              const double* d_ks, const double* d_Pzk, double rho_m0, double kstar,
              double* d_P1h , double* d_P2h );

int hmg_power_2halo_terms(hmg_ctx* ctx, int nz, int nm, int nk, const hmg_tracer* h_a, const hmg_tracer* h_b,
                          const double* d_nzm, const double* d_bh, const double* d_ms, const double* d_wm,
                          const double* d_ks, double rho_m0,
                          double* d_I1 , double* d_I2 , double* d_C12 );

int hmg_power_batch(hmg_ctx* ctx, int nz, int nm, int nk, int ntr, const hmg_tracer* h_tr,
                    int npairs, const int* h_pair_a, const int* h_pair_b,
                    const double* d_nzm, const double* d_bh, const double* d_ms, const double* d_wm,
                    const double* d_ks, const double* d_Pzk, double rho_m0, double kstar,
                    double* const* h_P1h, double* const* h_P2h);

typedef struct {
    const hmg_massfn_params* h_par;
    const double *d_ms, *d_lnms, *d_tinker_z;
    double *d_sigma2, *d_nzm, *d_bh;
} hmg_massfn_part;
#define HMG_HOD_ALL         0
#define HMG_HOD_OCCUPATIONS 1
#define HMG_HOD_SUMS        2
typedef struct {
    int stage;
    const hmg_hod_params* h_par;
    const double *d_zs, *d_ms, *d_log10mstar_thresh, *d_nzm, *d_bh, *d_wm;
    double *d_Nc, *d_Ns, *d_NsNsm1, *d_NcNs, *d_ngal, *d_bg;
} hmg_hod_part;
typedef struct {
    int kind;
    const double *d_m200c, *d_r200c, *d_rvir, *d_zs, *d_rhocz, *d_hz;
    double fit[9], gamma, alpha_const, amp_prefactor, post_prefactor;
    double *d_amp, *d_xc, *d_alpha, *d_expo, *d_cmax, *d_rscale, *d_post;
    const double *d_ks, *d_kts;
    int nk, fft_m;
    double* d_rowsc;
} hmg_rows_part;
#define HMG_ROWSC_STRIDE 8
typedef struct {
    const double *d_cs, *d_rs, *d_zs, *d_ks, *d_nfw_series;
    double* d_uk;
} hmg_nfw_part;
typedef struct {
    int nxs;
    double fft_step;
    const double *d_xs, *d_kts, *d_amp, *d_xc, *d_alpha, *d_expo;
    double amp_const, xc_const, alpha_const, expo_const, gamma;
    const double *d_cmax, *d_rss, *d_zs, *d_ks;
    int do_mass_norm;
    const double* d_post;
    double* d_out;
    int* d_nconst;
    double* d_cconst;
    const double* d_logxs;
    const double* d_rowsc;
} hmg_profile_fft_part;
typedef struct {
    int ntr;
    const hmg_tracer* h_tr;
    int npairs;
    const int *h_pair_a, *h_pair_b;
    const double *d_nzm, *d_bh, *d_ms, *d_wm, *d_ks, *d_Pzk;
    double rho_m0, kstar;
    double* const* h_P1h;
    double* const* h_P2h;
} hmg_power_batch_desc;
int hmg_sigma2_halo_front(hmg_ctx* ctx, int nz, int nm, int nq, const double* d_PT, const double* d_kq,
                          const double* d_wq, const double* d_R, double taylor_switch,
                          const double* d_ms, const hmg_halo_stage_args* h_halo,
                          const hmg_hod_part* h_hod_occupations ,
                          const hmg_rows_part* h_rows );
int hmg_group_rows(hmg_ctx* ctx, int nz, int nm, int nk, int nq, const hmg_massfn_part* h_massfn,
                   const hmg_hod_part* h_hod, const hmg_rows_part* h_rows, const hmg_nfw_part* h_nfw);
int hmg_group_profile(hmg_ctx* ctx, int nz, int nm, int nk, const hmg_profile_fft_part* h_fft,
                      const hmg_hod_part* h_hod, const hmg_power_batch_desc* h_prep);
int hmg_group_tensors(hmg_ctx* ctx, int nz, int nm, int nk, int nq, const hmg_massfn_part* h_massfn ,
                      const hmg_hod_part* h_hod , const hmg_power_batch_desc* h_prep ,
                      const hmg_nfw_part* h_nfw , const hmg_profile_fft_part* h_fft);
#define HMG_PB_PREPARED 1
int hmg_power_batch_run(hmg_ctx* ctx, int nz, int nm, int nk, const hmg_power_batch_desc* h_desc, int flags);

int hmg_add(hmg_ctx* ctx, size_t n, const double* d_a, const double* d_b, double* d_out);

int hmg_limber(hmg_ctx* ctx, int nells, const double* d_ells, int nz, int nk, const double* d_zs,
               const double* d_ks, const double* d_Pzk,
               const double* d_Pzk2 ,
               int ngz, const double* d_gzs,
               const double* d_pref, const double* d_chis, const double* d_wz, double* d_out);

#define HMG_FN_TINKER_BIAS    0
#define HMG_FN_TINKER_FNU     1
#define HMG_FN_MHALO_STELLAR  2
#define HMG_FN_HOD_NC         3
#define HMG_FN_HOD_NS         4
#define HMG_FN_HOD_MFUNC      5
#define HMG_FN_HOD_NSNSM1     6
#define HMG_FN_HOD_NCNS       7
#define HMG_FN_FCON           8
#define HMG_FN_RHO_NFW        9
#define HMG_FN_R_FROM_M      10
#define HMG_FN_DUFFY         11
#define HMG_FN_BATT_FIT      12
#define HMG_FN_RHO_GAS_X     13
#define HMG_FN_RHO_GAS_R     14
#define HMG_FN_PE_X          15
#define HMG_FN_PE_R          16
#define HMG_FN_NGAL_INTEGRAND 17
#define HMG_FN_A2Z           18
#define HMG_FN_MDELTA        19
#define HMG_FN_BG_INTEGRAND  20
#define HMG_FN_ST_FSIGMA     21
#define HMG_FN_TINKER_FSIGMA 22
#define HMG_FN_WKR           23
#define HMG_FN_LINCOMB3      24
#define HMG_FN_MHALO_STELLAR_CORE 25
#define HMG_FN_BRUTE_INTEGRAND 26
#define HMG_FN_COUNT         27
#define HMG_FN_MAXIN   6
#define HMG_FN_MAXPAR 16
int hmg_fn2d(hmg_ctx* ctx, int op, int rows, int cols, int nin, const double* const* h_d_in,
             const int* h_sr, const int* h_sc, const double* h_par, int npar, double* d_out);

int hmg_mstellar_halo(hmg_ctx* ctx, int nz, int nm, const double* d_zs, const double* d_log10mhalo,
                      double* d_out);

int hmg_trapz_rows(hmg_ctx* ctx, int rows, int cols, const double* d_y, const double* d_x, double* d_out);

int hmg_sine_transform(hmg_ctx* ctx, int rows, int n, const double* d_x, const double* d_y, double* d_uk);
// ... 70 lines not shown
```

Baseline: 864.5 billion.

## Skip power-batch tensor loads and accumulation for negligible-weight mass rows

The fused mass-function row kernel now records, per (z,m), whether the exponent in the mass-function exponential is at least 88. Such rows have weights near exp(-88) and are marked weightless. A host-side registry keyed by the nzm buffer hands these flags to the power-batch kernel. There they replace tensor loads with splats and skip the accumulation for those rows, cutting memory traffic and FMAs. This brings a slight numerical approximation, plus serial-based invalidation bookkeeping to keep the flags consistent across graph captures.

```diff
diff --git a/hmvec_amd/_native.py b/hmvec_amd/_native.py
--- a/hmvec_amd/_native.py
+++ b/hmvec_amd/_native.py
@@ -151,6 +151,7 @@
     "hmg_prefix_fill": [_P, _P],
     "hmg_prefix_pending": [_P, _P, C.POINTER(_I)],
     "hmg_prefix_fill_rows": [_P, _P, _P, _P, _I, _I],
+    "hmg_row_flags": [_P, _P, _P],
     "hmg_hod": [_P, _I, _I, C.POINTER(HodParams), _P, _P, _P, _P, _P, _P, _P, _P, _P, _P, _P, _P],
     "hmg_power": [_P, _I, _I, _I, C.POINTER(Tracer), C.POINTER(Tracer), _P, _P, _P, _P, _P, _P,
                   _D, _D, _P, _P],
@@ -407,7 +408,7 @@
         check(self.lib.hmg_elapsed_ms(self.handle, s0, s1, C.byref(ms)))
         return ms.value
 
-    _NO_FLUSH = frozenset(["hmg_bracket_next", "hmg_profile_support_epoch", "hmg_prefix_deferral"])
+    _NO_FLUSH = frozenset(["hmg_bracket_next", "hmg_profile_support_epoch", "hmg_prefix_deferral", "hmg_row_flags"])
 
     def call(self, name, *args):
         if name not in self._NO_FLUSH:
diff --git a/hmvec_amd/csrc/hmctx.hpp b/hmvec_amd/csrc/hmctx.hpp
--- a/hmvec_amd/csrc/hmctx.hpp
+++ b/hmvec_amd/csrc/hmctx.hpp
@@ -83,6 +83,11 @@
     bool pending = false;
 };
 
+struct RowFlags {
+    int* wl = nullptr;
+    long valid = 0;
+};
+
 struct hmg_ctx {
     int device = 0;
     hipStream_t stream = nullptr;
@@ -135,6 +140,8 @@
     std::map<int, hipGraphExec_t> graphs;
     std::map<int, int> graph_kernels;
     int next_graph_id = 1;
+    std::map<const void*, RowFlags> row_flags;
+    long flags_serial = 1;
     int prefix_deferral = 0;
     std::map<void*, PrefixEntry> prefix;
     std::map<void*, PrefixEntry> prefix_capture;
@@ -163,5 +170,10 @@
 static inline void prefix_drop_block(hmg_ctx* c, void* p, size_t bytes) {
     auto lo = c->prefix.lower_bound(p), hi = c->prefix.lower_bound((char*)p + bytes);
     c->prefix.erase(lo, hi);
+    for (auto it = c->row_flags.begin(); it != c->row_flags.end();) {
+        const char *k = (const char*)it->first, *v = (const char*)it->second.wl, *b = (const char*)p;
+        if ((k >= b && k < b + bytes) || (v >= b && v < b + bytes)) it = c->row_flags.erase(it);
+        else ++it;
+    }
 }
 static inline dim3 grid1d(size_t n, int block) { return dim3((unsigned)((n + block - 1) / block)); }
diff --git a/hmvec_amd/csrc/hmgrid.hip b/hmvec_amd/csrc/hmgrid.hip
--- a/hmvec_amd/csrc/hmgrid.hip
+++ b/hmvec_amd/csrc/hmgrid.hip
@@ -442,9 +442,12 @@
             const NfwArgs& N = R.N ? *R.N : none;
             const size_t nfw_blocks = R.N ? R.nfw_blocks : 0;
             REQUIRE((size_t)rows + R.nchain + nfw_blocks <= 2147483647u, "bad grid");
-            return launch_lds(tensor_group_kernel<B, P, M>, dim3((unsigned)(rows + R.nchain + nfw_blocks)), dim3(FUSED_NT),
-                              lds, c->stream, C, A, R.nchain, rows, N.T, N.acoef, N.ktile, N.nm, N.nk, N.cs, N.rss, N.zs,
-                              N.ks, N.uk);
+            const dim3 grid((unsigned)(rows + R.nchain + nfw_blocks));
+            if (C.has_mf && C.S.wl)
+                return launch_lds(tensor_group_kernel<B, P, M, true>, grid, dim3(FUSED_NT), lds, c->stream, C, A, R.nchain, rows,
+                                  N.T, N.acoef, N.ktile, N.nm, N.nk, N.cs, N.rss, N.zs, N.ks, N.uk);
+            return launch_lds(tensor_group_kernel<B, P, M, false>, grid, dim3(FUSED_NT), lds, c->stream, C, A, R.nchain, rows,
+                              N.T, N.acoef, N.ktile, N.nm, N.nk, N.cs, N.rss, N.zs, N.ks, N.uk);
         } else {
             REQUIRE(false, "internal: the tensor group is compiled for compile-time plans only");
         }
@@ -722,6 +725,13 @@
     return 0;
 }
 
+int hmg_row_flags(hmg_ctx* c, const double* nzm, int* weightless) {
+    REQUIRE(c && nzm, "NULL argument");
+    if (weightless) c->row_flags[nzm] = RowFlags{weightless, 0};
+    else c->row_flags.erase(nzm);
+    return 0;
+}
+
 int hmg_prefix_pending(hmg_ctx* c, const double* out, int* pending) {
     REQUIRE(c && out && pending, "NULL argument");
     REQUIRE(!c->capturing, "the pending state is what replays make it: ask outside the captured step");
@@ -889,7 +899,8 @@
     const size_t lds = (size_t)8 * NACC * V * 64 * sizeof(double);
     int stop = -1;
     if (bracket_open(c, HMG_KERNEL_POWER, &stop)) return 1;
-    if (launch_lds(power_batch_kernel<NT, NTR, V, W16, CODE>, grid, dim3(W16 ? 1024 : 512), lds, c->stream, A)) return 1;
+    if (A.wl ? launch_lds(power_batch_kernel<NT, NTR, V, W16, CODE, true>, grid, dim3(W16 ? 1024 : 512), lds, c->stream, A)
+             : launch_lds(power_batch_kernel<NT, NTR, V, W16, CODE, false>, grid, dim3(W16 ? 1024 : 512), lds, c->stream, A)) return 1;
     return bracket_close(c, stop);
 }
 
@@ -980,6 +991,7 @@
         A.nconst[i] = nullptr;
         A.cconst[i] = nullptr;
     }
+    A.wl = nullptr;
     for (int t = 0; t < ntr; ++t) {
         const int sp = Q.tr[t].t_prof, sc = Q.tr[t].t_cprof;
         REQUIRE((tr[t].d_prof_nconst == nullptr) == (tr[t].d_prof_cconst == nullptr) &&
@@ -1041,9 +1053,19 @@
     return fail("hmg_power_batch", "unreachable", __FILE__, __LINE__);
 }
 
+static int* pb_row_flags(hmg_ctx* c, const PbPlan& P, const double* nzm) {
+    if (P.thin != 0) return nullptr;
+    auto rf = c->row_flags.find(nzm);
+    return rf == c->row_flags.end() ? nullptr : rf->second.wl;
+}
+
 int hmg_power_batch_run(hmg_ctx* c, int nz, int nm, int nk, const hmg_power_batch_desc* d, int flags) {
     PbPlan P;
     if (pb_plan(c, nz, nm, nk, d, &P)) return 1;
+    {
+        auto rf = c->row_flags.find(d->d_nzm);
+        if (rf != c->row_flags.end() && rf->second.valid == c->flags_serial) P.A.wl = pb_row_flags(c, P, d->d_nzm);
+    }
     if (!(flags & HMG_PB_PREPARED)) {
         hipLaunchKernelGGL(power_batch_prep_kernel, dim3(nz, P.PA.nblk), dim3(64), 0, c->stream, P.PA);
         HIP_TRY(hipGetLastError());
@@ -1147,7 +1169,9 @@
             "no sigma^2 partial sums of this shape in the context: call hmg_sigma2_halo_front first");
     const int nseg = (nq + SIG_SEG_LEN - 1) / SIG_SEG_LEN;
     *S = SigmaMassFnArgs{nz, nm, nseg, P, (const double*)c->scratch[4], mf->d_ms, mf->d_lnms, mf->d_tinker_z,
-                         mf->d_sigma2, mf->d_nzm, mf->d_bh};
+                         mf->d_sigma2, mf->d_nzm, mf->d_bh, nullptr};
+    auto rf = c->row_flags.find(mf->d_nzm);
+    if (rf != c->row_flags.end()) rf->second.valid = 0;
     return 0;
 }
 
@@ -1259,6 +1283,10 @@
         if (massfn_setup(c, nz, nm, nq, mf, &C.S)) return 1;
         C.has_mf = 1;
         one = 1;
+        if (C.has_prep && prep->d_nzm == mf->d_nzm) {
+            C.S.wl = pb_row_flags(c, P, mf->d_nzm);
+            if (C.S.wl) c->row_flags[mf->d_nzm].valid = c->flags_serial;
+        }
     }
     NfwArgs N{};
     size_t nfw_blocks = 0;
diff --git a/hmvec_amd/csrc/kernels/groups.hpp b/hmvec_amd/csrc/kernels/groups.hpp
--- a/hmvec_amd/csrc/kernels/groups.hpp
+++ b/hmvec_amd/csrc/kernels/groups.hpp
@@ -72,10 +72,10 @@
     for (unsigned i = 0; i < sizeof(T) / 8; ++i) u.w[i] = q[i];
     return u.v;
 }
-template <int NT, bool MF = false>
+template <int NT, bool MF = false, bool WL = false>
 __device__ __forceinline__ void chain_row(const ChainArgs& C, int z, double* lds) {
     if (MF && C.has_mf) {
-        massfn_row<NT>(C.S, z, lds);
+        massfn_row<NT, WL>(C.S, z, lds);
         __threadfence_block();
         __syncthreads();
     }
@@ -147,7 +147,7 @@
     profile_fused_row<512, MAXB, MAXP, SPECM, false, true>(A, row_order(b - nchain, A.nm), smem);
 }
 
-template <int MAXB, int MAXP, int SPECM>
+template <int MAXB, int MAXP, int SPECM, bool WL>
 __global__ __launch_bounds__(512, (fused_occ<MAXB, SPECM>())) void tensor_group_kernel(
     ChainArgs C, FusedArgs A, int nchain, int nprof, const SiciTable* __restrict__ T, const double* __restrict__ acoef,
     int ktile, int nm, int nk, const double* __restrict__ cs, const double* __restrict__ rss,
@@ -155,7 +155,7 @@
     extern __shared__ __attribute__((aligned(16))) double smem[];
     int b = blockIdx.x;
     if (b < nchain) {
-        chain_row<512, true>(C, b, smem);
+        chain_row<512, true, WL>(C, b, smem);
         return;
     }
     b -= nchain;
diff --git a/hmvec_amd/csrc/kernels/massfn.hpp b/hmvec_amd/csrc/kernels/massfn.hpp
--- a/hmvec_amd/csrc/kernels/massfn.hpp
+++ b/hmvec_amd/csrc/kernels/massfn.hpp
@@ -20,25 +20,34 @@
     return 1.0 - A * nua / (nua + pow(dc, a)) + 0.183 * pow(nu, 1.5) + C * pow(nu, 2.4);
 }
 
+#ifndef HMG_ROW_E_CUT
+#define HMG_ROW_E_CUT 88.0
+#endif
+__device__ __forceinline__ bool row_weightless(double E ) {
+    return E >= HMG_ROW_E_CUT;
+}
+
 template <class SigmaAt>
 __device__ __forceinline__ void massfn_point(const MassFnDev& P, int z, int m, int nm, SigmaAt S,
                                              const double* __restrict__ ms, const double* __restrict__ lnm,
-                                             const double* __restrict__ tz, double& n_out, double& b_out) {
+                                             const double* __restrict__ tz, double& n_out, double& b_out, double& e_out) {
     const double sig2 = S(m);
     const double dc = P.deltac;
     double f, b;
     if (P.mode == HMG_MF_SHETH_TORMEN) {
         const double sig = sqrt(sig2);
-        f = P.A * sqrt(2.0 * P.a / M_PI) * (1.0 + pow(sig2 / P.a / (dc * dc), P.p)) * (dc / sig) *
-            exp(-P.a * (dc * dc) / 2.0 / sig2);
+        const double E = P.a * (dc * dc) / 2.0 / sig2;
+        f = P.A * sqrt(2.0 * P.a / M_PI) * (1.0 + pow(sig2 / P.a / (dc * dc), P.p)) * (dc / sig) * exp(-E);
+        e_out = E;
         const double t = P.a * (dc * dc) / sig2;
         b = 1.0 + (1.0 / dc) * (t - 1.0) + (2.0 * P.p / dc) / (1.0 + pow(t, P.p));
     } else {
         const double nu = dc / sqrt(sig2);
         const double al = tz[z * 5 + 0], be = tz[z * 5 + 1], ph = tz[z * 5 + 2], et = tz[z * 5 + 3],
                      ga = tz[z * 5 + 4];
-        const double fnu = al * ((1.0 + pow(be * nu, -2.0 * ph)) * pow(nu, 2.0 * et) *
-                                 exp(-ga * (nu * nu) / 2.0));
+        const double E = ga * (nu * nu) / 2.0;
+        const double fnu = al * ((1.0 + pow(be * nu, -2.0 * ph)) * pow(nu, 2.0 * et) * exp(-E));
+        e_out = E;
         f = nu * fnu;
         b = tinker10_bias(nu);
     }
@@ -70,8 +79,8 @@
     if (idx >= nz * nm) return;
     const int z = idx / nm, m = idx - z * nm;
     const double* row = s2 + (size_t)z * nm;
-    double n, b;
-    massfn_point(P, z, m, nm, [&](int i) { return row[i]; }, ms, lnm, tz, n, b);
+    double n, b, e;
+    massfn_point(P, z, m, nm, [&](int i) { return row[i]; }, ms, lnm, tz, n, b, e);
     nzm[idx] = n;
     bh[idx] = b;
 }
@@ -81,6 +90,7 @@
     MassFnDev P;
     const double *partial , *ms, *lnm, *tz;
     double *s2, *nzm, *bh;
+    int* wl;
 };
 __device__ __forceinline__ void sigma2_massfn_block(const SigmaMassFnArgs& A, int z, int m0, double (*red)[66],
                                                     double* sig) {
@@ -102,8 +112,8 @@
     __syncthreads();
     const int m = m0 + threadIdx.x;
     if (threadIdx.x < 64 && m < nm) {
-        double nn, bb;
-        massfn_point(A.P, z, m, nm, [&](int i) { return sig[i - m0 + 1]; }, A.ms, A.lnm, A.tz, nn, bb);
+        double nn, bb, ee;
+        massfn_point(A.P, z, m, nm, [&](int i) { return sig[i - m0 + 1]; }, A.ms, A.lnm, A.tz, nn, bb, ee);
         A.nzm[(size_t)z * nm + m] = nn;
         A.bh[(size_t)z * nm + m] = bb;
     }
@@ -131,14 +141,14 @@
     __syncthreads();
     const int m = m0 + (int)threadIdx.x;
     if (threadIdx.x < MF_TILE && m < nm) {
-        double nn, bb;
-        massfn_point(A.P, z, m, nm, [&](int i) { return sig[i - m0 + 1]; }, A.ms, A.lnm, A.tz, nn, bb);
+        double nn, bb, ee;
+        massfn_point(A.P, z, m, nm, [&](int i) { return sig[i - m0 + 1]; }, A.ms, A.lnm, A.tz, nn, bb, ee);
         A.nzm[(size_t)z * nm + m] = nn;
         A.bh[(size_t)z * nm + m] = bb;
     }
 }
 
-template <int NT>
+template <int NT, bool WL = false>
 __device__ __forceinline__ void massfn_row(const SigmaMassFnArgs& A, int z, double* sig) {
     const int nm = A.nm, n = A.nz * nm, t = (int)threadIdx.x;
     const bool one = nm <= NT;
@@ -155,10 +165,11 @@
         if (mine) A.s2[i] = v;
         __syncthreads();
         if (mine) {
-            double nn, bb;
-            massfn_point(A.P, z, m, nm, [&](int k) { return sig[k - base]; }, A.ms, A.lnm, A.tz, nn, bb);
+            double nn, bb, ee;
+            massfn_point(A.P, z, m, nm, [&](int k) { return sig[k - base]; }, A.ms, A.lnm, A.tz, nn, bb, ee);
             A.nzm[i] = nn;
             A.bh[i] = bb;
+            if (WL && A.wl) A.wl[i] = row_weightless(ee) ? 1 : 0;
         }
         __syncthreads();
     }
diff --git a/hmvec_amd/csrc/kernels/power_batch.hpp b/hmvec_amd/csrc/kernels/power_batch.hpp
--- a/hmvec_amd/csrc/kernels/power_batch.hpp
+++ b/hmvec_amd/csrc/kernels/power_batch.hpp
@@ -171,6 +171,7 @@
     const double* tens[PW_MAXT];
     const int* nconst[PW_MAXT];
     const double* cconst[PW_MAXT];
+    const int* wl;
     const double* coef;
     const double* sidep;
     const double* ngal[PB_MAXTR];
@@ -191,7 +192,7 @@
     return __hiloint2double(hi, lo);
 }
 
-template <int NT, int NTR, int V, bool W16, unsigned CODE = 0>
+template <int NT, int NTR, int V, bool W16, unsigned CODE = 0, bool WL = false>
 __global__ __launch_bounds__(W16 ? 1024 : 512) void power_batch_kernel(BatchArgs A) {
     extern __shared__ double red[];
     using vec_t = typename VecT<V>::type;
@@ -220,9 +221,10 @@
         if (W16) return wv + PB_NV * i;
         return i < L ? wv + PB_NV * i : wv + 8 + PB_NV * (i - L);
     };
-    struct Hint { int n[NT]; double val[NT]; };
+    struct Hint { int n[NT]; double val[NT]; int dead; };
     auto load_hint = [&](Hint& h, int m) {
         const size_t r = zrow + min(m, A.nm - 1);
+        h.dead = WL ? A.wl[r] : 0;
 #pragma unroll
         for (int i = 0; i < NT; ++i) {
             h.n[i] = A.nconst[i] ? A.nconst[i][r] : -1;
@@ -233,9 +235,10 @@
         const size_t off = (zrow + min(m, A.nm - 1)) * (size_t)A.nk + kofs;
 #pragma unroll
         for (int i = 0; i < NT; ++i) {
-            if (h.n[i] >= kend) dst[i] = vsplat<V>(h.val[i]);
+            if (h.dead || h.n[i] >= kend) dst[i] = vsplat<V>(h.val[i]);
             else dst[i] = vload_nt<V>(A.tens[i] + off);
         }
+        return h.dead;
     };
     auto park = [&]() {
 #pragma unroll
@@ -246,10 +249,10 @@
                 acc[a][v] = 0.0;
             }
     };
-    auto accumulate = [&](const vec_t (&t)[NT], int i) {
+    auto accumulate = [&](const vec_t (&t)[NT], int i, int dead) {
         if (!W16 && i == L) park();
         const int m = bin(i);
-        if (m >= A.nm) return;
+        if (m >= A.nm || dead) return;
         const double* __restrict__ c = A.coef + (zrow + m) * (size_t)STRIDE;
         const double wn = c[0], wnb = c[1];
 #pragma unroll
@@ -305,21 +308,21 @@
     Hint ha, hb;
     load_hint(ha, bin(0));
     load_hint(hb, bin(1));
-    fetch(ta, bin(0), ha);
+    int da = fetch(ta, bin(0), ha), db = 0;
 #pragma unroll 1
     for (; i + 1 < NB; i += 2) {
-        fetch(tb, bin(i + 1), hb);
+        db = fetch(tb, bin(i + 1), hb);
         load_hint(ha, bin(i + 2));
         __builtin_amdgcn_sched_barrier(0);
-        accumulate(ta, i);
+        accumulate(ta, i, da);
         __builtin_amdgcn_sched_barrier(0);
-        fetch(ta, bin(i + 2), ha);
+        da = fetch(ta, bin(i + 2), ha);
         load_hint(hb, bin(i + 3));
         __builtin_amdgcn_sched_barrier(0);
-        accumulate(tb, i + 1);
+        accumulate(tb, i + 1, db);
         __builtin_amdgcn_sched_barrier(0);
     }
-    if (i < NB) accumulate(ta, i);
+    if (i < NB) accumulate(ta, i, da);
     if (W16) {
         if (wv >= 8) {
 #pragma unroll
diff --git a/hmvec_amd/csrc/runtime.hip b/hmvec_amd/csrc/runtime.hip
--- a/hmvec_amd/csrc/runtime.hip
+++ b/hmvec_amd/csrc/runtime.hip
@@ -357,6 +357,7 @@
     REQUIRE(c->lane == 0, "start a capture on lane 0");
     HIP_TRY(hipStreamBeginCapture(c->lanes[0], hipStreamCaptureModeRelaxed));
     c->capturing = true;
+    ++c->flags_serial;
     return 0;
 }
 static void release_deferred_frees(hmg_ctx* c) {
@@ -368,6 +369,7 @@
     REQUIRE(c && id, "NULL argument");
     REQUIRE(c->capturing, "no capture in progress");
     c->capturing = false;
+    ++c->flags_serial;
     c->lane = 0;
     c->stream = c->lanes[0];
     hipGraph_t g = nullptr;
@@ -408,6 +410,7 @@
     REQUIRE(c, "NULL ctx");
     if (!c->capturing) return 0;
     c->capturing = false;
+    ++c->flags_serial;
     release_deferred_frees(c);
     c->prefix_capture.clear();
     c->lane = 0;
diff --git a/hmvec_amd/halomodel.py b/hmvec_amd/halomodel.py
--- a/hmvec_amd/halomodel.py
+++ b/hmvec_amd/halomodel.py
@@ -153,6 +153,8 @@
         self._stages = []
         self._stage_dims = None
         self.prefix_deferral = os.environ.get("HMG_NO_PREFIX_DEFERRAL", "0") != "1"
+        self.row_deferral = os.environ.get("HMG_NO_ROW_DEFERRAL", "0") != "1"
+        self._d_weightless = self._row_flags_key = None
 
         self._pcache = {}
         self.uk_profiles = DeviceDict(self._ctx, self._bump)
@@ -403,6 +405,11 @@
             ctx = self._aux()
         par, d_lnm, d_tz, d_delta, d_rho = self._dcache["mf_in"]
         self._d_nzm, self._d_bh = self._buf("nzm", (nz, nm)), self._buf("bh", (nz, nm))
+        self._d_weightless = self._buf("weightless", ((nz * nm + 1) // 2,)) if self._groups and self.row_deferral else None
+        key = (self._d_nzm.ptr, nat.ptr(self._d_weightless))
+        if key != self._row_flags_key and (key[1] or self._row_flags_key):
+            ctx.call("hmg_row_flags", *key)
+        self._row_flags_key = key
         d_ms = self._d_ms()
         self._d_cs, self._d_rvir, self._d_rs = (self._buf(k, (nz, nm)) for k in ("cs", "rvir", "rs"))
         self._d_nfw_series = self._buf("nfw_series", (nz, nm, nat.NFW_SERIES_STRIDE))
diff --git a/include/hmgrid.h b/include/hmgrid.h
--- a/include/hmgrid.h
+++ b/include/hmgrid.h
@@ -152,6 +152,7 @@
 int hmg_prefix_fill(hmg_ctx* ctx, double* d_out);
 int hmg_prefix_pending(hmg_ctx* ctx, const double* d_out, int* pending);
 int hmg_prefix_fill_rows(hmg_ctx* ctx, double* d_out, const int* d_nconst, const double* d_cconst, int rows, int nk);
+int hmg_row_flags(hmg_ctx* ctx, const double* d_nzm, int* d_weightless);
 
 typedef struct {
     double sig_log_mstellar, alphasat, Bsat, betasat, Bcut, betacut;
```

Measured after the change: 881.0 billion (median of 6 runs). 1.9% higher.
